# leejaeyong7/nerfacc

Hardware: AMD Instinct MI355X
Metric: rays/sec (fwd+bwd) through 128^3 occ-grid, 1M-ray batch (higher is better)
Workload: dtype f32; 1 GPU; cfg2: 1048576 image rays/GPU, 128^3 shell10 occ grid (G=1), step 2*sqrt(3)/1024, sampling+rendering fwd+bwd; rays_per_gpu=1048576, resolution=128, grid=shell10, samples_after_compaction=32244949, parallelism=ray-sharded x1, field=synthetic analytic field, native callbacks (see bench.py NativeField/TorchField)

## Files before the change

### include/nerfacc_hip.h

```cpp
#ifndef NERFACC_HIP_H
#define NERFACC_HIP_H

#include <stdint.h>

#ifdef __cplusplus
extern "C" {
#endif

#define NFA_OK 0
#define NFA_EINVAL (-1)
#define NFA_EHIP (-2)

#define NFA_MAX_GRID_LEVELS 8

typedef void *nfa_stream_t;

#define NFA_ELEM_F32 0
#define NFA_ELEM_F16 1
#define NFA_ELEM_BF16 2

const char *nfa_last_error(void);
#define NFA_VERSION 403
int nfa_version(void);
int nfa_set_tuning(const char *name, const char *value);
int nfa_device_arch(char *buf, int buflen);


int64_t nfa_cumsum_scratch_bytes(int64_t n);
int nfa_exclusive_cumsum_i64(const int64_t *cnts, int64_t n, int64_t *starts, int64_t *total,
                             void *scratch, nfa_stream_t stream);
int nfa_exclusive_cumsum_pairs_i64(const int64_t *cnts, int64_t n, int64_t *packed_info , int64_t *total,
                                   void *scratch, nfa_stream_t stream);
int nfa_exclusive_cumsum_pairs_stats_i64(const int64_t *cnts, int64_t n, int64_t *packed_info ,
                                         int64_t *total_and_stats , void *scratch, nfa_stream_t stream);

int nfa_pack_info(const int64_t *ray_indices, int64_t n, int64_t n_rays, int64_t *packed_info ,
                  int32_t *flags , void *scratch, nfa_stream_t stream);

int nfa_unpack_rows(const void *packed, const int64_t *packed_info , const uint8_t *mask, int64_t n_rays,
                    int64_t n_per_ray, int64_t n_packed, int64_t row_bytes, const void *pad_host, int32_t pad_bytes,
                    void *padded, nfa_stream_t stream);
int nfa_pack_rows(const void *padded, const int64_t *packed_info , const uint8_t *mask, int64_t n_rays,
                  int64_t n_per_ray, int64_t n_packed, int64_t row_bytes, void *packed, nfa_stream_t stream);
int nfa_mask_row_counts(const uint8_t *mask, int64_t n_rows, int64_t n_cols, int64_t *counts, nfa_stream_t stream);

int nfa_pack_bits(const uint8_t *binaries, int64_t n_cells, uint32_t *bits , nfa_stream_t stream);


int nfa_ray_aabb_intersect(const float *rays_o, const float *rays_d, int64_t n_rays,
                           const float *aabbs, int32_t n_aabbs, float near_plane, float far_plane,
                           float miss_value, float *t_mins, float *t_maxs, uint8_t *hits,
                           nfa_stream_t stream);

#define NFA_MAX_EVENT_LEVELS 8
int nfa_ray_events(const float *rays_o, const float *rays_d, int64_t n_rays, const float *aabbs, int32_t n_aabbs,
                   float *t_sorted, int64_t *t_indices, uint8_t *hits, nfa_stream_t stream);

typedef struct nfa_traverse_args {
    int64_t n_rays;
    const float *rays_o;
    const float *rays_d;
    const uint8_t *rays_mask;
    int32_t n_grids;
    int32_t res[3];
    const uint8_t *binaries;
    const float *aabbs;
    const uint8_t *hits;
    const float *t_sorted;
    const int64_t *t_indices;
    const float *near_planes;
    const float *far_planes;
    float step_size;
    float cone_angle;
    int32_t traverse_steps_limit;
    int32_t mode;
    float *iv_vals; int64_t *iv_ray_indices; uint8_t *iv_is_left; uint8_t *iv_is_right;
    int64_t *iv_starts; int64_t *iv_cnts;
    float *sm_vals; int64_t *sm_ray_indices; uint8_t *sm_is_valid;
    float *sm_t_starts; float *sm_t_ends;
    int64_t *sm_starts; int64_t *sm_cnts;
    float *terminate_planes;
    const int32_t *ray_filter;
    int32_t ray_filter_min;
    const uint64_t *bricks;
    const uint32_t *coarse;
    const int32_t *steps_limit_dev;
    const int64_t *n_listed_dev;
    const int32_t *run_if_nonzero;
} nfa_traverse_args;
int nfa_traverse_grids(const nfa_traverse_args *args, nfa_stream_t stream);

int64_t nfa_bricks_words(int32_t n_grids, const int32_t *res);
int nfa_pack_bricks(const uint8_t *binaries, int32_t n_grids, const int32_t *res, uint64_t *bricks,
                    uint32_t *coarse, nfa_stream_t stream);
int64_t nfa_walk_bits_words(int32_t n_grids, const int32_t *res);
int nfa_pack_walk_bits(const uint8_t *binaries, int32_t n_grids, const int32_t *res, uint32_t *bits, nfa_stream_t stream);
int nfa_traverse_runs(const nfa_traverse_args *args, const uint32_t *bits, int32_t *run_cnts, uint64_t *runs,
                      int32_t max_runs, int32_t *overflow_count, float near_hint, const int32_t *ray_order,
                      int64_t n_order, nfa_stream_t stream);
int nfa_bin_rays(const float *rays_o, const float *rays_d, int64_t n_rays, const float *box, int32_t *order,
                 void *scratch, nfa_stream_t stream);
int nfa_alive_rays(const float *opacity, const int64_t *packed_info , int64_t n_samples, float opacity_max,
                   int64_t n_rays, uint8_t *mask, int32_t *alive, int64_t *count, nfa_stream_t stream);
int nfa_testmode_begin(int64_t *alive_count, int32_t *state, int64_t n_rays, int32_t min_samples, int32_t max_samples,
                       int64_t *sm_cnts, int32_t *run_cnts, int64_t *zero_words, int32_t n_zero, nfa_stream_t stream);
int nfa_testmode_alive(const float *opacity, const int64_t *packed_info, int32_t *state, float opacity_max, int64_t n_rays,
                       uint8_t *mask, int32_t *alive, int64_t *count, int32_t count_samples, nfa_stream_t stream);
int nfa_bin_rays_levels(const float *rays_o, const float *rays_d, int64_t n_rays, const float *aabbs, int32_t n_grids,
                        const int32_t *res, float near_plane, int32_t *order, void *scratch,
                        uint64_t *coherence , nfa_stream_t stream);
int nfa_expand_runs(int64_t n_rays, float step_size, const int32_t *run_cnts, const uint64_t *runs,
                    int32_t max_runs, const int64_t *packed_info , float *t_starts,
                    float *t_ends, float *t_mids, int64_t *ray_indices, int64_t capacity, nfa_stream_t stream);
int nfa_fill_ray_indices(int64_t n_rays, const int64_t *packed_info , int64_t *ray_indices,
                         nfa_stream_t stream);
int nfa_traverse_cone_runs(const nfa_traverse_args *args, int32_t *run_cnts, uint64_t *runs, int32_t max_runs,
                           int32_t *overflow_count, const int32_t *ray_order ,
                           int64_t n_order, nfa_stream_t stream);
int nfa_traverse_cone_walk(const nfa_traverse_args *args, const uint32_t *bits, int32_t *run_cnts, uint64_t *runs,
                           int32_t max_runs, int32_t *overflow_count, uint32_t *arena, int32_t arena_capacity,
                           const int32_t *ray_order, int64_t n_order, nfa_stream_t stream);
int nfa_expand_cone_arena(const uint32_t *arena, int32_t n_entries, float step_size, float cone_angle,
                          const int64_t *packed_info , float *t_starts, float *t_ends, int64_t *ray_indices,
                          nfa_stream_t stream);
int nfa_expand_cone_runs(int64_t n_rays, float step_size, float cone_angle, const int32_t *run_cnts,
                         const uint64_t *runs, int32_t max_runs, const int64_t *packed_info, float *t_starts,
                         float *t_ends, int64_t *ray_indices, nfa_stream_t stream);
int nfa_expand_intervals(int64_t n_rays, float step_size, const int32_t *run_cnts, const uint64_t *runs,
                         int32_t max_runs, const int64_t *iv_packed_info , float *vals,
                         int64_t *ray_indices, uint8_t *is_left, uint8_t *is_right, nfa_stream_t stream);


int nfa_grid_cell_points(const int64_t *indices, const float *jitter , int64_t n, const int32_t *res,
                         const float *aabb , float *x , nfa_stream_t stream);
int nfa_grid_ema_update(float *occs, int64_t cell_base, const int64_t *indices, int64_t n, const float *occ,
                        float ema_decay, float *scratch , nfa_stream_t stream);
int64_t nfa_grid_rebinarize_scratch_bytes(void);
int nfa_grid_rebinarize(const float *occs, int32_t n_grids, const int32_t *res, float occ_thre, uint8_t *binaries,
                        uint32_t *walk_bits, void *scratch, nfa_stream_t stream);


void nfa_seg_plan(int64_t n_elems, int64_t n_rays, int64_t *tile_elems, int64_t *n_tiles);
int64_t nfa_seg_table_rows(int64_t n_tiles);
int nfa_seg_build_tiles(const int64_t *packed_info , int64_t n_rays, int64_t n_elems,
                        int64_t tile_elems, int64_t n_tiles, int64_t *tiles ,
                        int32_t *flags, nfa_stream_t stream);

int nfa_packed_scan(int kind, int reverse, const int64_t *packed_info, const int64_t *tiles, int64_t n_tiles,
                    int64_t n_rays, int64_t n_elems, const float *inputs, float *outputs,
                    nfa_stream_t stream);
int nfa_packed_scan_generic(int kind, int reverse, int normalize, const int64_t *packed_info,
                            int64_t n_rays, int64_t n_elems, const float *inputs, float *outputs,
                            nfa_stream_t stream);
int nfa_packed_prod_backward(int kind, const int64_t *packed_info, const int64_t *tiles, int64_t n_tiles,
                             int64_t n_rays, int64_t n_elems, const float *inputs,
                             const float *outputs, const float *grad_outputs, float *grad_inputs,
                             nfa_stream_t stream);

int nfa_render_from_density_fwd(const float *t_starts, const float *t_ends, const float *sigmas,
                                const float *prefix_trans , const int64_t *packed_info,
                                const int64_t *tiles, int64_t n_tiles, int64_t n_rays, int64_t n_elems,
                                float *weights, float *trans, float *alphas, nfa_stream_t stream);
int nfa_render_from_alpha_fwd(const float *alphas, const float *prefix_trans, const int64_t *packed_info,
                              const int64_t *tiles, int64_t n_tiles, int64_t n_rays, int64_t n_elems,
                              float *weights, float *trans, nfa_stream_t stream);
int nfa_render_from_density_bwd(const float *t_starts, const float *t_ends, const float *trans,
                                const float *alphas, const float *g_weights, const float *g_trans,
                                const float *g_alphas, const int64_t *packed_info, const int64_t *tiles, int64_t n_tiles,
                                int64_t n_rays, int64_t n_elems, float *grad_sigmas, float *grad_x,
                                nfa_stream_t stream);
int nfa_density_cdf_rows_fwd(const float *t_starts, const float *t_ends, const float *sigmas, const int64_t *packed_info,
                             const int64_t *tiles, int64_t n_tiles, int64_t n_rays, int64_t n_elems, int32_t row_len,
                             float *trans, float *alphas, float *cdfs , nfa_stream_t stream);
int nfa_density_cdf_rows_bwd(const float *t_starts, const float *t_ends, const float *trans, const float *alphas,
                             const float *g_cdfs , const int64_t *packed_info, const int64_t *tiles,
                             int64_t n_tiles, int64_t n_rays, int64_t n_elems, int32_t row_len, float *grad_sigmas,
                             nfa_stream_t stream);
int nfa_render_from_alpha_bwd(const float *alphas, const float *trans, const float *g_weights,
                              const float *g_trans, const int64_t *packed_info, const int64_t *tiles, int64_t n_tiles,
                              int64_t n_rays, int64_t n_elems, float *grad_alphas, nfa_stream_t stream);

int nfa_render_visibility(const float *t_starts, const float *t_ends, const float *sigmas_or_alphas,
                          const float *prefix_trans, float early_stop_eps, float alpha_thre,
                          const int64_t *packed_info, const int64_t *tiles, int64_t n_tiles, int64_t n_rays,
                          int64_t n_elems, uint8_t *vis, int64_t *vis_cnts, nfa_stream_t stream);
int nfa_render_visibility_cs(const float *t_starts, float step, const float *sigmas, const float *prefix_trans,
                             float early_stop_eps, float alpha_thre, const int64_t *packed_info, const int64_t *tiles,
                             int64_t n_tiles, int64_t n_rays, int64_t n_elems, uint8_t *vis, int64_t *vis_cnts,
                             nfa_stream_t stream);
int nfa_compact_samples(const uint8_t *vis, const float *t_starts, const float *t_ends,
                        const int64_t *packed_info, const int64_t *tiles, int64_t n_tiles, const int64_t *out_starts,
                        int64_t n_rays, int64_t n_elems, int64_t *out_ray_indices,
                        float *out_t_starts, float *out_t_ends, int64_t capacity, nfa_stream_t stream);

int nfa_accumulate_along_rays(const float *weights, const float *values, int32_t D,
                              const int64_t *packed_info, const int64_t *tiles, int64_t n_tiles, int64_t n_rays,
                              int64_t n_elems, int accumulate, float *out, nfa_stream_t stream);
int nfa_accumulate_along_rays_atomic(const float *weights, const float *values, int32_t D,
                                     const int64_t *ray_indices, int64_t n_rays, int64_t n_elems,
                                     float *out, nfa_stream_t stream);
int nfa_accumulate_along_rays_bwd(const float *weights, const float *values, int32_t D,
                                  const float *g_out, const int64_t *packed_info, const int64_t *tiles, int64_t n_tiles,
                                  int64_t n_rays, int64_t n_elems, float *g_weights, float *g_values,
                                  nfa_stream_t stream);
int nfa_render_accumulate_fwd(const float *weights, const float *rgbs, const float *t_starts,
                              const float *t_ends, const int64_t *packed_info, const int64_t *tiles, int64_t n_tiles,
                              int64_t n_rays, int64_t n_elems, float *colors, float *opacities,
                              float *depths, nfa_stream_t stream);
int nfa_render_accumulate_bwd(const float *weights, const float *rgbs, const float *t_starts,
                              const float *t_ends, const float *g_colors, const float *g_opacities,
                              const float *g_depths, const int64_t *packed_info, const int64_t *tiles, int64_t n_tiles,
                              int64_t n_rays, int64_t n_elems, float *g_weights, float *g_rgbs,
                              nfa_stream_t stream);

int nfa_render_fused_fwd(const float *t_starts, const float *t_ends, const float *sigmas, const float *rgbs,
                         const int64_t *packed_info, const int64_t *tiles, int64_t n_tiles, int64_t n_rays,
                         int64_t n_elems, float *weights, float *trans, float *alphas, float *colors,
                         float *opacities, float *depths, nfa_stream_t stream);
int nfa_render_fused_bwd(const float *t_starts, const float *t_ends, const float *rgbs, const float *trans,
                         const float *alphas, const float *g_colors, const float *g_opacities,
                         const float *g_depths, const float *g_weights, const float *g_trans,
                         const float *g_alphas, const int64_t *packed_info, const int64_t *tiles, int64_t n_tiles,
                         int64_t n_rays, int64_t n_elems, float *grad_sigmas, float *grad_rgbs,
                         nfa_stream_t stream);
int nfa_render_fused_fwd_cs(const float *t_starts, float step, const float *sigmas, const float *rgbs,
                            const int64_t *packed_info, const int64_t *tiles, int64_t n_tiles, int64_t n_rays,
                            int64_t n_elems, float *weights, float *trans, float *alphas, float *colors,
                            float *opacities, float *depths, nfa_stream_t stream);
int nfa_render_fused_bwd_cs(const float *t_starts, float step, const float *rgbs, const float *trans,
                            const float *alphas, const float *g_colors, const float *g_opacities,
                            const float *g_depths, const float *g_weights, const float *g_trans,
                            const float *g_alphas, const int64_t *packed_info, const int64_t *tiles, int64_t n_tiles,
                            int64_t n_rays, int64_t n_elems, float *grad_sigmas, float *grad_rgbs,
                            nfa_stream_t stream);

#define NFA_ACT_NONE 0
#define NFA_ACT_TRUNC_EXP 1
#define NFA_ACT_EXP 2
#define NFA_ACT_RELU 3
#define NFA_ACT_SOFTPLUS 4
#define NFA_RGB_ACT_NONE 0
#define NFA_RGB_ACT_SIGMOID 1
// ... 348 lines not shown
```

### nerfacc_amd/_backend.py

```python
from __future__ import annotations

import ctypes as C
import os
import threading
from typing import Optional

import torch

from . import _build

_lock = threading.Lock()
_lib: Optional[C.CDLL] = None

_vp, _i64, _i32, _f32, _u64, _int = C.c_void_p, C.c_int64, C.c_int32, C.c_float, C.c_uint64, C.c_int


class TraverseArgs(C.Structure):
    _fields_ = [
        ("n_rays", _i64), ("rays_o", _vp), ("rays_d", _vp), ("rays_mask", _vp),
        ("n_grids", _i32), ("res", _i32 * 3), ("binaries", _vp), ("aabbs", _vp),
        ("hits", _vp), ("t_sorted", _vp), ("t_indices", _vp),
        ("near_planes", _vp), ("far_planes", _vp),
        ("step_size", _f32), ("cone_angle", _f32), ("traverse_steps_limit", _i32), ("mode", _i32),
        ("iv_vals", _vp), ("iv_ray_indices", _vp), ("iv_is_left", _vp), ("iv_is_right", _vp),
        ("iv_starts", _vp), ("iv_cnts", _vp),
        ("sm_vals", _vp), ("sm_ray_indices", _vp), ("sm_is_valid", _vp),
        ("sm_t_starts", _vp), ("sm_t_ends", _vp), ("sm_starts", _vp), ("sm_cnts", _vp),
        ("terminate_planes", _vp),
        ("ray_filter", _vp), ("ray_filter_min", _i32),
        ("bricks", _vp), ("coarse", _vp),
        ("steps_limit_dev", _vp), ("n_listed_dev", _vp), ("run_if_nonzero", _vp),
    ]


class MLPDesc(C.Structure):
    _fields_ = [("n_in", _i32), ("n_out", _i32), ("width", _i32), ("n_hidden", _i32), ("bias", _i32), ("skip_mask", _i32)]


OPTIM_MAX_GROUPS, OPTIM_MAX_MILESTONES = 16, 8


class OptimGroup(C.Structure):
    _fields_ = [("lr", C.c_double), ("beta1", C.c_double), ("beta2", C.c_double), ("eps", C.c_double), ("weight_decay", C.c_double),
                ("flags", _i32), ("reserved", _i32)]


class OptimArgs(C.Structure):
    _fields_ = [("n_groups", _i32), ("n_milestones", _i32), ("groups", OptimGroup * OPTIM_MAX_GROUPS),
                ("start_factor", C.c_double), ("gamma", C.c_double), ("warmup_iters", _i64), ("milestones", _i64 * OPTIM_MAX_MILESTONES),
                ("growth_factor", _f32), ("backoff_factor", _f32), ("growth_interval", _i32), ("reserved", _i32)]


_SIGS = {
    "nfa_exclusive_cumsum_i64": [_vp, _i64, _vp, _vp, _vp, _vp],
    "nfa_exclusive_cumsum_pairs_i64": [_vp, _i64, _vp, _vp, _vp, _vp],
    "nfa_exclusive_cumsum_pairs_stats_i64": [_vp, _i64, _vp, _vp, _vp, _vp],
    "nfa_pack_info": [_vp, _i64, _i64, _vp, _vp, _vp, _vp],
    "nfa_pdf_loss_fwd": [_vp, _vp, _vp, _vp, _i64, _i32, _i32, _f32, _vp, _vp, _vp],
    "nfa_pdf_loss_bwd": [_vp, _vp, _vp, _i64, _i32, _i32, _f32, _vp, _vp, _vp, _vp],
    "nfa_pdf_loss_partials": [_i64, _i32, _i32],
    "nfa_pdf_loss_sum_fwd": [_vp, _vp, _vp, _vp, _i64, _i32, _i32, _f32, _vp, _vp, _vp],
    "nfa_pdf_loss_mean_bwd": [_vp, _vp, _vp, _i64, _i32, _i32, _f32, _vp, _vp, _vp, _vp],
    "nfa_pack_bits": [_vp, _i64, _vp, _vp],
    "nfa_unpack_rows": [_vp, _vp, _vp, _i64, _i64, _i64, _i64, _vp, _i32, _vp, _vp],
    "nfa_pack_rows": [_vp, _vp, _vp, _i64, _i64, _i64, _i64, _vp, _vp],
    "nfa_mask_row_counts": [_vp, _i64, _i64, _vp, _vp],
    "nfa_ray_aabb_intersect": [_vp, _vp, _i64, _vp, _i32, _f32, _f32, _f32, _vp, _vp, _vp, _vp],
    "nfa_ray_events": [_vp, _vp, _i64, _vp, _i32, _vp, _vp, _vp, _vp],
    "nfa_traverse_grids": [C.POINTER(TraverseArgs), _vp],
    "nfa_bricks_words": [_i32, C.POINTER(_i32)],
    "nfa_pack_bricks": [_vp, _i32, C.POINTER(_i32), _vp, _vp, _vp],
    "nfa_walk_bits_words": [_i32, C.POINTER(_i32)],
    "nfa_pack_walk_bits": [_vp, _i32, C.POINTER(_i32), _vp, _vp],
    "nfa_traverse_runs": [C.POINTER(TraverseArgs), _vp, _vp, _vp, _i32, _vp, _f32, _vp, _i64, _vp],
    "nfa_bin_rays": [_vp, _vp, _i64, _vp, _vp, _vp, _vp],
    "nfa_grid_cell_points": [_vp, _vp, _i64, C.POINTER(_i32), _vp, _vp, _vp],
    "nfa_grid_ema_update": [_vp, _i64, _vp, _i64, _vp, _f32, _vp, _vp],
    "nfa_grid_rebinarize_scratch_bytes": [],
    "nfa_grid_rebinarize": [_vp, _i32, C.POINTER(_i32), _f32, _vp, _vp, _vp, _vp],
    "nfa_expand_runs": [_i64, _f32, _vp, _vp, _i32, _vp, _vp, _vp, _vp, _vp, _i64, _vp],
    "nfa_fill_ray_indices": [_i64, _vp, _vp, _vp],
    "nfa_traverse_cone_runs": [C.POINTER(TraverseArgs), _vp, _vp, _i32, _vp, _vp, _i64, _vp],
    "nfa_alive_rays": [_vp, _vp, _i64, _f32, _i64, _vp, _vp, _vp, _vp],
    "nfa_testmode_begin": [_vp, _vp, _i64, _i32, _i32, _vp, _vp, _vp, _i32, _vp],
    "nfa_testmode_alive": [_vp, _vp, _vp, _f32, _i64, _vp, _vp, _vp, _i32, _vp],
    "nfa_traverse_cone_walk": [C.POINTER(TraverseArgs), _vp, _vp, _vp, _i32, _vp, _vp, _i32, _vp, _i64, _vp],
    "nfa_expand_cone_arena": [_vp, _i32, _f32, _f32, _vp, _vp, _vp, _vp, _vp],
    "nfa_bin_rays_levels": [_vp, _vp, _i64, _vp, _i32, C.POINTER(_i32), _f32, _vp, _vp, _vp, _vp],
    "nfa_expand_cone_runs": [_i64, _f32, _f32, _vp, _vp, _i32, _vp, _vp, _vp, _vp, _vp],
    "nfa_expand_intervals": [_i64, _f32, _vp, _vp, _i32, _vp, _vp, _vp, _vp, _vp, _vp],
    "nfa_seg_plan": [_i64, _i64, C.POINTER(_i64), C.POINTER(_i64)],
    "nfa_seg_table_rows": [_i64],
    "nfa_seg_build_tiles": [_vp, _i64, _i64, _i64, _i64, _vp, _vp, _vp],
    "nfa_packed_scan": [_int, _int, _vp, _vp, _i64, _i64, _i64, _vp, _vp, _vp],
    "nfa_packed_scan_generic": [_int, _int, _int, _vp, _i64, _i64, _vp, _vp, _vp],
    "nfa_packed_prod_backward": [_int, _vp, _vp, _i64, _i64, _i64, _vp, _vp, _vp, _vp, _vp],
    "nfa_render_from_density_fwd": [_vp, _vp, _vp, _vp, _vp, _vp, _i64, _i64, _i64, _vp, _vp, _vp, _vp],
    "nfa_render_from_alpha_fwd": [_vp, _vp, _vp, _vp, _i64, _i64, _i64, _vp, _vp, _vp],
    "nfa_render_from_density_bwd": [_vp, _vp, _vp, _vp, _vp, _vp, _vp, _vp, _vp, _i64, _i64, _i64, _vp, _vp, _vp],
    "nfa_density_cdf_rows_fwd": [_vp, _vp, _vp, _vp, _vp, _i64, _i64, _i64, _i32, _vp, _vp, _vp, _vp],
    "nfa_density_cdf_rows_bwd": [_vp, _vp, _vp, _vp, _vp, _vp, _vp, _i64, _i64, _i64, _i32, _vp, _vp],
    "nfa_render_from_alpha_bwd": [_vp, _vp, _vp, _vp, _vp, _vp, _i64, _i64, _i64, _vp, _vp],
    "nfa_render_visibility": [_vp, _vp, _vp, _vp, _f32, _f32, _vp, _vp, _i64, _i64, _i64, _vp, _vp, _vp],
    "nfa_render_visibility_cs": [_vp, _f32, _vp, _vp, _f32, _f32, _vp, _vp, _i64, _i64, _i64, _vp, _vp, _vp],
    "nfa_compact_samples": [_vp, _vp, _vp, _vp, _vp, _i64, _vp, _i64, _i64, _vp, _vp, _vp, _i64, _vp],
    "nfa_accumulate_along_rays": [_vp, _vp, _i32, _vp, _vp, _i64, _i64, _i64, _int, _vp, _vp],
    "nfa_accumulate_along_rays_atomic": [_vp, _vp, _i32, _vp, _i64, _i64, _vp, _vp],
    "nfa_accumulate_along_rays_bwd": [_vp, _vp, _i32, _vp, _vp, _vp, _i64, _i64, _i64, _vp, _vp, _vp],
    "nfa_render_accumulate_fwd": [_vp, _vp, _vp, _vp, _vp, _vp, _i64, _i64, _i64, _vp, _vp, _vp, _vp],
    "nfa_render_accumulate_bwd": [_vp, _vp, _vp, _vp, _vp, _vp, _vp, _vp, _vp, _i64, _i64, _i64, _vp, _vp, _vp],
    "nfa_render_fused_fwd": [_vp, _vp, _vp, _vp, _vp, _vp, _i64, _i64, _i64, _vp, _vp, _vp, _vp, _vp, _vp, _vp],
    "nfa_render_fused_bwd": [_vp] * 13 + [_i64, _i64, _i64, _vp, _vp, _vp],
    "nfa_render_fused_fwd_cs": [_vp, _f32, _vp, _vp, _vp, _vp, _i64, _i64, _i64, _vp, _vp, _vp, _vp, _vp, _vp, _vp],
    "nfa_render_fused_bwd_cs": [_vp, _f32] + [_vp] * 11 + [_i64, _i64, _i64, _vp, _vp, _vp],
    "nfa_render_raw_fwd": [_vp] * 5 + [_i32, _f32, _i32, _vp, _vp, _i64, _i64, _i64] + [_vp] * 9,
    "nfa_render_raw_bwd": [_vp] * 5 + [_i32, _f32, _i32] + [_vp] * 9 + [_i64, _i64, _i64, _vp, _vp, _vp],
    "nfa_render_raw_fwd_t": [_i32] + [_vp] * 5 + [_i32, _f32, _i32, _vp, _vp, _i64, _i64, _i64] + [_vp] * 9,
    "nfa_render_raw_bwd_t": [_i32] + [_vp] * 5 + [_i32, _f32, _i32] + [_vp] * 9 + [_i64, _i64, _i64, _vp, _vp, _vp],
    "nfa_render_sdf_fwd": [_vp] * 6 + [_i32, _vp, _f32, _i32, _vp, _vp, _i64, _i64, _i64] + [_vp] * 7,
    "nfa_render_sdf_bwd": [_vp] * 6 + [_i32, _vp, _f32, _i32] + [_vp] * 9 + [_i64, _i64, _i64] + [_vp] * 5,
    "nfa_render_step_accumulate": [_vp, _vp, _vp, _vp, _vp, _vp, _i64, _i64, _i64, _f32, _vp, _vp, _vp, _vp, _vp],
    "nfa_distortion_fwd": [_vp, _vp, _vp, _vp, _vp, _i64, _i64, _i64, _vp, _vp, _vp, _vp],
    "nfa_distortion_bwd": [_vp] * 8 + [_i64, _i64, _i64, _vp, _vp, _vp, _vp],
    "nfa_importance_sampling": [_vp, _vp, _vp, _i64, _i64, _i64, _int, _u64, _u64, _vp, _vp, _vp],
    "nfa_importance_sampling_t": [_vp, _vp, _vp, _i64, _i64, _i64, _int, _u64, _u64, _vp, _vp, _int, _f32, _f32, _vp, _vp, _vp],
    "nfa_importance_sampling_packed": [_vp, _vp, _vp, _i64, _i64, _vp, _vp, _int, _u64, _u64, _vp, _vp, _vp, _vp, _vp, _vp, _vp],
    "nfa_searchsorted": [_vp, _vp, _vp, _i64, _i64, _i64, _vp, _vp, _i64, _vp, _vp, _vp],
    "nfa_opencv_lens_undistortion": [_vp, _vp, _i64, _i32, _i64, _f32, _i32, _vp, _vp],
    "nfa_opencv_lens_undistortion_fisheye": [_vp, _vp, _i64, _i32, _i64, _f32, _i32, _vp, _vp],
    "nfa_hashgrid_fwd": [_vp, _vp, _i64, _i32, _i32, _i32, _vp, _vp, _vp, _i64, _vp, _vp],
    "nfa_hashgrid_bwd": [_vp, _vp, _vp, _i64, _i32, _i32, _i32, _vp, _vp, _vp, _i64, _vp, _vp, _vp],
    "nfa_sh_fwd": [_vp, _i64, _i32, _vp, _vp],
    "nfa_sh_bwd": [_vp, _vp, _i64, _i32, _vp, _vp],
    "nfa_hashgrid_fwd_t": [_i32, _vp, _vp, _i64, _i32, _i32, _i32, _vp, _vp, _vp, _i64, _vp, _vp],
    "nfa_hashgrid_bwd_t": [_i32, _vp, _vp, _vp, _i64, _i32, _i32, _i32, _vp, _vp, _vp, _i64, _vp, _vp, _vp],
    "nfa_hashgrid_bwd_bwd": [_vp, _vp, _vp, _vp, _i64, _i32, _i32, _i32, _vp, _vp, _vp, _i64, _vp, _vp, _vp, _vp],
    "nfa_hashgrid_bwd_bwd_t": [_i32, _vp, _vp, _vp, _vp, _i64, _i32, _i32, _i32, _vp, _vp, _vp, _i64, _vp, _vp, _vp, _vp],
    "nfa_hashgrid_sorted_scratch_bytes": [_i64, _i32, _i32],
    "nfa_hashgrid_bwd_sorted": [_i32, _vp, _vp, _vp, _i64, _i32, _i32, _i32, _vp, _vp, _vp, _i64, _vp, _vp, _vp, _i64, _vp],
    "nfa_hashgrid_bwd_bwd_sorted": [_i32, _vp, _vp, _vp, _vp, _i64, _i32, _i32, _i32, _vp, _vp, _vp, _i64, _vp, _vp, _vp, _vp, _i64, _vp],
    "nfa_hashgrid_fwd_i": [_i32, _i32, _vp, _vp, _i64, _i32, _i32, _i32, _vp, _vp, _vp, _i64, _vp, _vp],
    "nfa_hashgrid_bwd_i": [_i32, _i32, _vp, _vp, _vp, _i64, _i32, _i32, _i32, _vp, _vp, _vp, _i64, _vp, _vp, _vp],
    "nfa_hashgrid_bwd_bwd_i": [_i32, _i32, _vp, _vp, _vp, _vp, _i64, _i32, _i32, _i32, _vp, _vp, _vp, _i64, _vp, _vp, _vp, _vp],
    "nfa_hashgrid_bwd_sorted_i": [_i32, _i32, _vp, _vp, _vp, _i64, _i32, _i32, _i32, _vp, _vp, _vp, _i64, _vp, _vp, _vp, _i64, _vp],
    "nfa_hashgrid_bwd_bwd_sorted_i": [_i32, _i32, _vp, _vp, _vp, _vp, _i64, _i32, _i32, _i32, _vp, _vp, _vp, _i64, _vp, _vp, _vp, _vp,
                                      _i64, _vp],
    "nfa_hashgrid_fwd_d": [_i32, _i32, _i32, _vp, _vp, _i64, _i32, _i32, _i32, _vp, _vp, _vp, _i64, _vp, _vp],
    "nfa_hashgrid_bwd_d": [_i32, _i32, _i32, _vp, _vp, _vp, _i64, _i32, _i32, _i32, _vp, _vp, _vp, _i64, _vp, _vp, _vp],
    "nfa_hashgrid_bwd_sorted_d": [_i32, _i32, _i32, _vp, _vp, _vp, _i64, _i32, _i32, _i32, _vp, _vp, _vp, _i64, _vp, _vp, _vp, _i64,
                                  _vp],
    "nfa_hashgrid_sorted_scratch_bytes_d": [_i32, _i64, _i32, _i32],
    "nfa_sh_fwd_t": [_i32, _vp, _i64, _i32, _vp, _vp],
    "nfa_sh_bwd_t": [_i32, _vp, _vp, _i64, _i32, _vp, _vp],
    "nfa_planegrid_fwd": [_i32, _i32, _i32, _vp, _vp, _i64, _i32, _i32, C.POINTER(_i32), _vp, _vp],
    "nfa_planegrid_bwd": [_i32, _i32, _i32, _vp, _vp, _vp, _i64, _i32, _i32, C.POINTER(_i32), _vp, _vp, _vp],
    "nfa_planereg_partials": [_i32, _i32, _i32, C.POINTER(_i32)],
    "nfa_planereg_fwd": [_i32, _vp, _i32, _i32, C.POINTER(_i32), _vp, _i64, _vp, _vp],
    "nfa_planereg_bwd": [_i32, _vp, _i32, _i32, C.POINTER(_i32), _vp, _vp, _vp],
    "nfa_vmgrid_fwd": [_i32, _i32, _vp, _vp, _i64, _i32, C.POINTER(_i32), _vp, _vp],
    "nfa_vmgrid_bwd": [_i32, _i32, _vp, _vp, _vp, _i64, _i32, C.POINTER(_i32), _vp, _vp, _vp],
    "nfa_vmgrid_resample": [_vp, C.POINTER(_i32), _vp, C.POINTER(_i32), _i32, _vp],
    "nfa_vmreg_partials": [_i32, C.POINTER(_i32)],
    "nfa_vmreg_fwd": [_vp, _i32, C.POINTER(_i32), _vp, _i64, _vp, _vp, _vp],
    "nfa_vmreg_bwd": [_vp, _i32, C.POINTER(_i32), _vp, _vp, _vp, _vp],
    "nfa_sinenc_fwd": [_i32, _vp, _vp, _vp, _i64, _i32, _i32, _i32, _i32, _vp, _vp],
    "nfa_sinenc_bwd": [_i32, _vp, _vp, _vp, _vp, _i64, _i32, _i32, _i32, _i32, _vp, _vp, _vp],
    "nfa_sinenc_bwd_bwd": [_i32, _vp, _vp, _vp, _vp, _i64, _i32, _i32, _i32, _i32, _vp, _vp, _vp],
    "nfa_sample_positions_fwd": [_vp, _vp, _vp, _vp, _vp, _i64, _i64, _i64, _vp, _vp, _i32, _i32, _vp, _vp, _vp, _vp],
    "nfa_sample_positions_bwd": [_vp] * 9 + [_i64, _i64, _i64, _i64, _vp, _vp, _i32, _i32, _vp, _vp, _vp, _vp, _vp, _vp],
    "nfa_generate_rays_fwd": [_vp, _vp, _i32, _vp, _i64, _i64, _vp, _i64, _vp, _i64, _vp, _i32, _i64, _i32, _i32, _f32, _i32, _f32, _i32,
                              _vp, _vp, _vp],
    "nfa_generate_rays_bwd": [_vp, _vp, _i32, _vp, _vp, _i64, _i64, _vp, _i64, _vp, _i64, _vp, _i32, _i64, _i32, _i32, _f32, _i32, _f32,
                              _i32, _vp, _vp, _vp, _i64, _i32, _vp, _vp, _vp],
    "nfa_generate_rays_chunk": [],
    "nfa_mlp_pack_weights": [_i32, _vp, _i32, _i32, _i32, _i32, _vp, _i64, _vp, _i64, _vp],
    "nfa_mlp_fwd": [_i32, _vp, _i32, _vp, _i64, _i32, _i32, _i32, _i32, _vp, _i32, _vp, _i32, _vp],
    "nfa_mlp_bwd_data": [_i32, _vp, _i32, _vp, _vp, _i64, _i32, _i32, _i32, _i32, _vp, _vp, _vp, _i32, _vp],
    "nfa_mlp_bwd_weights": [_i32, _vp, _i32, _vp, _vp, _vp, _i64, _i32, _i32, _i32, _i32, _vp, _i64, _vp, _vp],
    "nfa_mlp_tangent": [_i32, _vp, _i32, _vp, _vp, _i64, _i32, _i32, _i32, _i32, _vp, _vp, _i32, _vp],
    "nfa_mlp_net_pack_weights": [_i32, C.POINTER(MLPDesc), _vp, _vp, _i64, _vp, _i64, _vp],
    "nfa_mlp_net_fwd": [_i32, C.POINTER(MLPDesc), _vp, _i32, _vp, _vp, _i64, _vp, _i32, _vp, _i32, _vp],
    "nfa_mlp_net_bwd_data": [_i32, C.POINTER(MLPDesc), _vp, _i32, _vp, _vp, _i64, _vp, _vp, _vp, _i32, _vp],
    "nfa_mlp_net_bwd_weights": [_i32, C.POINTER(MLPDesc), _vp, _i32, _vp, _vp, _vp, _i64, _vp, _i64, _vp, _i32, _vp],
    "nfa_mlp_net_tangent": [_i32, C.POINTER(MLPDesc), _vp, _i32, _vp, _vp, _i64, _vp, _vp, _i32, _vp],
    "nfa_mlp_stream_pack_weights": [_i32, C.POINTER(MLPDesc), _vp, _vp, _i64, _vp, _i64, _vp],
    "nfa_mlp_stream_fwd": [_i32, C.POINTER(MLPDesc), _vp, _i32, _vp, _vp, _i64, _vp, _i32, _vp, _i32, _vp],
    "nfa_mlp_stream_bwd_data": [_i32, C.POINTER(MLPDesc), _vp, _i32, _vp, _vp, _i64, _vp, _vp, _vp, _i32, _vp],
    "nfa_mlp_stream_bwd_weights": [_i32, C.POINTER(MLPDesc), _vp, _i32, _vp, _vp, _vp, _i64, _vp, _i64, _vp, _i32, _vp],
    "nfa_optim_chunk_elems": [],
    "nfa_optim_scan": [_i32, _vp, _i32, _vp, _i64, _vp, _vp],
    "nfa_optim_decide": [C.POINTER(OptimArgs), _vp, _vp, _vp],
    "nfa_optim_update": [_i32, _vp, _i32, _vp, _i64, _vp, _i32, _vp],
    "nfa_cumsum_scratch_bytes": [_i64],
    "nfa_last_error": [],
    "nfa_version": [],
    "nfa_set_tuning": [C.c_char_p, C.c_char_p],
    "nfa_device_arch": [C.c_char_p, _int],
}
_RESTYPES = {"nfa_grid_rebinarize_scratch_bytes": _i64, "nfa_hashgrid_sorted_scratch_bytes": _i64, "nfa_hashgrid_sorted_scratch_bytes_d": _i64, "nfa_planereg_partials": _i64, "nfa_vmreg_partials": _i64, "nfa_bricks_words": _i64, "nfa_walk_bits_words": _i64, "nfa_pdf_loss_partials": _i64, "nfa_cumsum_scratch_bytes": _i64, "nfa_seg_table_rows": _i64, "nfa_seg_plan": None, "nfa_last_error": C.c_char_p}

EXPORTED_SYMBOLS = tuple(_SIGS)


def library_path() -> str:
    return _build.LIB_PATH


def load() -> C.CDLL:
    global _lib
    if _lib is not None:
        return _lib
    with _lock:
        if _lib is not None:
            return _lib
        path = _build.LIB_PATH
        if _build.is_stale() and _build.hipcc() is not None:
            path = _build.build()
        if not os.path.exists(path):
            raise RuntimeError(
                "nerfacc_amd: libnerfacc_hip.so is missing and hipcc is not available to build it. "
                "There is no CPU fallback for the native ops.")
        lib = C.CDLL(path)
        for name, argtypes in _SIGS.items():
            fn = getattr(lib, name)
            fn.argtypes = argtypes
            fn.restype = _RESTYPES[name] if name in _RESTYPES else _int
        if lib.nfa_version() != ABI_VERSION:
            raise RuntimeError(f"nerfacc_amd: {path} was built from include/nerfacc_hip.h version {lib.nfa_version()}, these "
                               f"bindings are written for {ABI_VERSION}: rebuild the library (nerfacc_amd._build.build(force=True))")
        _lib = lib
    return _lib


ABI_VERSION = 403


ELEM_CODES = {torch.float32: 0, torch.float16: 1, torch.bfloat16: 2}
INTERP_CODES = {"Linear": 0, "Smoothstep": 1}
PLANE_REDUCE_CODES = {"product": 0, "sum": 1}
VM_REDUCE_CODES = {"concat": 0, "sum": 1}


def set_tuning(name: str, value: Optional[str]) -> None:
    call("nfa_set_tuning", name.encode(), None if value is None else str(value).encode())


class NativeError(RuntimeError):
    """Counterpart of the RuntimeError TORCH_CHECK raises in the reference."""


def call(name: str, *args) -> None:
    lib = load()
    rc = getattr(lib, name)(*args)
    if rc != 0:
        msg = lib.nfa_last_error()
        raise NativeError(f"{name}: {msg.decode() if msg else rc}")


def call_group(name: str, fn) -> None:
    fn()


def ptr(t: Optional[torch.Tensor]):
    return None if t is None else t.data_ptr()


_RAW_STREAM = getattr(torch._C, "_cuda_getCurrentRawStream", None)
_CUR_DEVICE = getattr(torch._C, "_cuda_getDevice", None)


def stream() -> int:
    if _RAW_STREAM is not None and _CUR_DEVICE is not None:
        return _RAW_STREAM(_CUR_DEVICE())
    return torch.cuda.current_stream().cuda_stream


def require_device(*tensors: Optional[torch.Tensor]) -> torch.device:
    dev = None
    for t in tensors:
        if t is None:
            continue
        if not t.is_cuda:
            raise NotImplementedError(
                "nerfacc_amd: this op runs only on a ROCm device (the reference has no CPU "
                "implementation of its native ops either); got a tensor on " + str(t.device))
        if dev is None:
            dev = t.device
        elif t.device != dev:
            raise RuntimeError(f"nerfacc_amd: tensors on different devices ({dev} vs {t.device})")
    if dev is None:
        raise RuntimeError("nerfacc_amd: no tensor argument")
    return dev


def seg_plan(n_elems: int, n_rays: int = 0):
    t, n = _i64(0), _i64(0)
    load().nfa_seg_plan(n_elems, n_rays, C.byref(t), C.byref(n))
    return int(t.value), int(n.value)


def cumsum_scratch(n: int, device) -> torch.Tensor:
    nbytes = ((max(n, 1) + 2047) // 2048 + 1) * 8
    return torch.empty(nbytes // 8, dtype=torch.int64, device=device)
```

### nerfacc_amd/_segments.py

```python
from __future__ import annotations

import ctypes
import weakref
from dataclasses import dataclass
from typing import Optional

import torch
from torch import Tensor

from . import _backend as B


@dataclass
class SegInfo:
    packed_info: Tensor
    n_rays: int
    n_elems: int
    tiles: Optional[Tensor]
    contiguous: bool
    sorted_indices: bool = True
    n_tiles: int = 0
    trusted: bool = False


_ATTR = "_nfa_seg"
_ATTR_RI = "_nfa_seg_from_ray_indices"


def _build_tiles(packed_info: Tensor, n_elems: int, trusted: bool) -> SegInfo:
    dev = B.require_device(packed_info)
    n_rays = packed_info.shape[0]
    with torch.cuda.device(dev):
        tile_elems, n_tiles = B.seg_plan(n_elems, n_rays)
        tiles = torch.empty((int(B.load().nfa_seg_table_rows(n_tiles)), 2), dtype=torch.int64, device=dev)
        flag = None if trusted else torch.empty(1, dtype=torch.int32, device=dev)
        B.call("nfa_seg_build_tiles", B.ptr(packed_info), n_rays, n_elems, tile_elems, n_tiles, B.ptr(tiles), B.ptr(flag),
               B.stream())
        ok = True if trusted else (int(flag.item()) == 0)
    return SegInfo(packed_info, n_rays, n_elems, tiles if ok else None, ok, n_tiles=n_tiles, trusted=trusted)


def seginfo_from_packed(packed_info: Tensor, n_elems: int, trusted: bool = False) -> SegInfo:
    assert packed_info.dim() == 2 and packed_info.shape[-1] == 2, "packed_info must be 2-D with shape (B, 2)."
    cached = getattr(packed_info, _ATTR, None)
    if cached is not None and cached[0] == packed_info._version and cached[1] == n_elems:
        return cached[2]
    pi = packed_info
    if pi.dtype != torch.int64 or not pi.is_contiguous():
        pi = pi.to(torch.int64).contiguous()
    info = _build_tiles(pi, n_elems, trusted)
    try:
        setattr(packed_info, _ATTR, (packed_info._version, n_elems, info))
    except Exception:
        pass
    return info


def tag_trusted(packed_info: Tensor, n_elems: int) -> SegInfo:
    return seginfo_from_packed(packed_info, n_elems, trusted=True)


def pack_info_native(ray_indices: Tensor, n_rays: int):
    dev = B.require_device(ray_indices)
    ri = ray_indices if (ray_indices.dtype == torch.int64 and ray_indices.is_contiguous()) else \
        ray_indices.to(torch.int64).contiguous()
    with torch.cuda.device(dev):
        packed = torch.empty((n_rays, 2), dtype=torch.int64, device=dev)
        flag = torch.empty(1, dtype=torch.int32, device=dev)
        scratch = B.cumsum_scratch(n_rays, dev)
        B.call("nfa_pack_info", B.ptr(ri), ri.numel(), n_rays, B.ptr(packed), B.ptr(flag), B.ptr(scratch), B.stream())
    return packed, flag


def seginfo_from_ray_indices(ray_indices: Tensor, n_rays: int) -> SegInfo:
    assert ray_indices.dim() == 1, "ray_indices must be a 1D tensor with shape (n_samples)."
    assert n_rays is not None, "n_rays must be provided"
    cached = getattr(ray_indices, _ATTR_RI, None)
    if cached is not None and cached[0] == ray_indices._version and cached[1] == n_rays:
        return cached[2]
    packed, flag = pack_info_native(ray_indices, n_rays)
    info = _build_tiles(packed, ray_indices.numel(), trusted=True)
    info.sorted_indices = int(flag.item()) == 0
    try:
        setattr(ray_indices, _ATTR_RI, (ray_indices._version, n_rays, info))
    except Exception:
        pass
    return info


def tag_ray_indices(ray_indices: Tensor, n_rays: int, info: SegInfo) -> None:
    setattr(ray_indices, _ATTR_RI, (ray_indices._version, n_rays, info))


def resolve(n_elems: int, packed_info: Optional[Tensor], ray_indices: Optional[Tensor],
            n_rays: Optional[int]) -> Optional[SegInfo]:
    if packed_info is not None:
        return seginfo_from_packed(packed_info, n_elems)
    if ray_indices is not None:
        if n_rays is None:
            n_rays = int(ray_indices.max().item()) + 1 if ray_indices.numel() else 0
        return seginfo_from_ray_indices(ray_indices, n_rays)
    return None


_ATTR_CS = "_nfa_const_step"


def tag_const_step(t_starts: Tensor, t_ends: Tensor, step: float) -> None:
    tag = (t_ends._version, weakref.ref(t_starts), t_starts.data_ptr(), t_starts._version, ctypes.c_float(float(step)).value)
    try:
        setattr(t_ends, _ATTR_CS, tag)
    except Exception:
        pass


def const_step_of(t_starts: Optional[Tensor], t_ends: Optional[Tensor]) -> Optional[float]:
    tag = getattr(t_ends, _ATTR_CS, None) if t_ends is not None else None
    if tag is None or t_starts is None:
        return None
    te_version, ts_ref, ts_ptr, ts_version, step = tag
    if t_ends._version != te_version or ts_ref() is not t_starts:
        return None
    if t_starts.data_ptr() != ts_ptr or t_starts._version != ts_version:
        return None
    for t in (t_starts, t_ends):
        if not (t.is_cuda and t.dtype == torch.float32 and t.dim() == 1 and t.is_contiguous()):
            return None
    if t_starts.shape != t_ends.shape or not (0.0 < step < float("inf")):
        return None
    return step


_UNIFORM: "dict[tuple, SegInfo]" = {}


def uniform_seginfo(n_rows: int, row_len: int, device: torch.device) -> SegInfo:
    key = (int(n_rows), int(row_len), device.type, device.index)
    info = _UNIFORM.get(key)
    if info is None:
        starts = torch.arange(n_rows, dtype=torch.int64, device=device) * row_len
        packed = torch.stack([starts, torch.full_like(starts, row_len)], dim=-1)
        info = _build_tiles(packed, n_rows * row_len, trusted=True)
        setattr(packed, _ATTR, (packed._version, n_rows * row_len, info))
        if len(_UNIFORM) >= 6:
            _UNIFORM.pop(next(iter(_UNIFORM)))
        _UNIFORM[key] = info
    return info


def batched_native(*tensors: Optional[Tensor]) -> Optional[SegInfo]:
    ref = None
    for t in tensors:
        if t is None:
            continue
        if not t.is_cuda or t.dtype != torch.float32 or t.dim() < 1:
            return None
        if ref is None:
            ref = t
        elif t.shape != ref.shape:
            return None
    if ref is None or ref.numel() == 0:
        return None
    return uniform_seginfo(ref.numel() // ref.shape[-1], ref.shape[-1], ref.device)
```

### nerfacc_amd/csrc/common.hip.h

```cpp
#pragma once
#include <hip/hip_runtime.h>
#include <stdint.h>
#include <stdio.h>
#include <stdlib.h>
#include <string.h>

#include <type_traits>

#include "../../include/nerfacc_hip.h"

#define NFA_WAVE 64

namespace nfa {

void set_error(const char *fmt, ...);

#define NFA_REQUIRE(cond, ...)                         \
    do {                                               \
        if (!(cond)) {                                 \
            nfa::set_error(__VA_ARGS__);               \
            return NFA_EINVAL;                         \
        }                                              \
    } while (0)

#define NFA_CHECK_LAUNCH(name)                                                       \
    do {                                                                             \
        hipError_t e__ = hipGetLastError();                                          \
        if (e__ != hipSuccess) {                                                     \
            nfa::set_error("%s: launch failed: %s", name, hipGetErrorString(e__));   \
            return NFA_EHIP;                                                         \
        }                                                                            \
    } while (0)

const char *tuning_env(const char *name);

struct RefillPlan {
    bool refill;
    int64_t chunk;
    int32_t min_busy;
};
static inline RefillPlan refill_plan(int64_t n_walk, int32_t steps_limit)
{
    const char *refill_env = tuning_env("NFA_REFILL"), *refill_all = tuning_env("NFA_REFILL_ALL");
    if (!(steps_limit > 0 || (refill_all && refill_all[0] == '1')) || (refill_env && refill_env[0] == '0')) return RefillPlan{false, 64, 64};
    int64_t chunk = ((n_walk + 4095) / 4096 + 63) / 64 * 64;
    chunk = chunk < 64 ? 64 : (chunk > 1024 ? 1024 : chunk);
    int min_busy = 48;
    if (refill_env) { long c = 0; int m = 0; if (sscanf(refill_env, "%ld,%d", &c, &m) == 2 && c >= 64 && m >= 1 && m <= 64) { chunk = c / 64 * 64; min_busy = m; } }
    return RefillPlan{true, chunk, min_busy};
}

static inline hipStream_t as_stream(nfa_stream_t s) { return reinterpret_cast<hipStream_t>(s); }

__host__ __device__ static inline int64_t ceil_div64(int64_t a, int64_t b) { return (a + b - 1) / b; }

static inline unsigned grid_1d(int64_t n, int block, int64_t cap = 256 * 16)
{
    int64_t g = ceil_div64(n, block);
    if (g > cap) g = cap;
    if (g < 1) g = 1;
    return (unsigned)g;
}

static inline bool aligned16(const void *p) { return (reinterpret_cast<uintptr_t>(p) & 15) == 0; }
template <typename... P>
static inline bool all_aligned16(P... p) { return (aligned16(p) && ...); }

template <class F>
static void dispatch_bool(bool b, F &&f)
{
    if (b) f(std::true_type{});
    else f(std::false_type{});
}
template <class F>
static void dispatch_channels(int c, F &&f)
{
    if (c == 4) f(std::integral_constant<int, 4>{});
    else if (c == 3) f(std::integral_constant<int, 3>{});
    else if (c == 2) f(std::integral_constant<int, 2>{});
    else f(std::integral_constant<int, 1>{});
}
template <class F>
static void dispatch_lanes(int l, F &&f)
{
    if (l == 2) f(std::integral_constant<int, 2>{});
    else if (l == 4) f(std::integral_constant<int, 4>{});
    else if (l == 8) f(std::integral_constant<int, 8>{});
    else if (l == 16) f(std::integral_constant<int, 16>{});
    else if (l == 32) f(std::integral_constant<int, 32>{});
    else f(std::integral_constant<int, 64>{});
}
template <int... V, class Fn>
static void dispatch_value(int32_t v, Fn &&f)
{
    (void)((v == V && (f(std::integral_constant<int, V>{}), true)) || ...);
}

__device__ __forceinline__ int lane_id() { return __lane_id(); }

template <typename T>
__device__ __forceinline__ T wave_shfl_up(T v, int delta) { return __shfl_up(v, delta, NFA_WAVE); }
template <typename T>
__device__ __forceinline__ T wave_shfl(T v, int src) { return __shfl(v, src, NFA_WAVE); }

__device__ __forceinline__ int64_t wave_incl_sum_i64(int64_t v)
{
    const int lane = lane_id();
#pragma unroll
    for (int off = 1; off < NFA_WAVE; off <<= 1) {
        int64_t u = __shfl_up(v, off, NFA_WAVE);
        if (lane >= off) v += u;
    }
    return v;
}

__device__ __forceinline__ float wave_sum_f32(float v)
{
#pragma unroll
    for (int off = 32; off > 0; off >>= 1) v += __shfl_xor(v, off, NFA_WAVE);
    return v;
}

__device__ __forceinline__ int64_t uniform64(int64_t v)
{
    const uint32_t lo = (uint32_t)__builtin_amdgcn_readfirstlane((int32_t)(uint32_t)v);
    const uint32_t hi = (uint32_t)__builtin_amdgcn_readfirstlane((int32_t)(uint32_t)((uint64_t)v >> 32));
    return (int64_t)(((uint64_t)hi << 32) | lo);
}

template <int S>
__device__ __forceinline__ int32_t dpp_step(int32_t old, int32_t src)
{
    static_assert(S >= 0 && S < 6, "dpp_step");
    if constexpr (S == 0) return __builtin_amdgcn_update_dpp(old, src, 0x111, 0xf, 0xf, false);
    else if constexpr (S == 1) return __builtin_amdgcn_update_dpp(old, src, 0x112, 0xf, 0xf, false);
    else if constexpr (S == 2) return __builtin_amdgcn_update_dpp(old, src, 0x114, 0xf, 0xf, false);
    else if constexpr (S == 3) return __builtin_amdgcn_update_dpp(old, src, 0x118, 0xf, 0xf, false);
    else if constexpr (S == 4) return __builtin_amdgcn_update_dpp(old, src, 0x142, 0xa, 0xf, false);
    else return __builtin_amdgcn_update_dpp(old, src, 0x143, 0xc, 0xf, false);
}
template <int S>
__device__ __forceinline__ float dpp_step(float old, float src)
{
    return __int_as_float(dpp_step<S>(__float_as_int(old), __float_as_int(src)));
}
__device__ __forceinline__ int32_t dpp_prev_lane(int32_t old, int32_t src)
{
    return __builtin_amdgcn_update_dpp(old, src, 0x138, 0xf, 0xf, false);
}
__device__ __forceinline__ float dpp_prev_lane(float old, float src)
{
    return __int_as_float(dpp_prev_lane(__float_as_int(old), __float_as_int(src)));
}
__device__ __forceinline__ int32_t event_level(int64_t idx, int32_t G)
{
    const int32_t i = (int32_t)idx;
    return i >= G ? i - G : i;
}

__device__ __forceinline__ uint32_t mad_u24(uint32_t a, uint32_t b, uint32_t c)
{
    uint32_t r;
    asm("v_mad_u32_u24 %0, %1, %2, %3" : "=v"(r) : "v"(a), "v"(b), "v"(c));
    return r;
}
__device__ __forceinline__ int64_t xcd_fair_block(uint32_t b, uint32_t n_blocks)
{
    const uint32_t group = b >> 3;
    if (((group + 1u) << 3) > n_blocks) return b;
    return (int64_t)((b & ~7u) | ((b + group) & 7u));
}

__device__ __forceinline__ uint32_t sel_mask(uint32_t k, uint32_t x, uint32_t y)
{
    return __builtin_amdgcn_bitop3_b32(k, x, y, 0xca);
}
__device__ __forceinline__ float sel_mask(uint32_t k, float x, float y)
{
    return __builtin_bit_cast(float, __builtin_amdgcn_bitop3_b32(k, __builtin_bit_cast(uint32_t, x), __builtin_bit_cast(uint32_t, y), 0xca));
}
__device__ __forceinline__ uint32_t mask_less(float a, float b)
{
    return (uint32_t)(__builtin_bit_cast(int32_t, a - b) >> 31);
}
__device__ __forceinline__ float min3_f32(float a, float b, float c)
{
    float m;
    asm("v_min3_f32 %0, %1, %2, %3" : "=v"(m) : "v"(a), "v"(b), "v"(c));
    return m;
}

__device__ __forceinline__ int32_t last_lane(int32_t v) { return __builtin_amdgcn_readlane(v, 63); }
__device__ __forceinline__ float last_lane(float v) { return __int_as_float(__builtin_amdgcn_readlane(__float_as_int(v), 63)); }
__device__ __forceinline__ int32_t lane_value(int32_t v, int32_t l) { return __builtin_amdgcn_readlane(v, l); }
__device__ __forceinline__ float lane_value(float v, int32_t l) { return __int_as_float(__builtin_amdgcn_readlane(__float_as_int(v), l)); }


typedef float nfa_v4f __attribute__((ext_vector_type(4)));
typedef long long nfa_v2l __attribute__((ext_vector_type(2)));
typedef uint32_t nfa_v2u __attribute__((ext_vector_type(2)));
typedef uint32_t nfa_v4u __attribute__((ext_vector_type(4)));

typedef _Float16 nfa_f16;
// ... 200 lines not shown
```

### nerfacc_amd/csrc/grid.hip

```cpp
#include <stdarg.h>

#include "common.hip.h"
#include "march.h"

namespace nfa {

static thread_local char g_err[512] = "";
void set_error(const char *fmt, ...)
{
    va_list ap;
    va_start(ap, fmt);
    vsnprintf(g_err, sizeof(g_err), fmt, ap);
    va_end(ap);
}

struct TuningKnob { char name[32]; char value[64]; };
static TuningKnob g_knobs[8];
static int g_n_knobs = 0;
const char *tuning_env(const char *name)
{
    for (int i = 0; i < g_n_knobs; ++i)
        if (strcmp(g_knobs[i].name, name) == 0) return g_knobs[i].value[0] ? g_knobs[i].value : nullptr;
    return nullptr;
}
// ... 252 lines not shown
        if (a.traverse_steps_limit <= 0) return;
    }
    const int64_t n_walk = (EMIT == EMIT_RUNS && ro.order) ? ro.n_order : a.n_rays;
    for (int64_t slot_i = (int64_t)blockIdx.x * blockDim.x + threadIdx.x; slot_i < n_walk;
         slot_i += (int64_t)blockDim.x * gridDim.x) {
        const int64_t tid = (EMIT == EMIT_RUNS && ro.order) ? (int64_t)ro.order[slot_i] : slot_i;
        const bool overalloc = a.mode == 2;
        if (ray_masked(a, ro, tid)) continue;
        if (a.ray_filter != nullptr && a.ray_filter[tid] <= a.ray_filter_min) continue;
        int64_t iv_base = 0, sm_base = 0;
        if (EMIT != EMIT_NONE && EMIT != EMIT_RUNS) {
            if (a.mode == 1) {
                if (HAS_IV && a.iv_cnts[tid] == 0) continue;
                if (HAS_SM && a.sm_cnts[tid] == 0) continue;
            }
            if (HAS_IV) iv_base = a.iv_starts[tid];
            if (HAS_SM) sm_base = a.sm_starts[tid];
        }
        float near_plane, far_plane, o[3], d[3];
        const bool ray_ok = ray_load(a, tid, near_plane, far_plane, o, d);
        const float inv[3] = {1.0f / d[0], 1.0f / d[1], 1.0f / d[2]};

        RayState st;
        st.t_last = near_plane;
        st.continuous = 0;
        st.n_intervals = 0;
        st.n_samples = 0;
        st.brick_id = -1; st.brick_lo = st.brick_hi = 0u;
        st.n_runs = 0; st.run_len = 0;

        int32_t ev = ray_ok ? 0 : 2 * a.n_grids, level;
        float this_tmin, this_tmax;
        while (next_span<FUSED>(a, tid, o, inv, near_plane, far_plane, ev, level, this_tmin, this_tmax)) {
            traverse_span<EMIT, HAS_IV, HAS_SM>(a, tid, o, d, inv, level, this_tmin, this_tmax, iv_base, sm_base, st, ro);
            if (FUSED || (a.traverse_steps_limit > 0 && st.n_samples >= a.traverse_steps_limit)) break;
        }
        if (EMIT == EMIT_RUNS) {
            run_ray_close(a, ro, tid, st.t_last, st.n_samples, st.n_runs);
            continue;
        }
        if (a.terminate_planes) a.terminate_planes[tid] = st.t_last;
        if (EMIT == EMIT_NONE || overalloc) {
            if (HAS_IV) a.iv_cnts[tid] = st.n_intervals;
            if (HAS_SM) a.sm_cnts[tid] = st.n_samples;
        }
    }
}

template <int EMIT, bool HAS_IV, bool HAS_SM>
static void launch_traverse(const nfa_traverse_args &a, bool fused, hipStream_t s, const RunOut ro = RunOut{nullptr, nullptr, 0, nullptr, nullptr, 0})
{
    const unsigned grid = grid_1d((EMIT == EMIT_RUNS && ro.order) ? ro.n_order : a.n_rays, 256, 1 << 20);
    if (fused) hipLaunchKernelGGL((traverse_kernel<EMIT, HAS_IV, HAS_SM, true>), dim3(grid), dim3(256), 0, s, a, ro);
    else       hipLaunchKernelGGL((traverse_kernel<EMIT, HAS_IV, HAS_SM, false>), dim3(grid), dim3(256), 0, s, a, ro);
}

template <bool FUSED>
struct BrickWalker {
    const nfa_traverse_args &a;
    const RunOut &ro;
    int64_t tid;
    int32_t ev;
    float near_plane, far_plane, o[3], d[3], inv[3];
    RayState st;
    SpanState &sp;
    __device__ __forceinline__ bool take(int64_t ray)
    {
        tid = ray;
        if (ray_masked(a, ro, tid)) return false;
        if (a.ray_filter != nullptr && a.ray_filter[tid] <= a.ray_filter_min) return false;
        const bool ray_ok = ray_load(a, tid, near_plane, far_plane, o, d);
#pragma unroll
        for (int ax = 0; ax < 3; ++ax) inv[ax] = 1.0f / d[ax];
        st.t_last = near_plane; st.continuous = 0; st.n_samples = 0;
        st.brick_id = -1; st.n_runs = 0; st.run_len = 0;
        ev = ray_ok ? 0 : 2 * a.n_grids;
        return true;
    }
    __device__ __forceinline__ bool next_span()
    {
        int32_t level;
        float this_tmin, this_tmax;
        if (!nfa::next_span<FUSED>(a, tid, o, inv, near_plane, far_plane, ev, level, this_tmin, this_tmax)) return false;
        span_begin(a, o, d, inv, level, this_tmin, this_tmax, st, sp);
        return true;
    }
    __device__ __forceinline__ int cell()
    {
        if (!span_cell<EMIT_RUNS, false, true, true>(a, tid, 0, 0, sp, st, ro)) return RF_WALK;
        return (a.traverse_steps_limit > 0 && st.n_samples >= a.traverse_steps_limit) ? RF_FINISH : RF_SPAN;
    }
    __device__ __forceinline__ void finish() { run_ray_close(a, ro, tid, st.t_last, st.n_samples, st.n_runs); }
};
template <bool FUSED>
__global__ __launch_bounds__(256) void traverse_refill_kernel(const nfa_traverse_args a, const RunOut ro, const int32_t chunk,
                                                              const int32_t min_busy)
{
    SpanState sp;
    BrickWalker<FUSED> w{a, ro, 0, 0, 0.0f, 0.0f, {0.0f, 0.0f, 0.0f}, {0.0f, 0.0f, 0.0f}, {0.0f, 0.0f, 0.0f}, RayState{0.0f, 0, 0, 0, -1, 0u, 0u, 0, 0}, sp};
    refill_schedule(w, ro.order, ro.order ? ro.n_order : a.n_rays, (int64_t)blockIdx.x * (blockDim.x >> 6) + (threadIdx.x >> 6), chunk, min_busy);
}

constexpr int CS_THREADS = 256;
constexpr int CS_ITEMS = 8;
constexpr int CS_BLOCK = CS_THREADS * CS_ITEMS;

__device__ __forceinline__ int64_t block_excl_scan_i64(int64_t v, int64_t &block_total, int64_t *lds )
{
    const int lane = lane_id(), wave = threadIdx.x >> 6;
    const int64_t incl = wave_incl_sum_i64(v);
    if (lane == 63) lds[wave] = incl;
    __syncthreads();
    int64_t wave_off = 0, tot = 0;
#pragma unroll
    for (int w = 0; w < CS_THREADS / 64; ++w) {
        const int64_t x = lds[w];
        if (w < wave) wave_off += x;
        tot += x;
    }
    __syncthreads();
    block_total = tot;
    return wave_off + incl - v;
}

__global__ __launch_bounds__(CS_THREADS) void cumsum_partials_kernel(const int64_t *__restrict__ in, int64_t n,
                                                                      int64_t in_stride, int64_t *__restrict__ partials)
{
    __shared__ int64_t lds[8];
    const int64_t base = (int64_t)blockIdx.x * CS_BLOCK + (int64_t)threadIdx.x * CS_ITEMS;
    int64_t s = 0;
#pragma unroll
    for (int k = 0; k < CS_ITEMS; ++k)
        if (base + k < n) s += in[(base + k) * in_stride];
    int64_t tot;
    block_excl_scan_i64(s, tot, lds);
    if (threadIdx.x == 0) partials[blockIdx.x] = tot;
}

__global__ __launch_bounds__(CS_THREADS) void cumsum_spine_kernel(int64_t *partials, int64_t n_blocks, int64_t *total)
{
    __shared__ int64_t lds[8];
    int64_t carry = 0;
    for (int64_t base = 0; base < n_blocks; base += CS_THREADS) {
        const int64_t i = base + threadIdx.x;
        const int64_t v = i < n_blocks ? partials[i] : 0;
        int64_t tot;
        const int64_t ex = block_excl_scan_i64(v, tot, lds);
        if (i < n_blocks) partials[i] = carry + ex;
        carry += tot;
    }
    if (threadIdx.x == 0 && total) *total = carry;
}

template <bool SPINE>
__global__ __launch_bounds__(CS_THREADS) void cumsum_final_kernel(const int64_t *__restrict__ in, int64_t n,
                                                                   int64_t in_stride,
                                                                   const int64_t *__restrict__ partials,
                                                                   int64_t *__restrict__ out, int pairs,
                                                                   int64_t *__restrict__ total,
                                                                   unsigned long long *__restrict__ stats = nullptr)
{
    __shared__ int64_t lds[8];
    int64_t block_off = 0;
    if (SPINE) {
        int64_t before = 0;
        for (int64_t j = threadIdx.x; j < (int64_t)blockIdx.x; j += CS_THREADS) before += partials[j];
        block_excl_scan_i64(before, block_off, lds);
    } else {
        block_off = partials[blockIdx.x];
    }
    const int64_t base = (int64_t)blockIdx.x * CS_BLOCK + (int64_t)threadIdx.x * CS_ITEMS;
    int64_t v[CS_ITEMS];
    int64_t s = 0;
#pragma unroll
    for (int k = 0; k < CS_ITEMS; ++k) {
        v[k] = (base + k < n) ? in[(base + k) * in_stride] : 0;
        s += v[k];
    }
    int64_t tot;
    int64_t run = block_off + block_excl_scan_i64(s, tot, lds);
    if (SPINE && total && blockIdx.x == gridDim.x - 1 && threadIdx.x == 0) *total = block_off + tot;
    if (SPINE && stats && (blockIdx.x & 7) == 0) {
        int64_t m = 0;
#pragma unroll
        for (int k = 0; k < CS_ITEMS; ++k) m = v[k] > m ? v[k] : m;
        for (int off = 1; off < 8; off <<= 1) { const int64_t u = __shfl_xor(m, off, 64); m = u > m ? u : m; }
        int64_t gm = (lane_id() & 7) == 0 ? m : 0;
        for (int off = 8; off < 64; off <<= 1) gm += __shfl_xor(gm, off, 64);
        if (lane_id() == 0) atomicAdd(&stats[0], (unsigned long long)gm);
        if (threadIdx.x == 0) atomicAdd(&stats[1], (unsigned long long)tot);
    }
#pragma unroll
    for (int k = 0; k < CS_ITEMS; ++k) {
        if (base + k < n) {
            if (pairs) { out[2 * (base + k)] = run; out[2 * (base + k) + 1] = v[k]; }
            else out[base + k] = run;
        }
        run += v[k];
    }
}

static int run_cumsum(const int64_t *in, int64_t n, int64_t in_stride, int64_t *out, int pairs, int64_t *total,
                      void *scratch, hipStream_t s, unsigned long long *stats = nullptr)
{
    const int64_t n_blocks = ceil_div64(n > 0 ? n : 1, CS_BLOCK);
    int64_t *partials = reinterpret_cast<int64_t *>(scratch);
    hipLaunchKernelGGL(cumsum_partials_kernel, dim3((unsigned)n_blocks), dim3(CS_THREADS), 0, s, in, n, in_stride, partials);
    if (n_blocks <= 2048) {
        hipLaunchKernelGGL(cumsum_final_kernel<true>, dim3((unsigned)n_blocks), dim3(CS_THREADS), 0, s, in, n, in_stride, partials,
                           out, pairs, total, stats);
    } else {
        hipLaunchKernelGGL(cumsum_spine_kernel, dim3(1), dim3(CS_THREADS), 0, s, partials, n_blocks, total);
        hipLaunchKernelGGL(cumsum_final_kernel<false>, dim3((unsigned)n_blocks), dim3(CS_THREADS), 0, s, in, n, in_stride, partials,
                           out, pairs, nullptr, nullptr);
    }
    NFA_CHECK_LAUNCH("exclusive_cumsum_i64");
    return NFA_OK;
}

__global__ __launch_bounds__(256) void pack_hist_kernel(const int64_t *__restrict__ ray_indices, int64_t n,
                                                        int64_t n_rays, unsigned long long *__restrict__ packed,
                                                        int32_t *__restrict__ flags)
{
    const int lane = lane_id();
    for (int64_t base = ((int64_t)blockIdx.x * blockDim.x + threadIdx.x) - lane; base < n;
         base += (int64_t)blockDim.x * gridDim.x) {
        const int64_t i = base + lane;
        const bool valid = i < n;
        const int64_t r = valid ? ray_indices[i] : -1;
        int64_t prev = __shfl_up(r, 1, NFA_WAVE);
        if (lane == 0) prev = (i > 0 && valid) ? ray_indices[i - 1] : r;
        const bool in_range = valid && r >= 0 && r < n_rays;
        if (valid && (!in_range || r < prev)) atomicOr(flags, 1);
        const bool head = valid && (lane == 0 || r != prev);
        const unsigned long long heads = __ballot(head);
        const unsigned long long live = __ballot(valid);
        if (head && in_range) {
            const unsigned long long later = (lane == 63) ? 0ull : (heads >> (lane + 1));
            const int next = later ? (lane + 1 + __builtin_ctzll(later)) : (int)__builtin_popcountll(live);
            atomicAdd(&packed[2 * r + 1], (unsigned long long)(next - lane));
        }
    }
}

__global__ void zero_i64_kernel(int64_t *p, int64_t n, int32_t *flags)
{
    for (int64_t i = (int64_t)blockIdx.x * blockDim.x + threadIdx.x; i < n; i += (int64_t)blockDim.x * gridDim.x) p[i] = 0;
    if (flags && blockIdx.x == 0 && threadIdx.x == 0) *flags = 0;
}

__global__ __launch_bounds__(256) void pack_bits_kernel(const uint8_t *__restrict__ b, int64_t n, uint32_t *__restrict__ bits)
{
    const int lane = lane_id();
    for (int64_t base = ((int64_t)blockIdx.x * blockDim.x + threadIdx.x) - lane; base < n;
         base += (int64_t)blockDim.x * gridDim.x) {
        const int64_t i = base + lane;
        const unsigned long long m = __ballot(i < n && b[i] != 0);
        if (lane == 0) bits[base >> 5] = (uint32_t)m;
        if (lane == 32 && base + 32 < n) bits[(base >> 5) + 1] = (uint32_t)(m >> 32);
    }
}

}

using namespace nfa;

extern "C" {

const char *nfa_last_error(void) { return g_err; }
int nfa_version(void) { return NFA_VERSION; }
int nfa_set_tuning(const char *name, const char *value)
{
    NFA_REQUIRE(name && strlen(name) > 0 && strlen(name) < sizeof(g_knobs[0].name), "set_tuning: bad name");
    NFA_REQUIRE(!value || strlen(value) < sizeof(g_knobs[0].value), "set_tuning: value too long");
    int i = 0;
    while (i < g_n_knobs && strcmp(g_knobs[i].name, name) != 0) ++i;
    if (i == g_n_knobs) {
        NFA_REQUIRE(g_n_knobs < (int)(sizeof(g_knobs) / sizeof(g_knobs[0])), "set_tuning: too many knobs");
        strcpy(g_knobs[g_n_knobs++].name, name);
    }
    strcpy(g_knobs[i].value, value ? value : "");
    return NFA_OK;
}

int nfa_device_arch(char *buf, int buflen)
{
    int dev = 0;
    hipDeviceProp_t prop;
    if (hipGetDevice(&dev) != hipSuccess || hipGetDeviceProperties(&prop, dev) != hipSuccess) {
        set_error("no HIP device");
        return NFA_EHIP;
    }
    snprintf(buf, buflen, "%s", prop.gcnArchName);
    return NFA_OK;
}

int64_t nfa_cumsum_scratch_bytes(int64_t n) { return (ceil_div64(n > 0 ? n : 1, CS_BLOCK) + 1) * 8; }

int nfa_exclusive_cumsum_i64(const int64_t *cnts, int64_t n, int64_t *starts, int64_t *total, void *scratch,
                             nfa_stream_t stream)
{
    NFA_REQUIRE(n >= 0 && scratch && (n == 0 || (cnts && starts)), "exclusive_cumsum_i64: bad arguments");
    return run_cumsum(cnts, n, 1, starts, 0, total, scratch, as_stream(stream));
}

int nfa_exclusive_cumsum_pairs_i64(const int64_t *cnts, int64_t n, int64_t *packed_info, int64_t *total, void *scratch,
                                   nfa_stream_t stream)
{
    NFA_REQUIRE(n >= 0 && scratch && (n == 0 || (cnts && packed_info)), "exclusive_cumsum_pairs_i64: bad arguments");
    return run_cumsum(cnts, n, 1, packed_info, 1, total, scratch, as_stream(stream));
}

int nfa_exclusive_cumsum_pairs_stats_i64(const int64_t *cnts, int64_t n, int64_t *packed_info, int64_t *total_and_stats,
                                         void *scratch, nfa_stream_t stream)
{
    NFA_REQUIRE(n >= 0 && scratch && total_and_stats && (n == 0 || (cnts && packed_info)),
                "exclusive_cumsum_pairs_stats_i64: bad arguments");
    return run_cumsum(cnts, n, 1, packed_info, 1, total_and_stats, scratch, as_stream(stream),
                      reinterpret_cast<unsigned long long *>(total_and_stats + 1));
}

int nfa_pack_info(const int64_t *ray_indices, int64_t n, int64_t n_rays, int64_t *packed_info, int32_t *flags,
                  void *scratch, nfa_stream_t stream)
{
    NFA_REQUIRE(n >= 0 && n_rays >= 0 && flags && scratch, "pack_info: bad arguments");
    NFA_REQUIRE(n_rays == 0 || packed_info, "pack_info: packed_info is null");
    NFA_REQUIRE(n == 0 || ray_indices, "pack_info: ray_indices is null");
    hipStream_t s = as_stream(stream);
    hipLaunchKernelGGL(zero_i64_kernel, dim3(grid_1d(2 * n_rays + 1, 256)), dim3(256), 0, s, packed_info, 2 * n_rays, flags);
    if (n > 0 && n_rays > 0)
        hipLaunchKernelGGL(pack_hist_kernel, dim3(grid_1d(n, 256)), dim3(256), 0, s, ray_indices, n, n_rays,
                           reinterpret_cast<unsigned long long *>(packed_info), flags);
    NFA_CHECK_LAUNCH("pack_info");
    if (n_rays == 0) return NFA_OK;
    return run_cumsum(packed_info + 1, n_rays, 2, packed_info, 1, nullptr, scratch, s);
}

int nfa_pack_bits(const uint8_t *binaries, int64_t n_cells, uint32_t *bits, nfa_stream_t stream)
{
    NFA_REQUIRE(n_cells >= 0 && (n_cells == 0 || (binaries && bits)), "pack_bits: bad arguments");
    if (n_cells == 0) return NFA_OK;
    hipLaunchKernelGGL(pack_bits_kernel, dim3(grid_1d(n_cells, 256)), dim3(256), 0, as_stream(stream), binaries, n_cells, bits);
    NFA_CHECK_LAUNCH("pack_bits");
    return NFA_OK;
}

int nfa_ray_aabb_intersect(const float *rays_o, const float *rays_d, int64_t n_rays, const float *aabbs,
                           int32_t n_aabbs, float near_plane, float far_plane, float miss_value, float *t_mins,
                           float *t_maxs, uint8_t *hits, nfa_stream_t stream)
{
    NFA_REQUIRE(n_rays >= 0 && n_aabbs >= 0, "ray_aabb_intersect: negative size");
    if (n_rays * (int64_t)n_aabbs == 0) return NFA_OK;
    NFA_REQUIRE(rays_o && rays_d && aabbs && t_mins && t_maxs && hits, "ray_aabb_intersect: null pointer");
    hipLaunchKernelGGL(ray_aabb_kernel, dim3(grid_1d(n_rays * n_aabbs, 256)), dim3(256), 0, as_stream(stream), rays_o,
                       rays_d, n_rays, aabbs, n_aabbs, near_plane, far_plane, miss_value, t_mins, t_maxs, hits);
    NFA_CHECK_LAUNCH("ray_aabb_intersect");
    return NFA_OK;
}

int nfa_ray_events(const float *rays_o, const float *rays_d, int64_t n_rays, const float *aabbs, int32_t n_aabbs,
                   float *t_sorted, int64_t *t_indices, uint8_t *hits, nfa_stream_t stream)
{
    NFA_REQUIRE(n_rays >= 0 && n_aabbs >= 1 && n_aabbs <= NFA_MAX_EVENT_LEVELS, "ray_events: 1..NFA_MAX_EVENT_LEVELS boxes");
    if (n_rays == 0) return NFA_OK;
    NFA_REQUIRE(rays_o && rays_d && aabbs && t_sorted && t_indices && hits, "ray_events: null pointer");
    const dim3 grid(grid_1d(n_rays, 256)), block(256);
    hipStream_t s = as_stream(stream);
    static constexpr decltype(&ray_events_kernel<1>) kernels[NFA_MAX_EVENT_LEVELS] = {
        ray_events_kernel<1>, ray_events_kernel<2>, ray_events_kernel<3>, ray_events_kernel<4>,
        ray_events_kernel<5>, ray_events_kernel<6>, ray_events_kernel<7>, ray_events_kernel<8>};
    hipLaunchKernelGGL(kernels[n_aabbs - 1], grid, block, 0, s, rays_o, rays_d, n_rays, aabbs, t_sorted, t_indices, hits);
    NFA_CHECK_LAUNCH("ray_events");
    return NFA_OK;
}

int nfa_traverse_grids(const nfa_traverse_args *pa, nfa_stream_t stream)
{
    NFA_REQUIRE(pa != nullptr, "traverse_grids: null args");
    const nfa_traverse_args &a = *pa;
    NFA_REQUIRE(a.n_rays >= 0 && a.n_rays < (int64_t)1 << 31, "traverse_grids: n_rays out of range");
    if (a.n_rays == 0) return NFA_OK;
    NFA_REQUIRE(a.mode >= 0 && a.mode <= 2, "traverse_grids: mode must be 0, 1 or 2");
    NFA_REQUIRE(a.rays_o && a.rays_d && a.binaries && a.aabbs && a.near_planes && a.far_planes,
                "traverse_grids: null input pointer");
    NFA_REQUIRE(a.n_grids >= 1 && a.res[0] > 0 && a.res[1] > 0 && a.res[2] > 0, "traverse_grids: bad grid shape");
    NFA_REQUIRE((int64_t)a.res[0] * a.res[1] * a.res[2] < (int64_t)1 << 31, "traverse_grids: grid level too large");
    const bool fused = !a.t_sorted && !a.t_indices && !a.hits;
    NFA_REQUIRE(fused || (a.t_sorted && a.t_indices && a.hits),
                "traverse_grids: t_sorted, t_indices and hits must be given together");
    NFA_REQUIRE(!fused || a.n_grids == 1, "traverse_grids: in-kernel intersection supports one grid; pass t_sorted/t_indices/hits");
    NFA_REQUIRE(a.mode != 2 || a.traverse_steps_limit > 0,
                "traverse_steps_limit must be > 0 when over_allocate is true");
    const bool has_iv = a.iv_cnts != nullptr, has_sm = a.sm_cnts != nullptr;
    NFA_REQUIRE(has_iv || has_sm, "traverse_grids: nothing to compute");
    const bool direct = a.sm_t_starts != nullptr;
    hipStream_t s = as_stream(stream);
    if (a.mode == 0) {
        if (has_iv && has_sm) launch_traverse<EMIT_NONE, true, true>(a, fused, s);
        else if (has_sm) launch_traverse<EMIT_NONE, false, true>(a, fused, s);
        else launch_traverse<EMIT_NONE, true, false>(a, fused, s);
    } else {
        NFA_REQUIRE(!has_iv || (a.iv_vals && a.iv_ray_indices && a.iv_is_left && a.iv_is_right && a.iv_starts),
                    "traverse_grids: interval outputs missing");
        NFA_REQUIRE(!has_sm || a.sm_starts, "traverse_grids: sample starts missing");
        if (direct) {
            NFA_REQUIRE(!has_iv && has_sm && a.sm_t_ends,
                        "traverse_grids: direct emission needs sm_t_starts, sm_t_ends and no intervals");
            launch_traverse<EMIT_DIRECT, false, true>(a, fused, s);
        } else {
            NFA_REQUIRE(!has_sm || (a.sm_vals && a.sm_ray_indices && a.sm_is_valid), "traverse_grids: sample outputs missing");
            if (has_iv && has_sm) launch_traverse<EMIT_API, true, true>(a, fused, s);
            else if (has_sm) launch_traverse<EMIT_API, false, true>(a, fused, s);
            else launch_traverse<EMIT_API, true, false>(a, fused, s);
        }
    }
    NFA_CHECK_LAUNCH("traverse_grids");
    return NFA_OK;
}

int nfa_traverse_cone_runs(const nfa_traverse_args *pa, int32_t *run_cnts, uint64_t *runs, int32_t max_runs,
                           int32_t *overflow_count, const int32_t *ray_order, int64_t n_order, nfa_stream_t stream)
{
    NFA_REQUIRE(pa != nullptr, "traverse_cone_runs: null args");
    const nfa_traverse_args &a = *pa;
    NFA_REQUIRE(a.n_rays >= 0 && a.n_rays < (int64_t)1 << 31, "traverse_cone_runs: n_rays out of range");
    NFA_REQUIRE(overflow_count, "traverse_cone_runs: overflow_count is null");
    hipStream_t s = as_stream(stream);
    if (hipMemsetAsync(overflow_count, 0, sizeof(int32_t), s) != hipSuccess) { set_error("traverse_cone_runs: memset failed"); return NFA_EHIP; }
    if (a.n_rays == 0) return NFA_OK;
    NFA_REQUIRE(a.step_size > 0.0f && a.cone_angle > 0.0f, "traverse_cone_runs: needs step_size > 0 and cone_angle > 0");
    NFA_REQUIRE(a.mode == 0 || a.mode == 2, "traverse_cone_runs: mode must be 0 (all rays) or 2 (rays_mask + traverse_steps_limit)");
    NFA_REQUIRE(a.mode != 2 || a.traverse_steps_limit > 0, "traverse_steps_limit must be > 0 when over_allocate is true");
    NFA_REQUIRE(a.rays_o && a.rays_d && a.binaries && a.aabbs && a.near_planes && a.far_planes && a.sm_cnts && !a.iv_cnts &&
                    run_cnts && runs, "traverse_cone_runs: null pointer (or interval outputs requested)");
    NFA_REQUIRE(max_runs >= 1 && max_runs <= 32, "traverse_cone_runs: max_runs must be in [1, 32]");
    NFA_REQUIRE(a.n_grids >= 1 && a.res[0] > 0 && a.res[1] > 0 && a.res[2] > 0, "traverse_cone_runs: bad grid shape");
    NFA_REQUIRE((int64_t)a.res[0] * a.res[1] * a.res[2] < (int64_t)1 << 31, "traverse_cone_runs: grid level too large");
    const bool fused = !a.t_sorted && !a.t_indices && !a.hits;
    NFA_REQUIRE(fused || (a.t_sorted && a.t_indices && a.hits), "traverse_cone_runs: t_sorted, t_indices and hits must be given together");
    NFA_REQUIRE(!fused || a.n_grids == 1, "traverse_cone_runs: in-kernel intersection supports one grid");
    RunOut ro;
    ro.run_cnts = run_cnts;
    ro.runs = reinterpret_cast<unsigned long long *>(runs);
    ro.max_runs = max_runs;
    ro.overflow = overflow_count;
    ro.order = ray_order;
    ro.n_order = ray_order ? n_order : a.n_rays;
    NFA_REQUIRE(!ray_order || (n_order >= 0 && n_order <= a.n_rays), "traverse_cone_runs: n_order out of range");
    if (ray_order && n_order == 0) return NFA_OK;
    const RefillPlan plan = refill_plan(ro.n_order, a.traverse_steps_limit);
    if (plan.refill) {
        const unsigned grid = (unsigned)ceil_div64(ceil_div64(ro.n_order, plan.chunk), 4);
        if (fused) hipLaunchKernelGGL((traverse_refill_kernel<true>), dim3(grid), dim3(256), 0, s, a, ro, (int32_t)plan.chunk, plan.min_busy);
        else       hipLaunchKernelGGL((traverse_refill_kernel<false>), dim3(grid), dim3(256), 0, s, a, ro, (int32_t)plan.chunk, plan.min_busy);
    } else {
        launch_traverse<EMIT_RUNS, false, true>(a, fused, s, ro);
    }
    NFA_CHECK_LAUNCH("traverse_cone_runs");
    return NFA_OK;
}

}
```

### nerfacc_amd/csrc/segscan.hip

```cpp
#include <stdlib.h>

#include "common.hip.h"
#include "samples.h"

namespace nfa {

constexpr int SE = 4;
constexpr int SQ = SE / 4;
constexpr int SEG_CHUNK = 64 * SE;
#ifndef NFA_SEG_TILE_ROWS
#define NFA_SEG_TILE_ROWS 256
#endif
constexpr int64_t SEG_TILE_ROWS = NFA_SEG_TILE_ROWS;
#ifndef NFA_VIS_EXP_FREE
#define NFA_VIS_EXP_FREE 1
#endif
#ifndef NFA_SEG_WAVES_PER_BLOCK
#define NFA_SEG_WAVES_PER_BLOCK 4
#endif
constexpr int SEG_WAVES_PER_BLOCK = NFA_SEG_WAVES_PER_BLOCK;

__global__ __launch_bounds__(256) void seg_build_tiles_kernel(const int64_t *__restrict__ packed_info, int64_t n_rays,
                                                              int64_t n_elems, int64_t tile_elems, int64_t n_tiles,
                                                              longlong2 *__restrict__ tiles, int32_t *__restrict__ flags)
{
    for (int64_t r = (int64_t)blockIdx.x * blockDim.x + threadIdx.x; r <= n_rays;
         r += (int64_t)blockDim.x * gridDim.x) {
        int64_t b_lo, b_hi, e_first;
        bool bad = false;
        if (r < n_rays) {
            const int64_t s = packed_info[2 * r], n = packed_info[2 * r + 1];
            int64_t s_prev = -1;
            if (r > 0) {
                const int64_t ps = packed_info[2 * r - 2], pn = packed_info[2 * r - 1];
                s_prev = ps;
                bad |= (ps + pn != s);
            }
            bad |= (n < 0) || (s < 0) || (s + n > n_elems);
            if (bad) { if (flags) atomicOr(flags, 1); continue; }
            b_lo = (s_prev < 0) ? 0 : s_prev / tile_elems + (r - 1) / SEG_TILE_ROWS + 1;
            b_hi = s / tile_elems + r / SEG_TILE_ROWS;
            e_first = s;
        } else {
            const int64_t s_prev = n_rays > 0 ? packed_info[2 * n_rays - 2] : -1;
            const int64_t n_prev = n_rays > 0 ? packed_info[2 * n_rays - 1] : 0;
            b_lo = (s_prev < 0) ? 0 : s_prev / tile_elems + (n_rays - 1) / SEG_TILE_ROWS + 1;
            b_hi = n_tiles;
            e_first = (s_prev < 0) ? 0 : s_prev + n_prev;
            if (s_prev > n_elems) { if (flags) atomicOr(flags, 1); continue; }
        }
        for (int64_t b = b_lo; b <= b_hi && b <= n_tiles; ++b) tiles[b] = make_longlong2(r, e_first);
    }
}

__host__ __device__ inline int64_t seg_table_rows(int64_t n_tiles) { return n_tiles + 1; }

struct F4 { float v[SE]; };

struct Pos {
    int64_t c;
    int32_t off;
    int32_t safe;
    bool valid[SE];
    bool any, all;
    int32_t d_lo, d_hi;
    bool qany[SQ], qall[SQ];
    __device__ __forceinline__ int64_t p0() const { return c + off; }
};

template <bool VEC>
__device__ __forceinline__ void ld4(const float *__restrict__ p, const Pos &q, F4 &out)
{
    const float *b = p + q.c;
    if (VEC) {
#pragma unroll
        for (int h = 0; h < SQ; ++h) {
            const nfa_v4f v = *reinterpret_cast<const nfa_v4f *>(b + (q.qany[h] ? q.off + 4 * h : q.safe));
            out.v[4 * h] = v.x; out.v[4 * h + 1] = v.y; out.v[4 * h + 2] = v.z; out.v[4 * h + 3] = v.w;
        }
    } else {
#pragma unroll
        for (int j = 0; j < SE; ++j) out.v[j] = b[q.valid[j] ? q.off + j : q.safe];
    }
}
__device__ __forceinline__ float sel(const F4 &r, int j, const bool valid[SE], float fill) { return valid[j] ? r.v[j] : fill; }

#define NFA_ELEMENTWISE_PATH() asm volatile("; element-wise path" ::: "memory")
template <bool VEC>
__device__ __forceinline__ void store4(float *__restrict__ p, const Pos &q, const float v[SE])
{
    float *b = p + q.c;
#pragma unroll
    for (int h = 0; h < SQ; ++h) {
        if (VEC && q.qall[h]) {
            store_f4(b + q.off + 4 * h, v[4 * h], v[4 * h + 1], v[4 * h + 2], v[4 * h + 3]);
        } else {
            NFA_ELEMENTWISE_PATH();
#pragma unroll
            for (int j = 4 * h; j < 4 * h + 4; ++j)
                if (q.valid[j]) b[q.off + j] = v[j];
        }
    }
}

struct StepHeads {
    int32_t lh[SE];
    uint32_t acc;
    bool open_prefix;
    bool carry_on_lane_end;
    int32_t carry_lane;
    int32_t ph;
    int32_t rid[SE], prev_rid[SE];
    bool is_head[SE];
};

template <int S>
__device__ __forceinline__ void heads_step(int32_t &ah, uint32_t &acc)
{
    const int32_t uh = dpp_step<S>(-1, ah);
    if (ah < 0) { acc |= 1u << S; ah = uh; }
}

template <int DIR>
__device__ __forceinline__ void resolve_heads(const int32_t hj[SE], const bool valid[SE], int32_t carry_rid, StepHeads &hd)
{
#pragma unroll
    for (int k = 0; k < SE; ++k) {
        const int j = DIR > 0 ? k : SE - 1 - k;
        const int32_t h = valid[j] ? hj[j] : -1;
        hd.is_head[k] = h >= 0;
        hd.lh[k] = (k == 0 || h >= 0) ? h : hd.lh[k - 1 < 0 ? 0 : k - 1];
    }
    int32_t ah = hd.lh[SE - 1];
    uint32_t acc = 0;
    heads_step<0>(ah, acc); heads_step<1>(ah, acc); heads_step<2>(ah, acc);
    heads_step<3>(ah, acc); heads_step<4>(ah, acc); heads_step<5>(ah, acc);
    const int lane = lane_id(), r = lane & 15;
    const uint32_t has_src = (r >= 1 ? 1u : 0u) | (r >= 2 ? 2u : 0u) | (r >= 4 ? 4u : 0u) | (r >= 8 ? 8u : 0u) |
                             ((lane & 16) ? 16u : 0u) | (lane >= 32 ? 32u : 0u);
    hd.acc = acc & has_src;
    int32_t ph = dpp_prev_lane(-1, ah);
    hd.open_prefix = ph < 0;
    if (ph < 0) ph = carry_rid;
    hd.ph = ph;
    int32_t pr = ph;
#pragma unroll
    for (int k = 0; k < SE; ++k) {
        hd.prev_rid[k] = pr;
        hd.rid[k] = hd.lh[k] >= 0 ? hd.lh[k] : ph;
        pr = hd.rid[k];
    }
}

template <int S, int N, class FI, class FC>
__device__ __forceinline__ void values_step(const StepHeads &hd, float av[N], FI identity, FC comb)
{
    const bool take = (hd.acc >> S) & 1u;
#pragma unroll
    for (int ch = 0; ch < N; ++ch) {
        const float uv = dpp_step<S>(identity(ch), av[ch]);
        if (take) av[ch] = comb(ch, uv, av[ch]);
    }
}

template <int N, class FI, class FC>
__device__ __forceinline__ void scan_values(const StepHeads &hd, const float x[SE][N], float carry[N], float incl[SE][N],
// ... 2743 lines not shown
```

### nerfacc_amd/csrc/walk.hip

```cpp
#include "common.hip.h"
#include "march.h"
#include "walk_layout.h"

namespace nfa {

constexpr int WK_EV = 16;
static_assert(WK_EV == 16 || WK_EV == 8, "the list-full test is one bit of the slot address: a power of two");
constexpr int WK_WAVES = 5;
constexpr int WK_LG = 8;
constexpr int WK_THREADS = 1 << (WK_LG - 2);
constexpr uint32_t WK_FULL = (uint32_t)WK_EV << WK_LG;
constexpr uint32_t WK_GUARD = (1u << 9) | (1u << 19) | (1u << 29);
constexpr int WK_MAX_RES = 512;

__global__ __launch_bounds__(256) void pack_walk_bits_kernel(const uint8_t *__restrict__ binaries, int32_t n_grids, int32_t rx, int32_t ry,
                                                             int32_t rz, WalkLayout L, uint32_t *__restrict__ bits)
{
    const int64_t n_words = ((int64_t)n_grids << L.bits) >> 5;
    for (int64_t wi = (int64_t)blockIdx.x * blockDim.x + threadIdx.x; wi < n_words; wi += (int64_t)blockDim.x * gridDim.x) {
        const uint32_t base = (uint32_t)(wi << 5);
        const uint32_t lvl = base >> L.bits, in_lvl = base & ((1u << L.bits) - 1u);
        uint32_t w = 0u;
        for (uint32_t b = 0; b < 32u; ++b) {
            const uint32_t pidx = in_lvl | b;
            const uint32_t x = bit_extract(pidx, L.mask[0]), y = bit_extract(pidx, L.mask[1]), z = bit_extract(pidx, L.mask[2]);
            const uint32_t rest = pidx & ~(L.mask[0] | L.mask[1] | L.mask[2]);
            if (rest == 0u && x < (uint32_t)rx && y < (uint32_t)ry && z < (uint32_t)rz &&
                binaries[(((int64_t)lvl * rx + x) * ry + y) * rz + z])
                w |= 1u << b;
        }
        bits[wi] = w;
    }
}

struct WalkParams {
    const uint32_t *bits;
    WalkLayout lay;
    int32_t *run_cnts;
    unsigned long long *runs;
    int64_t n_rays;
    int32_t max_runs;
    int32_t *overflow;
    const int32_t *order;
    int64_t n_order;
    ApproachTable approach;
    LatticeTable lat;
};

enum { WK_EMPTY = 0, WK_OCC = 1, WK_SPAN = 2 };
__device__ __forceinline__ bool is_span_entry(uint32_t ev_span, int32_t k) { return (ev_span >> k) & 1u; }

struct Marcher {
    float t_last;
    int32_t continuous;
    int32_t n_samples, n_chains, n_runs;
    float run_inc;
    float span_tmax;
    int32_t ptype;
    int32_t at_near;
    uint32_t fe, fq;
    float fstep, frcp;
};

__device__ __forceinline__ float vmin_f32(float a, float b)
{
    float m;
    asm("v_min_f32 %0, %1, %2" : "=v"(m) : "v"(a), "v"(b));
    return m;
}

__device__ __forceinline__ void marcher_refresh(Marcher &s, float dt)
{
    const uint32_t e = f32_bits(s.t_last) >> 23;
    if (e == s.fe) return;
    s.fe = e; s.fq = 0u; s.fstep = 0.f; s.frcp = 0.f;
    if (e >= 1u && e < 254u) {
        const float r = ldexpf(dt, 150 - (int)e);
        if (r >= 0.5f && r < 8388608.0f) {
            const float k = floorf(r), f = r - k;
            if (f != 0.5f) {
                s.fq = (uint32_t)k + (f > 0.5f ? 1u : 0u);
                s.fstep = ldexpf((float)s.fq, (int)e - 150);
                s.frcp = NFA_RCP(s.fstep);
            }
        }
    }
}

__device__ __forceinline__ void store_run(const WalkParams &p, int32_t slot, int64_t tid, unsigned long long rec)
{
    if (slot < p.max_runs) (p.runs + tid)[(uint64_t)(uint32_t)slot * (uint64_t)(uint32_t)p.n_rays] = rec;
}

__device__ __forceinline__ void marcher_emit(Marcher &s, float t0, float inc, uint32_t n, const WalkParams &p, int64_t tid)
{
    if (!(s.continuous && inc == s.run_inc)) {
        store_run(p, s.n_runs, tid,
                      (unsigned long long)f32_bits(t0) |
                          ((unsigned long long)((uint32_t)s.n_samples | (s.continuous ? 0x80000000u : 0u)) << 32));
        s.n_runs++;
        s.n_chains += s.continuous ? 0 : 1;
        s.run_inc = inc;
    }
    s.n_samples += (int32_t)n;
    s.continuous = 1;
}

struct ApproachLds {
    float T[APPROACH_MAX];
    uint32_t q[APPROACH_MAX];
};
__device__ __forceinline__ void marcher_approach(const WalkParams &p, const ApproachLds &tb, float &t, float half, float thr)
{
    const uint32_t n = p.approach.n, e_lo = p.approach.e_lo;
    if (n == 0u || f32_bits(t) != p.approach.near_bits) return;
    const float c = thr - half;
    if (!(c > 0.0f)) return;
    uint32_t ec = f32_bits(c) >> 23;
    if (ec > e_lo + n - 1u) ec = e_lo + n - 1u;
    for (int d = 0; d < 2; ++d) {
        const uint32_t e = ec - (uint32_t)d;
        if (e < e_lo || e > ec) return;
        const uint32_t i = e - e_lo;
        const float T = tb.T[i];
        if (tb.q[i] != 0u && T > t && T + half < thr) { t = T; return; }
    }
}

__device__ __forceinline__ int marcher_cross(Marcher &s, float thr, int type, float dt, float half, int32_t limit, const WalkParams &p,
                                             const ApproachLds &tb, int64_t tid)
{
    int progress = 0;
    if (s.at_near) {
        s.at_near = 0;
        progress = 1;
        if (type != WK_OCC) marcher_approach(p, tb, s.t_last, half, thr);
    }
#pragma unroll 1
    for (int round = 0; round < 4; ++round) {
        const uint32_t fe_before = s.fe;
        marcher_refresh(s, dt);
        if (s.fe != fe_before) progress = 1;
        if (s.fq == 0u) return 0;
        const float t = s.t_last;
        if (!(t + half < thr)) break;
        const uint32_t bt = f32_bits(t), q = s.fq;
        const uint32_t room = (bt | 0x7FFFFFu) - bt;
        uint32_t budget = 0xFFFFFFFFu;
        if (type == WK_OCC && limit > 0) {
            if (s.n_samples >= limit) break;
            budget = (uint32_t)(limit - s.n_samples);
        }
        if (q <= room) {
            uint32_t n_b = (uint32_t)((float)room * NFA_RCP((float)q));
            if (n_b * q > room) n_b--;
            if (n_b * q > room) n_b--;
            if ((n_b + 1u) * q <= room) n_b++;
            if ((n_b + 1u) * q <= room) n_b++;
            if (n_b == 0u || n_b * q > room || (n_b + 1u) * q <= room) return 0;
            if (!(bits_f32(bt + (n_b - 1u) * q) + half < thr)) break;
            n_b = min(n_b, budget);
            if (type == WK_OCC) marcher_emit(s, t, s.fstep, n_b, p, tid);
            s.t_last = bits_f32(bt + n_b * q);
            progress = 1;
            if (n_b == budget) break;
            budget -= n_b;
        }
        const float t1 = s.t_last;
        if (!(t1 + half < thr)) break;
        const float tn = t1 + dt;
        if (tn == t1 || (f32_bits(tn) >> 23) == (f32_bits(t1) >> 23)) return 0;
        if (type == WK_OCC) marcher_emit(s, t1, tn - t1, 1u, p, tid);
        s.t_last = tn;
        progress = 1;
    }
    marcher_refresh(s, dt);
    return progress ? 2 : 1;
}

__device__ __forceinline__ void marcher_general(Marcher &s, float thr, int type, float dt, float half, int32_t limit,
                                                const WalkParams &p, int64_t tid)
{
    Stepper stp;
    stepper_init(stp);
    const bool emit = type == WK_OCC;
    for (;;) {
        if (!(s.t_last + half < thr)) break;
        uint32_t budget = 0xFFFFFFFFu;
        if (emit && limit > 0) {
            if (s.n_samples >= limit) break;
            budget = (uint32_t)(limit - s.n_samples);
        }
        const float t = s.t_last;
        float tn = t, inc;
        const uint32_t n = stepper_advance(stp, tn, dt, half, thr, budget, &inc);
        if (n == 0u) {
            if (!emit) s.t_last = thr;
// ... 417 lines not shown
        bool hit = true;
        const float *bmin = a.aabbs, *bmax = a.aabbs + 3;
        if (inv[0] >= 0) { tmin = (bmin[0] - o[0]) * inv[0]; tmax = (bmax[0] - o[0]) * inv[0]; }
        else             { tmin = (bmax[0] - o[0]) * inv[0]; tmax = (bmin[0] - o[0]) * inv[0]; }
#pragma unroll
        for (int ax = 1; ax < 3; ++ax) {
            if (inv[ax] >= 0) { lo = (bmin[ax] - o[ax]) * inv[ax]; hi = (bmax[ax] - o[ax]) * inv[ax]; }
            else              { lo = (bmax[ax] - o[ax]) * inv[ax]; hi = (bmin[ax] - o[ax]) * inv[ax]; }
            if (tmin > hi || lo > tmax) hit = false;
            if (lo > tmin) tmin = lo;
            if (hi < tmax) tmax = hi;
        }
        if (tmax <= 0) hit = false;
        f_tmin = fmaxf(tmin, near_plane); f_tmax = fminf(tmax, far_plane);
        f_pending = hit && f_tmin < f_tmax;
    }
    const int32_t G = a.n_grids;
    int32_t next_i = 0;
    if (!(isfinite(o[0]) && isfinite(o[1]) && isfinite(o[2]) && isfinite(d[0]) && isfinite(d[1]) && isfinite(d[2]))) {
        f_pending = false;
        next_i = 2 * G;
    }
    if (LATTICE && f32_bits(near_plane) != p.lat.near_bits) {
        atomicOr(reinterpret_cast<unsigned int *>(p.overflow + 1), 1u);
        f_pending = false;
        next_i = 2 * G;
    }

    WalkSpan sp;
    sp.tx = sp.ty = sp.tz = sp.dx = sp.dy = sp.dz = 0.f; sp.mx = sp.my = sp.mz = 0u; sp.rem = 0u; sp.widx = 0u; sp.flip = 0u; sp.end = 0u; sp.over = 0u;
    int32_t in_span = 0, has_open = 0, open_type = 0;
    float m_p = 0.f, m_q = 0.f;
    uint32_t i_p = 0u, w_p = 0u, i_q = 0u, w_q = 0u;
    int32_t par = 0;
    uint32_t ev_addr = lane_off;
    uint32_t ev_span = 0u;
    float m_last = 0.f;

    for (;;) {
        int32_t finished = 0;
        for (;;) {
            if (!in_span) {
                const uint32_t used = (ev_addr >> WK_LG) + (uint32_t)has_open;
                if (used > (uint32_t)(WK_EV - 2)) break;
                float this_tmin = 0.f, this_tmax = 0.f;
                int32_t level = 0;
                bool found = false;
                if (FUSED) {
                    found = f_pending; f_pending = false;
                    this_tmin = f_tmin; this_tmax = f_tmax;
                } else {
                    const uint8_t *hits = a.hits + tid * G;
                    const float *ts = a.t_sorted + tid * 2 * G;
                    const int64_t *ti = a.t_indices + tid * 2 * G;
                    while (!found && next_i < 2 * G - 1) {
                        const int32_t i = next_i++;
                        const int64_t idx = ti[i];
                        level = event_level(idx, G);
                        if ((uint32_t)level >= (uint32_t)G || !hits[level]) continue;
                        if (!(idx < G)) {
                            const int64_t nidx = ti[i + 1];
                            if (nidx < G) continue;
                            level = event_level(nidx, G);
                            if ((uint32_t)level >= (uint32_t)G || !hits[level]) continue;
                        }
                        this_tmin = fmaxf(ts[i], near_plane); this_tmax = fminf(ts[i + 1], far_plane);
                        if (this_tmin >= this_tmax) continue;
                        found = true;
                    }
                }
                if (!found) { finished = 1; break; }
                uint32_t kk = used;
                *reinterpret_cast<float *>(col + (kk << WK_LG)) = this_tmin;
                *reinterpret_cast<float *>(col + ((kk + 1u) << WK_LG)) = this_tmax;
                ev_span |= 1u << kk;
                walk_span_setup(a, p.lay, o, d, level, this_tmin, this_tmax, sp);
                const uint32_t idx0 = sp.widx ^ sp.flip;
                w_p = bits[idx0 >> 5]; i_p = idx0;
                open_type = (int32_t)((w_p >> (idx0 & 31u)) & 1u);
                ev_span |= (uint32_t)open_type << (16u + kk);
                ev_addr = ((kk + 2u) << WK_LG) | lane_off;
                has_open = 1;
                in_span = 1;
                __builtin_amdgcn_s_waitcnt(0xC07F);
                m_p = dda_step_reg_end(sp.dx, sp.dy, sp.dz, sp.mx, sp.my, sp.mz, sp.tx, sp.ty, sp.tz, sp.end, sp.widx, sp.over);
                walk_request(sp.widx, sp.flip, bits, i_q, w_q);
                par = 0;
            }
            float tx = sp.tx, ty = sp.ty, tz = sp.tz;
            const uint32_t flip = sp.flip;
            uint32_t over = sp.over;
            uint32_t widx = sp.widx;
            __builtin_amdgcn_s_waitcnt(0x0070);
            if (over != 0u) {
                bool go = true;
                if (par) {
                    m_p = dda_step_reg_end(sp.dx, sp.dy, sp.dz, sp.mx, sp.my, sp.mz, tx, ty, tz, sp.end, widx, over);
                    walk_arrived(w_q, over);
                    walk_record(m_q, w_q, i_q, open_type, ev_addr, ev_lds);
                    walk_request(widx, flip, bits, i_q, w_q);
                    par = 0;
                    go = !walk_stop(over, ev_addr);
                }
                if (go) for (;;) {
                    m_q = dda_step_reg_end(sp.dx, sp.dy, sp.dz, sp.mx, sp.my, sp.mz, tx, ty, tz, sp.end, widx, over);
                    walk_arrived(w_p, over);
                    walk_record(m_p, w_p, i_p, open_type, ev_addr, ev_lds);
                    walk_request(widx, flip, bits, i_p, w_p);
                    if (walk_stop(over, ev_addr)) { par = 1; break; }
                    m_p = dda_step_reg_end(sp.dx, sp.dy, sp.dz, sp.mx, sp.my, sp.mz, tx, ty, tz, sp.end, widx, over);
                    walk_arrived(w_q, over);
                    walk_record(m_q, w_q, i_q, open_type, ev_addr, ev_lds);
                    walk_request(widx, flip, bits, i_q, w_q);
                    if (walk_stop(over, ev_addr)) break;
                }
                asm volatile("" : "+v"(par));
                m_last = par ? m_p : m_q;
            }
            walk_arrived_all(w_p, w_q);
            sp.tx = tx; sp.ty = ty; sp.tz = tz; sp.widx = widx; sp.over = over;
            if (ev_addr >= WK_FULL) break;
            m_last = par ? m_q : m_p;
            walk_record(m_last, par ? w_q : w_p, par ? i_q : i_p, open_type, ev_addr, ev_lds);
            in_span = 0;
        }
        int32_t cnt = (int32_t)(ev_addr >> WK_LG);
        if (finished && has_open) { cnt += 1; has_open = 0; }
        if (LATTICE) lattice_run<HAS_LIMIT>(ls, col, cnt, ev_span, dt * 0.5f, limit, p, lt, tid);
        else marcher_run<HAS_LIMIT>(s, col, cnt, ev_span, dt, limit, p, tb, tid);
        if (finished || (limit > 0 && (LATTICE ? ls.n_samples : s.n_samples) >= limit)) break;
        ev_span = 0u;
        ev_addr = lane_off;
        if (has_open) *reinterpret_cast<float *>(col) = m_last;
    }
    if (LATTICE) { out.t_last = lattice_value(lt, ls.jr); out.n_samples = ls.n_samples; out.n_chains = ls.n_chains; out.n_runs = ls.n_runs; }
    else { out.t_last = s.t_last; out.n_samples = s.n_samples; out.n_chains = s.n_chains; out.n_runs = s.n_runs; }
}

template <bool FUSED, bool HAS_LIMIT, bool LATTICE>
__device__ __forceinline__ void walk_body(const nfa_traverse_args &a, const WalkParams &p)
{
    __shared__ __attribute__((aligned(16))) char ev_lds[(WK_EV + 1) << WK_LG];
    __shared__ ApproachLds tb;
    __shared__ LatticeLds lt;
    if (LATTICE) lattice_to_lds(lt);
    else approach_to_lds(tb);
    __syncthreads();
    const uint32_t lane_off = 4u * threadIdx.x;
    const int32_t steps_limit = (HAS_LIMIT && a.steps_limit_dev) ? *a.steps_limit_dev : a.traverse_steps_limit;
    if (HAS_LIMIT && steps_limit <= 0) return;
    int64_t n_walk = p.order ? p.n_order : a.n_rays;
    if (p.order && a.n_listed_dev) n_walk = min(n_walk, *a.n_listed_dev);
    const int64_t bid = xcd_fair_block(blockIdx.x, gridDim.x);
    for (int64_t slot_i = bid * blockDim.x + threadIdx.x; slot_i < n_walk;
         slot_i += (int64_t)blockDim.x * gridDim.x) {
        const int64_t tid = p.order ? (int64_t)p.order[slot_i] : slot_i;
        if (a.mode == 2 && a.rays_mask != nullptr && !a.rays_mask[tid]) {
            if (a.terminate_planes) a.terminate_planes[tid] = a.near_planes[tid];
            a.sm_cnts[tid] = 0;
            if (a.iv_cnts) a.iv_cnts[tid] = 0;
            p.run_cnts[tid] = 0;
            continue;
        }
        WalkOut s;
        walk_ray<FUSED, HAS_LIMIT, LATTICE>(a, p, tid, ev_lds, lane_off, tb, lt, steps_limit, s);
        if (a.terminate_planes) a.terminate_planes[tid] = s.t_last;
        a.sm_cnts[tid] = s.n_samples;
        if (a.iv_cnts) a.iv_cnts[tid] = s.n_samples + s.n_chains;
        int32_t n_runs = s.n_runs;
        if (s.n_samples > (1 << 21) && n_runs <= p.max_runs) n_runs = p.max_runs + 1;
        p.run_cnts[tid] = n_runs;
        if (n_runs > p.max_runs) atomicAdd(p.overflow, 1);
    }
}
template <bool FUSED, bool HAS_LIMIT>
__attribute__((amdgpu_waves_per_eu(WK_WAVES, WK_WAVES))) __global__ __launch_bounds__(WK_THREADS) void walk_lattice_kernel(const nfa_traverse_args a, const WalkParams p)
{
    walk_body<FUSED, HAS_LIMIT, true>(a, p);
}
template <bool FUSED, bool HAS_LIMIT>
__global__ __launch_bounds__(WK_THREADS) void walk_kernel(const nfa_traverse_args a, const WalkParams p)
{
    walk_body<FUSED, HAS_LIMIT, false>(a, p);
}

struct ConeParams {
    const uint32_t *bits;
    WalkLayout lay;
    RunOut ro;
    int32_t chunk, min_busy;
    char *tab_lds;
    uint4 *arena;
    int32_t arena_cap;
    int32_t *arena_count;
};
constexpr uint32_t CONE_ARENA_BLOCK = 16u;
constexpr uint32_t CONE_ARENA_NONE = 0xFFFFFFFFu;
constexpr uint32_t CONE_ARENA_FRESH = 0xFFFFFFFEu;
struct ConeRay {
    float t_last;
    int32_t continuous, n_samples, n_runs, run_len;
};

__device__ __forceinline__ void cone_span_begin(const nfa_traverse_args &a, const ConeParams &p, const float o[3], const float d[3],
                                                int32_t level, float this_tmin, float this_tmax, ConeRay &st, WalkSpan &sp,
                                                unsigned long long &w_cur, uint32_t &i_cur)
{
    if (!st.continuous) st.t_last = fast_forward(st.t_last, this_tmin, a.step_size, a.cone_angle);
    walk_span_setup(a, p.lay, o, d, level, this_tmin, this_tmax, sp);
    dda_table_write(p.tab_lds, sp);
    i_cur = sp.widx ^ sp.flip;
    w_cur = reinterpret_cast<const unsigned long long *>(p.bits)[i_cur >> 6];
}

template <bool SPLIT>
__device__ __forceinline__ bool cone_cell(const nfa_traverse_args &a, const ConeParams &p, int64_t tid, float this_tmax, WalkSpan &sp,
                                          unsigned long long &w_cur, uint32_t &i_cur, ConeRay &st, uint32_t *arena_slot )
{
    const int32_t limit = a.traverse_steps_limit;
    const uint32_t w_half = (i_cur & 32u) ? (uint32_t)(w_cur >> 32) : (uint32_t)w_cur;
    const bool occupied = __builtin_amdgcn_ubfe(w_half, i_cur, 1u) != 0u;
    const uint32_t tab_x = 16u * threadIdx.x;
    float m;
    bool done;
    if constexpr (SPLIT) {
        m = dda_step_lds(p.tab_lds, tab_x, tab_x + 2u * WK_TAB_AXIS, sp.tx, sp.ty, sp.tz, sp.rem, sp.widx);
        done = (sp.rem & WK_GUARD) != WK_GUARD;
    } else {
        m = dda_step_lds_end(p.tab_lds, tab_x, tab_x + 2u * WK_TAB_AXIS, sp.tx, sp.ty, sp.tz, sp.end, sp.widx, sp.over);
        done = sp.over == 0u;
    }
    const float t_traverse = vmin_f32(m, this_tmax);
    const uint32_t i_next = sp.widx ^ sp.flip;
    const bool fetch = !done && ((i_next ^ i_cur) >> 6) != 0u;
    unsigned long long w_next = 0ull;
    if (fetch) w_next = reinterpret_cast<const unsigned long long *>(p.bits)[i_next >> 6];

    auto emit = [&](float) {
        const bool cut = !st.continuous || st.run_len == CONE_RUN_CAP;
        if (cut) {
            const unsigned long long rec = run_record(st.t_last, st.n_samples, st.continuous);
            const int32_t inl = p.arena ? p.ro.max_runs - 1 : p.ro.max_runs;
            if (st.n_runs < inl) {
                p.ro.runs[(int64_t)st.n_runs * a.n_rays + tid] = rec;
            } else if (p.arena) {
                uint32_t e = *arena_slot;
                if (st.n_runs == inl) {
                    p.ro.runs[(int64_t)inl * a.n_rays + tid] = 0x7FC00000ull | ((unsigned long long)(uint32_t)st.n_samples << 32);
                    e = CONE_ARENA_FRESH;
                } else if (e < CONE_ARENA_NONE) {
                    reinterpret_cast<uint32_t *>(p.arena + e)[3] = (uint32_t)st.run_len;
                }
                if (e != CONE_ARENA_NONE) {
                    e = (e == CONE_ARENA_FRESH || ((e + 1u) & (CONE_ARENA_BLOCK - 1u)) == 0u) ? (uint32_t)atomicAdd(p.arena_count, (int32_t)CONE_ARENA_BLOCK)
                                                                                             : e + 1u;
                    if (e + CONE_ARENA_BLOCK <= (uint32_t)p.arena_cap || (e & (CONE_ARENA_BLOCK - 1u)) != 0u)
                        p.arena[e] = make_uint4((uint32_t)rec, (uint32_t)(rec >> 32), (uint32_t)tid, 0u);
                    else
                        e = CONE_ARENA_NONE;
                }
                *arena_slot = e;
            }
            st.n_runs++;
        }
        st.run_len = cut ? 1 : st.run_len + 1;
    };
    march_cell<SPLIT>(st.t_last, st.continuous, st.n_samples, occupied, t_traverse, a.step_size, a.cone_angle, limit, emit);
    i_cur = i_next;
    w_cur = fetch ? w_next : w_cur;
    return done || (limit > 0 && st.n_samples >= limit);
}

constexpr int CONE_EV_MAX = 8;
struct EventsStaged {
    uint32_t ti_pack, hit_mask;
    float *ts_col;
    __device__ __forceinline__ void stage(const nfa_traverse_args &a, int64_t tid)
    {
        const int32_t G = a.n_grids;
        const EventsInMemory e(a, tid);
        uint32_t pk = 0u, hm = 0u;
#pragma unroll
        for (int i = 0; i < CONE_EV_MAX; ++i)
            if (i < 2 * G) {
                const int64_t v = e.ti[i];
                pk |= ((uint64_t)v < (uint64_t)(2 * G) ? (uint32_t)v : 15u) << (4 * i);
                ts_col[i * CONE_THREADS] = e.ts[i];
            }
#pragma unroll
        for (int g = 0; g < CONE_EV_MAX / 2; ++g)
            if (g < G) hm |= (e.hits[g] != 0 ? 1u : 0u) << g;
        ti_pack = pk; hit_mask = hm;
    }
    __device__ __forceinline__ int32_t index(int32_t i) const { return (int32_t)((ti_pack >> (4 * i)) & 15u); }
    __device__ __forceinline__ float t(int32_t i) const { return ts_col[i * CONE_THREADS]; }
    __device__ __forceinline__ bool hit(int32_t level) const { return ((hit_mask >> level) & 1u) != 0u; }
};

template <bool FUSED>
__device__ __forceinline__ bool cone_next_span(const nfa_traverse_args &a, const ConeParams &p, int64_t tid, const EventsStaged *staged,
                                               const float o[3], const float d[3], float near_plane, float far_plane, int32_t &ev,
                                               ConeRay &st, WalkSpan &sp, float &span_tmax, unsigned long long &w_cur, uint32_t &i_cur)
{
    int32_t level = 0;
    float this_tmin, this_tmax;
    bool found;
    if (FUSED) {
        if (ev != 0) return false;
        ev = 1;
        const float inv[3] = {1.0f / d[0], 1.0f / d[1], 1.0f / d[2]};
        float lo, hi;
        found = true;
        const float *bmin = a.aabbs, *bmax = a.aabbs + 3;
        if (inv[0] >= 0) { this_tmin = (bmin[0] - o[0]) * inv[0]; this_tmax = (bmax[0] - o[0]) * inv[0]; }
        else             { this_tmin = (bmax[0] - o[0]) * inv[0]; this_tmax = (bmin[0] - o[0]) * inv[0]; }
#pragma unroll
        for (int ax = 1; ax < 3; ++ax) {
            if (inv[ax] >= 0) { lo = (bmin[ax] - o[ax]) * inv[ax]; hi = (bmax[ax] - o[ax]) * inv[ax]; }
            else              { lo = (bmax[ax] - o[ax]) * inv[ax]; hi = (bmin[ax] - o[ax]) * inv[ax]; }
            if (this_tmin > hi || lo > this_tmax) found = false;
            if (lo > this_tmin) this_tmin = lo;
            if (hi < this_tmax) this_tmax = hi;
        }
        if (this_tmax <= 0) found = false;
        this_tmin = fmaxf(this_tmin, near_plane); this_tmax = fminf(this_tmax, far_plane);
        found = found && this_tmin < this_tmax;
    } else if (staged) {
        found = next_event_span(*staged, a.n_grids, near_plane, far_plane, ev, level, this_tmin, this_tmax);
    } else {
        found = next_event_span(EventsInMemory(a, tid), a.n_grids, near_plane, far_plane, ev, level, this_tmin, this_tmax);
    }
    if (!found) return false;
    span_tmax = this_tmax;
    cone_span_begin(a, p, o, d, level, this_tmin, this_tmax, st, sp, w_cur, i_cur);
    return true;
}

__device__ __forceinline__ void cone_ray_out(const nfa_traverse_args &a, const ConeParams &p, int64_t tid, const ConeRay &st,
                                             const uint32_t *arena_slot)
{
    int32_t n_runs = st.n_runs;
    if (p.arena && n_runs >= p.ro.max_runs) {
        const uint32_t e = *arena_slot;
        if (e < CONE_ARENA_FRESH) { reinterpret_cast<uint32_t *>(p.arena + e)[3] = (uint32_t)st.run_len; n_runs = p.ro.max_runs; }
        else n_runs = p.ro.max_runs + 1;
    }
    run_ray_close(a, p.ro, tid, st.t_last, st.n_samples, n_runs);
}

constexpr int CONE_WALK_WAVES = 6;
template <bool FUSED>
__attribute__((amdgpu_waves_per_eu(CONE_WALK_WAVES, CONE_WALK_WAVES)))
__global__ __launch_bounds__(CONE_THREADS) void cone_walk_kernel(const nfa_traverse_args a, const ConeParams p_in)
{
    __shared__ __attribute__((aligned(16))) char s_tab[3 * WK_TAB_AXIS];
    ConeParams p = p_in;
    p.tab_lds = s_tab;
    __shared__ uint32_t s_arena[CONE_THREADS];
    uint32_t *const arena_slot = s_arena + threadIdx.x;
    const int64_t n_walk = p.ro.order ? p.ro.n_order : a.n_rays;
    const int32_t limit = a.traverse_steps_limit;
    for (int64_t slot_i = xcd_fair_block(blockIdx.x, gridDim.x) * blockDim.x + threadIdx.x; slot_i < n_walk;
         slot_i += (int64_t)blockDim.x * gridDim.x) {
        const int64_t tid = p.ro.order ? (int64_t)p.ro.order[slot_i] : slot_i;
        if (ray_masked(a, p.ro, tid)) continue;
        float near_plane, far_plane, o[3], d[3];
        const bool ray_ok = ray_load(a, tid, near_plane, far_plane, o, d);
        ConeRay st;
        st.t_last = near_plane; st.continuous = 0; st.n_samples = 0; st.n_runs = 0; st.run_len = 0;
        int32_t ev = ray_ok ? 0 : 2 * a.n_grids;
        WalkSpan sp;
        float span_tmax = 0.f;
        unsigned long long w_cur = 0ull;
        uint32_t i_cur = 0u;
        while (cone_next_span<FUSED>(a, p, tid, nullptr, o, d, near_plane, far_plane, ev, st, sp, span_tmax, w_cur, i_cur)) {
            while (!cone_cell<false>(a, p, tid, span_tmax, sp, w_cur, i_cur, st, arena_slot)) {}
            if (limit > 0 && st.n_samples >= limit) break;
        }
        cone_ray_out(a, p, tid, st, arena_slot);
    }
}

template <bool FUSED, bool STAGED >
struct ConeWalker {
    const nfa_traverse_args &a;
    const ConeParams &p;
    uint32_t *arena_slot;
    EventsStaged staged;
    int64_t tid;
    int32_t ev;
    float near_plane, far_plane, span_tmax, o[3], d[3];
    ConeRay st;
    WalkSpan sp;
    unsigned long long w_cur;
    uint32_t i_cur;
    __device__ __forceinline__ bool take(int64_t ray)
    {
        tid = ray;
        if (ray_masked(a, p.ro, tid)) return false;
        const bool ray_ok = ray_load(a, tid, near_plane, far_plane, o, d);
        if (STAGED) staged.stage(a, tid);
        st.t_last = near_plane; st.continuous = 0; st.n_samples = 0; st.n_runs = 0; st.run_len = 0;
        ev = ray_ok ? 0 : 2 * a.n_grids;
        return true;
    }
    __device__ __forceinline__ bool next_span()
    {
        return cone_next_span<FUSED>(a, p, tid, STAGED ? &staged : nullptr, o, d, near_plane, far_plane, ev, st, sp, span_tmax, w_cur, i_cur);
    }
    __device__ __forceinline__ int cell()
    {
        if (!cone_cell<true>(a, p, tid, span_tmax, sp, w_cur, i_cur, st, arena_slot)) return RF_WALK;
        return (a.traverse_steps_limit > 0 && st.n_samples >= a.traverse_steps_limit) ? RF_FINISH : RF_SPAN;
    }
    __device__ __forceinline__ void finish() { cone_ray_out(a, p, tid, st, arena_slot); }
};
template <bool FUSED, bool STAGED>
__global__ __launch_bounds__(CONE_THREADS) void cone_refill_kernel(const nfa_traverse_args a, const ConeParams p_in)
{
    static_assert(!(FUSED && STAGED), "a fused walk has no event list");
    __shared__ __attribute__((aligned(16))) char s_tab[3 * WK_TAB_AXIS];
    ConeParams p = p_in;
    p.tab_lds = s_tab;
    __shared__ float ts_lds[STAGED ? CONE_EV_MAX * CONE_THREADS : 1];
    __shared__ uint32_t s_arena[CONE_THREADS];
    ConeWalker<FUSED, STAGED> w{a, p, s_arena + threadIdx.x, {0u, 0u, ts_lds + (STAGED ? threadIdx.x : 0)}};
    refill_schedule(w, p.ro.order, p.ro.order ? p.ro.n_order : a.n_rays,
                    xcd_fair_block(blockIdx.x, gridDim.x) * (blockDim.x >> 6) + (threadIdx.x >> 6), p.chunk, p.min_busy);
}


}

using namespace nfa;

extern "C" {

int64_t nfa_walk_bits_words(int32_t n_grids, const int32_t *res)
{
    const WalkLayout L = walk_layout(res);
    return (((int64_t)n_grids << L.bits) + 31) / 32;
}

int nfa_pack_walk_bits(const uint8_t *binaries, int32_t n_grids, const int32_t *res, uint32_t *bits, nfa_stream_t stream)
{
    NFA_REQUIRE(binaries && res && bits && n_grids >= 1, "pack_walk_bits: bad arguments");
    NFA_REQUIRE(res[0] > 0 && res[1] > 0 && res[2] > 0 && res[0] <= WK_MAX_RES && res[1] <= WK_MAX_RES && res[2] <= WK_MAX_RES,
                "pack_walk_bits: 1..512 cells per axis");
    const WalkLayout L = walk_layout(res);
    NFA_REQUIRE(L.bits >= 5 && ((int64_t)n_grids << L.bits) < ((int64_t)1 << 31), "pack_walk_bits: grid too large");
    const int64_t n_words = ((int64_t)n_grids << L.bits) >> 5;
    hipLaunchKernelGGL(pack_walk_bits_kernel, dim3(grid_1d(n_words, 256)), dim3(256), 0, as_stream(stream), binaries, n_grids, res[0],
                       res[1], res[2], L, bits);
    NFA_CHECK_LAUNCH("pack_walk_bits");
    return NFA_OK;
}

int nfa_traverse_runs(const nfa_traverse_args *pa, const uint32_t *bits, int32_t *run_cnts, uint64_t *runs, int32_t max_runs,
                      int32_t *overflow_count, float near_hint, const int32_t *ray_order, int64_t n_order, nfa_stream_t stream)
{
    NFA_REQUIRE(pa != nullptr, "traverse_runs: null args");
    const nfa_traverse_args &a = *pa;
    NFA_REQUIRE(a.n_rays >= 0 && a.n_rays < (int64_t)1 << 31, "traverse_runs: n_rays out of range");
    NFA_REQUIRE(overflow_count, "traverse_runs: overflow_count is null");
    hipStream_t s = as_stream(stream);
    if (!a.steps_limit_dev && hipMemsetAsync(overflow_count, 0, 2 * sizeof(int32_t), s) != hipSuccess) { set_error("traverse_runs: memset failed"); return NFA_EHIP; }
    if (a.n_rays == 0) return NFA_OK;
    NFA_REQUIRE(a.step_size > 0.0f && a.cone_angle == 0.0f, "traverse_runs: needs step_size > 0 and cone_angle == 0");
    NFA_REQUIRE(a.mode == 0 || a.mode == 2, "traverse_runs: mode must be 0 (all rays) or 2 (rays_mask + limit)");
    NFA_REQUIRE(a.mode != 2 || a.traverse_steps_limit > 0, "traverse_steps_limit must be > 0 when over_allocate is true");
    NFA_REQUIRE(a.rays_o && a.rays_d && a.aabbs && a.near_planes && a.far_planes && a.sm_cnts && bits && run_cnts && runs,
                "traverse_runs: null pointer");
    NFA_REQUIRE(max_runs >= 1 && max_runs <= 32, "traverse_runs: max_runs must be in [1, 32]");
    NFA_REQUIRE(a.n_grids >= 1 && a.res[0] > 0 && a.res[1] > 0 && a.res[2] > 0, "traverse_runs: bad grid shape");
    NFA_REQUIRE(a.res[0] <= WK_MAX_RES && a.res[1] <= WK_MAX_RES && a.res[2] <= WK_MAX_RES,
                "traverse_runs: at most 512 cells per axis (use nfa_traverse_grids beyond)");
    const bool fused = !a.t_sorted && !a.t_indices && !a.hits;
    NFA_REQUIRE(fused || (a.t_sorted && a.t_indices && a.hits), "traverse_runs: t_sorted, t_indices and hits must be given together");
    NFA_REQUIRE(!fused || a.n_grids == 1, "traverse_runs: in-kernel intersection supports one grid");
    WalkParams p;
    p.bits = bits;
    p.lay = walk_layout(a.res);
    NFA_REQUIRE(p.lay.bits >= 5 && ((int64_t)a.n_grids << p.lay.bits) < ((int64_t)1 << 31), "traverse_runs: grid too large");
    p.run_cnts = run_cnts;
    p.runs = reinterpret_cast<unsigned long long *>(runs);
    p.max_runs = max_runs;
    p.n_rays = a.n_rays;
    p.overflow = overflow_count;
    p.order = ray_order;
    p.n_order = ray_order ? n_order : a.n_rays;
    NFA_REQUIRE(!ray_order || (n_order >= 0 && n_order <= a.n_rays), "traverse_runs: n_order out of range");
    if (ray_order && n_order == 0) return NFA_OK;
    p.approach.n = 0;
    p.lat.n_rows = 0;
    if (near_hint == near_hint && !tuning_env("NFA_WALK_NO_LATTICE")) lattice_table_build(p.lat, near_hint, a.step_size);
    const bool lattice = p.lat.n_rows >= 1 && p.lat.n_binades >= 1;
    if (!lattice && near_hint == near_hint) approach_table_build(p.approach, near_hint, a.step_size);
    const size_t shmem = 0;
    const unsigned grid = grid_1d(p.n_order, WK_THREADS, 1 << 20);
    const bool lim = a.traverse_steps_limit > 0;
    static constexpr decltype(&walk_kernel<false, false>) kernels[2][2][2] = {
        {{walk_lattice_kernel<true, false>, walk_lattice_kernel<true, true>}, {walk_lattice_kernel<false, false>, walk_lattice_kernel<false, true>}},
        {{walk_kernel<true, false>, walk_kernel<true, true>}, {walk_kernel<false, false>, walk_kernel<false, true>}}};
    hipLaunchKernelGGL(kernels[!lattice][!fused][lim], dim3(grid), dim3(WK_THREADS), shmem, s, a, p);
    NFA_CHECK_LAUNCH("traverse_runs");
    return NFA_OK;
}

__global__ __launch_bounds__(256) void expand_cone_arena_kernel(const uint4 *__restrict__ arena, int32_t n_entries, float step, float cone,
                                                                const longlong2 *__restrict__ packed_info, float *__restrict__ t_starts,
                                                                float *__restrict__ t_ends, int64_t *__restrict__ ray_indices)
{
    const int32_t e = (int32_t)(blockIdx.x * 4u + (threadIdx.x >> 6));
    if (e >= n_entries) return;
    const uint4 rec = arena[e];
    const uint32_t i = threadIdx.x & 63u;
    if (i >= rec.w) return;
    float t = bits_f32(rec.x);
    for (uint32_t k = 0; k < i; ++k) t = t + calc_dt(t, cone, step);
    const int64_t at = packed_info[rec.z].x + (int64_t)(rec.y & 0x7FFFFFFFu) + i;
    t_starts[at] = t;
    t_ends[at] = t + calc_dt(t, cone, step);
    ray_indices[at] = (int64_t)rec.z;
}

int nfa_expand_cone_arena(const uint32_t *arena, int32_t n_entries, float step_size, float cone_angle, const int64_t *packed_info,
                          float *t_starts, float *t_ends, int64_t *ray_indices, nfa_stream_t stream)
{
    NFA_REQUIRE(n_entries >= 0, "expand_cone_arena: negative n_entries");
    if (n_entries == 0) return NFA_OK;
    NFA_REQUIRE(arena && packed_info && t_starts && t_ends && ray_indices, "expand_cone_arena: null pointer");
    NFA_REQUIRE(step_size > 0.0f && cone_angle > 0.0f, "expand_cone_arena: step_size and cone_angle must be > 0");
    hipLaunchKernelGGL(expand_cone_arena_kernel, dim3((unsigned)((n_entries + 3) / 4)), dim3(256), 0, as_stream(stream),
                       reinterpret_cast<const uint4 *>(arena), n_entries, step_size, cone_angle, reinterpret_cast<const longlong2 *>(packed_info),
                       t_starts, t_ends, ray_indices);
    NFA_CHECK_LAUNCH("expand_cone_arena");
    return NFA_OK;
}

int nfa_traverse_cone_walk(const nfa_traverse_args *pa, const uint32_t *bits, int32_t *run_cnts, uint64_t *runs, int32_t max_runs,
                           int32_t *overflow_count, uint32_t *arena, int32_t arena_capacity, const int32_t *ray_order, int64_t n_order,
                           nfa_stream_t stream)
{
    NFA_REQUIRE(pa != nullptr, "traverse_cone_walk: null args");
    const nfa_traverse_args &a = *pa;
    NFA_REQUIRE(a.n_rays >= 0 && a.n_rays < (int64_t)1 << 31, "traverse_cone_walk: n_rays out of range");
    NFA_REQUIRE(overflow_count, "traverse_cone_walk: overflow_count is null");
    hipStream_t s = as_stream(stream);
    if (hipMemsetAsync(overflow_count, 0, 2 * sizeof(int32_t), s) != hipSuccess) { set_error("traverse_cone_walk: memset failed"); return NFA_EHIP; }
    NFA_REQUIRE(arena_capacity >= 0 && (arena == nullptr || arena_capacity % (int32_t)CONE_ARENA_BLOCK == 0), "traverse_cone_walk: arena_capacity must be a multiple of 16");
    if (a.n_rays == 0) return NFA_OK;
    NFA_REQUIRE(a.step_size > 0.0f && a.cone_angle > 0.0f, "traverse_cone_walk: needs step_size > 0 and cone_angle > 0");
    NFA_REQUIRE(a.mode == 0 || a.mode == 2, "traverse_cone_walk: mode must be 0 (all rays) or 2 (rays_mask + traverse_steps_limit)");
    NFA_REQUIRE(a.mode != 2 || a.traverse_steps_limit > 0, "traverse_steps_limit must be > 0 when over_allocate is true");
    NFA_REQUIRE(a.rays_o && a.rays_d && a.aabbs && a.near_planes && a.far_planes && a.sm_cnts && !a.iv_cnts && bits && run_cnts && runs,
                "traverse_cone_walk: null pointer (or interval outputs requested)");
    NFA_REQUIRE(max_runs >= 1 && max_runs <= 32, "traverse_cone_walk: max_runs must be in [1, 32]");
    NFA_REQUIRE(a.n_grids >= 1 && a.res[0] > 0 && a.res[1] > 0 && a.res[2] > 0, "traverse_cone_walk: bad grid shape");
    NFA_REQUIRE(a.res[0] <= WK_MAX_RES && a.res[1] <= WK_MAX_RES && a.res[2] <= WK_MAX_RES,
                "traverse_cone_walk: at most 512 cells per axis (use nfa_traverse_cone_runs beyond)");
    const bool fused = !a.t_sorted && !a.t_indices && !a.hits;
    NFA_REQUIRE(fused || (a.t_sorted && a.t_indices && a.hits), "traverse_cone_walk: t_sorted, t_indices and hits must be given together");
    NFA_REQUIRE(!fused || a.n_grids == 1, "traverse_cone_walk: in-kernel intersection supports one grid");
    ConeParams p;
    p.bits = bits;
    p.lay = walk_layout(a.res);
    NFA_REQUIRE(p.lay.bits >= 6 && ((int64_t)a.n_grids << p.lay.bits) < ((int64_t)1 << 31),
                "traverse_cone_walk: a level of the grid copy must be a whole number of 64-bit words (at least 4 cells per axis) and the copy below 2^31 bits");
    p.ro.run_cnts = run_cnts;
    p.ro.runs = reinterpret_cast<unsigned long long *>(runs);
    p.ro.max_runs = max_runs;
    p.ro.overflow = overflow_count;
    p.arena = (arena && arena_capacity > 0 && max_runs >= 2) ? reinterpret_cast<uint4 *>(arena) : nullptr;
    p.arena_cap = arena_capacity;
    p.arena_count = overflow_count + 1;
    p.ro.order = ray_order;
    p.ro.n_order = ray_order ? n_order : a.n_rays;
    NFA_REQUIRE(!ray_order || (n_order >= 0 && n_order <= a.n_rays), "traverse_cone_walk: n_order out of range");
    if (ray_order && n_order == 0) return NFA_OK;
    const RefillPlan plan = refill_plan(p.ro.n_order, a.traverse_steps_limit);
    p.chunk = (int32_t)plan.chunk; p.min_busy = plan.min_busy;
    if (plan.refill) {
        const unsigned grid = (unsigned)ceil_div64(ceil_div64(p.ro.n_order, plan.chunk), CONE_THREADS / 64);
        const char *staged_env = tuning_env("NFA_CONE_STAGED");
        const bool staged = !fused && 2 * a.n_grids <= CONE_EV_MAX && !(staged_env && staged_env[0] == '0');
        if (fused)       hipLaunchKernelGGL((cone_refill_kernel<true, false>), dim3(grid), dim3(CONE_THREADS), 0, s, a, p);
        else if (staged) hipLaunchKernelGGL((cone_refill_kernel<false, true>), dim3(grid), dim3(CONE_THREADS), 0, s, a, p);
        else             hipLaunchKernelGGL((cone_refill_kernel<false, false>), dim3(grid), dim3(CONE_THREADS), 0, s, a, p);
    } else {
        const unsigned grid = grid_1d(p.ro.n_order, CONE_THREADS, 1 << 20);
        if (fused) hipLaunchKernelGGL((cone_walk_kernel<true>), dim3(grid), dim3(CONE_THREADS), 0, s, a, p);
        else       hipLaunchKernelGGL((cone_walk_kernel<false>), dim3(grid), dim3(CONE_THREADS), 0, s, a, p);
    }
    NFA_CHECK_LAUNCH("traverse_cone_walk");
    return NFA_OK;
}

}
```

### nerfacc_amd/grid.py

```python
from __future__ import annotations

import ctypes as C
import os
from typing import Optional, Tuple

import torch
from torch import Tensor

from . import _backend as B
from ._segments import tag_const_step, tag_ray_indices, tag_trusted
from .data_specs import RayIntervals, RaySamples


@torch.no_grad()
def ray_aabb_intersect(
    rays_o: Tensor,
    rays_d: Tensor,
    aabbs: Tensor,
    near_plane: float = -float("inf"),
    far_plane: float = float("inf"),
    miss_value: float = float("inf"),
) -> Tuple[Tensor, Tensor, Tensor]:
    assert rays_o.ndim == 2 and rays_o.shape[-1] == 3
    assert rays_d.ndim == 2 and rays_d.shape[-1] == 3
    assert aabbs.ndim == 2 and aabbs.shape[-1] == 6
    dev = B.require_device(rays_o, rays_d, aabbs)
    rays_o, rays_d, aabbs = rays_o.float().contiguous(), rays_d.float().contiguous(), aabbs.float().contiguous()
    n, m = rays_o.shape[0], aabbs.shape[0]
    t_mins = torch.empty((n, m), dtype=torch.float32, device=dev)
    t_maxs = torch.empty((n, m), dtype=torch.float32, device=dev)
    hits = torch.empty((n, m), dtype=torch.bool, device=dev)
    with torch.cuda.device(dev):
        B.call("nfa_ray_aabb_intersect", B.ptr(rays_o), B.ptr(rays_d), n, B.ptr(aabbs), m, float(near_plane),
               float(far_plane), float(miss_value), B.ptr(t_mins), B.ptr(t_maxs), B.ptr(hits), B.stream())
    return t_mins, t_maxs, hits


def _traverse_args(rays_o, rays_d, rays_mask, binaries, aabbs, t_sorted, t_indices, hits, near_planes, far_planes,
                   step_size, cone_angle, limit, mode) -> B.TraverseArgs:
    a = B.TraverseArgs()
    a.n_rays = rays_o.shape[0]
    a.rays_o, a.rays_d, a.rays_mask = B.ptr(rays_o), B.ptr(rays_d), B.ptr(rays_mask)
    a.n_grids = binaries.shape[0]
    a.res[0], a.res[1], a.res[2] = binaries.shape[1], binaries.shape[2], binaries.shape[3]
    a.binaries, a.aabbs = B.ptr(binaries), B.ptr(aabbs)
    a.hits, a.t_sorted, a.t_indices = B.ptr(hits), B.ptr(t_sorted), B.ptr(t_indices)
    a.near_planes, a.far_planes = B.ptr(near_planes), B.ptr(far_planes)
    a.step_size, a.cone_angle = float(step_size), float(cone_angle)
    a.traverse_steps_limit, a.mode = int(limit), int(mode)
    bricks, coarse = _get_bricks(binaries)
    a._keepalive = (bricks, coarse)
    a.bricks, a.coarse = B.ptr(bricks), B.ptr(coarse)
    return a


def _launch(a: B.TraverseArgs) -> None:
    B.call("nfa_traverse_grids", C.byref(a), B.stream())


def _exclusive_cumsum(cnts: Tensor, total_out: Tensor):
    starts = torch.empty_like(cnts)
    scratch = B.cumsum_scratch(cnts.numel(), cnts.device)
    B.call("nfa_exclusive_cumsum_i64", B.ptr(cnts), cnts.numel(), B.ptr(starts), B.ptr(total_out), B.ptr(scratch),
           B.stream())
    return starts


def _cumsum_packed(cnts: Tensor, total_out: Tensor, stats: bool = False) -> Tensor:
    packed = torch.empty((cnts.numel(), 2), dtype=torch.int64, device=cnts.device)
    scratch = B.cumsum_scratch(cnts.numel(), cnts.device)
    B.call("nfa_exclusive_cumsum_pairs_stats_i64" if stats else "nfa_exclusive_cumsum_pairs_i64", B.ptr(cnts), cnts.numel(),
           B.ptr(packed), B.ptr(total_out), B.ptr(scratch), B.stream())
    return packed


MAX_EVENT_LEVELS = 8


def ray_events(rays_o: Tensor, rays_d: Tensor, aabbs: Tensor):
    G = aabbs.shape[0]
    if G > MAX_EVENT_LEVELS or not rays_o.is_cuda:
        t_mins, t_maxs, hits = ray_aabb_intersect(rays_o, rays_d, aabbs)
        t_sorted, t_indices = torch.sort(torch.cat([t_mins, t_maxs], dim=-1), dim=-1)
        return t_sorted, t_indices, hits
    dev = B.require_device(rays_o, rays_d, aabbs)
    rays_o, rays_d, aabbs = rays_o.float().contiguous(), rays_d.float().contiguous(), aabbs.float().contiguous()
    n = rays_o.shape[0]
    t_sorted = torch.empty((n, 2 * G), dtype=torch.float32, device=dev)
    t_indices = torch.empty((n, 2 * G), dtype=torch.int64, device=dev)
    hits = torch.empty((n, G), dtype=torch.bool, device=dev)
    with torch.cuda.device(dev):
        B.call("nfa_ray_events", B.ptr(rays_o), B.ptr(rays_d), n, B.ptr(aabbs), G, B.ptr(t_sorted), B.ptr(t_indices),
               B.ptr(hits), B.stream())
    return t_sorted, t_indices, hits


def _prepare(rays_o, rays_d, binaries, aabbs, near_planes, far_planes, rays_mask, t_sorted, t_indices, hits,
             allow_fused: bool):
    dev = B.require_device(rays_o, rays_d, binaries, aabbs)
    assert rays_o.ndim == 2 and rays_o.shape[-1] == 3 and rays_d.shape == rays_o.shape
    assert binaries.ndim == 4 and aabbs.ndim == 2 and aabbs.shape == (binaries.shape[0], 6)
    rays_o, rays_d, aabbs = rays_o.float().contiguous(), rays_d.float().contiguous(), aabbs.float().contiguous()
    binaries = (binaries if binaries.dtype == torch.bool else binaries.bool()).contiguous()
    n_rays = rays_o.shape[0]
    if near_planes is None:
        near_planes = torch.zeros(n_rays, dtype=torch.float32, device=dev)
    if far_planes is None:
        far_planes = torch.full((n_rays,), float("inf"), dtype=torch.float32, device=dev)
    near_planes, far_planes = near_planes.float().contiguous(), far_planes.float().contiguous()
    if rays_mask is not None:
        rays_mask = rays_mask.bool().contiguous()
    if t_sorted is None or t_indices is None or hits is None:
        if allow_fused and binaries.shape[0] == 1:
            t_sorted = t_indices = hits = None
        else:
            t_sorted, t_indices, hits = ray_events(rays_o, rays_d, aabbs)
    if t_sorted is not None:
        t_sorted = t_sorted.float().contiguous()
        t_indices = t_indices.to(torch.int64).contiguous()
        hits = hits.bool().contiguous()
    return dev, rays_o, rays_d, binaries, aabbs, near_planes, far_planes, rays_mask, t_sorted, t_indices, hits


@torch.no_grad()
def traverse_grids(
    rays_o: Tensor,
    rays_d: Tensor,
    binaries: Tensor,
    aabbs: Tensor,
    near_planes: Optional[Tensor] = None,
    far_planes: Optional[Tensor] = None,
    step_size: Optional[float] = 1e-3,
    cone_angle: Optional[float] = 0.0,
    traverse_steps_limit: Optional[int] = None,
    over_allocate: Optional[bool] = False,
    rays_mask: Optional[Tensor] = None,
    t_sorted: Optional[Tensor] = None,
    t_indices: Optional[Tensor] = None,
    hits: Optional[Tensor] = None,
) -> Tuple[RayIntervals, RaySamples, Tensor]:
    near_hint = 0.0 if near_planes is None else None
    if traverse_steps_limit is None:
        traverse_steps_limit = -1
    if over_allocate:
        assert traverse_steps_limit > 0, "traverse_steps_limit must be set if over_allocate is True."
    (dev, rays_o, rays_d, binaries, aabbs, near_planes, far_planes, rays_mask, t_sorted, t_indices,
     hits) = _prepare(rays_o, rays_d, binaries, aabbs, near_planes, far_planes, rays_mask, t_sorted, t_indices, hits,
                      allow_fused=True)
    n_rays = rays_o.shape[0]
    i64 = dict(dtype=torch.int64, device=dev)
    with torch.cuda.device(dev):
        terminate = torch.empty(n_rays, dtype=torch.float32, device=dev)
        totals = torch.empty(2, **i64)
        iv_packed = sm_packed = None
        if over_allocate:
            limit = int(traverse_steps_limit)
            mask_l = torch.ones(n_rays, **i64) if rays_mask is None else rays_mask.to(torch.int64)
            sm_alloc = mask_l * limit
            iv_alloc = sm_alloc * 2
            sm_off = torch.cumsum(sm_alloc, 0) - sm_alloc
            iv_off = sm_off * 2
            n_alive = int(mask_l.sum().item()) if rays_mask is not None else n_rays
            n_sm, n_iv = n_alive * limit, n_alive * limit * 2
            iv_cnts, sm_cnts = torch.empty(n_rays, **i64), torch.empty(n_rays, **i64)
            iv_vals = torch.zeros(n_iv, dtype=torch.float32, device=dev)
            iv_ri = torch.zeros(n_iv, **i64)
            iv_l = torch.zeros(n_iv, dtype=torch.bool, device=dev)
            iv_r = torch.zeros(n_iv, dtype=torch.bool, device=dev)
            sm_vals = torch.zeros(n_sm, dtype=torch.float32, device=dev)
            sm_ri = torch.zeros(n_sm, **i64)
            sm_valid = torch.zeros(n_sm, dtype=torch.bool, device=dev)
            a = _traverse_args(rays_o, rays_d, rays_mask, binaries, aabbs, t_sorted, t_indices, hits, near_planes,
                               far_planes, step_size, cone_angle, limit, 2)
            a.iv_vals, a.iv_ray_indices, a.iv_is_left, a.iv_is_right = B.ptr(iv_vals), B.ptr(iv_ri), B.ptr(iv_l), B.ptr(iv_r)
            a.iv_starts, a.iv_cnts = B.ptr(iv_off), B.ptr(iv_cnts)
            a.sm_vals, a.sm_ray_indices, a.sm_is_valid = B.ptr(sm_vals), B.ptr(sm_ri), B.ptr(sm_valid)
            a.sm_starts, a.sm_cnts = B.ptr(sm_off), B.ptr(sm_cnts)
            a.terminate_planes = B.ptr(terminate)
            _launch(a)
            iv_starts = _exclusive_cumsum(iv_cnts, totals[0:1])
            sm_starts = _exclusive_cumsum(sm_cnts, totals[1:2])
        elif float(step_size) > 0.0 and float(cone_angle) == 0.0 and _walk_supported(binaries):
            iv_cnts, sm_cnts = torch.empty(n_rays, **i64), torch.empty(n_rays, **i64)
            meta = torch.zeros(3, **i64)
            a = _traverse_args(rays_o, rays_d, None, binaries, aabbs, t_sorted, t_indices, hits, near_planes,
                               far_planes, step_size, cone_angle, traverse_steps_limit, 0)
            a.iv_cnts, a.sm_cnts, a.terminate_planes = B.ptr(iv_cnts), B.ptr(sm_cnts), B.ptr(terminate)
            bits = _get_walk_bits(binaries)
            run_cnts = torch.empty(n_rays, dtype=torch.int32, device=dev)
            runs = torch.empty((MAX_RUNS, n_rays), dtype=torch.int64, device=dev)
            while True:
                B.call("nfa_traverse_runs", C.byref(a), B.ptr(bits), B.ptr(run_cnts), B.ptr(runs), MAX_RUNS,
                       B.ptr(meta[2:3]), float("nan") if near_hint is None else near_hint, None, 0, B.stream())
                iv_packed = _cumsum_packed(iv_cnts, meta[0:1])
                sm_packed = _cumsum_packed(sm_cnts, meta[1:2])
                n_iv, n_sm, n_overflow = (int(v) for v in meta.tolist())
                n_overflow, off_lattice = n_overflow & 0xFFFFFFFF, n_overflow >> 32
                if not off_lattice or near_hint is None:
                    break
                near_hint = None
                meta.zero_()
            iv_vals = torch.empty(n_iv, dtype=torch.float32, device=dev)
            iv_ri = torch.empty(n_iv, **i64)
            iv_l = torch.empty(n_iv, dtype=torch.bool, device=dev)
            iv_r = torch.empty(n_iv, dtype=torch.bool, device=dev)
            sm_vals = torch.empty(n_sm, dtype=torch.float32, device=dev)
            sm_ri = torch.empty(n_sm, **i64)
            sm_valid = torch.ones(n_sm, dtype=torch.bool, device=dev)
            if n_sm > 0:
                B.call("nfa_expand_runs", n_rays, float(step_size), B.ptr(run_cnts), B.ptr(runs), MAX_RUNS, B.ptr(sm_packed),
                       None, None, B.ptr(sm_vals), B.ptr(sm_ri), n_sm, B.stream())
                B.call("nfa_expand_intervals", n_rays, float(step_size), B.ptr(run_cnts), B.ptr(runs), MAX_RUNS,
                       B.ptr(iv_packed), B.ptr(iv_vals), B.ptr(iv_ri), B.ptr(iv_l), B.ptr(iv_r), B.stream())
                if n_overflow > 0:
                    iv_starts, sm_starts = iv_packed[:, 0].contiguous(), sm_packed[:, 0].contiguous()
                    a.mode = 1
                    a.terminate_planes = None
                    a.iv_vals, a.iv_ray_indices, a.iv_is_left, a.iv_is_right = (B.ptr(iv_vals), B.ptr(iv_ri), B.ptr(iv_l),
                                                                                 B.ptr(iv_r))
                    a.iv_starts = B.ptr(iv_starts)
                    a.sm_vals, a.sm_ray_indices, a.sm_is_valid = B.ptr(sm_vals), B.ptr(sm_ri), B.ptr(sm_valid)
                    a.sm_starts = B.ptr(sm_starts)
                    a.ray_filter, a.ray_filter_min = B.ptr(run_cnts), MAX_RUNS
                    _launch(a)
        else:
            iv_cnts, sm_cnts = torch.empty(n_rays, **i64), torch.empty(n_rays, **i64)
            a = _traverse_args(rays_o, rays_d, None, binaries, aabbs, t_sorted, t_indices, hits, near_planes,
                               far_planes, step_size, cone_angle, traverse_steps_limit, 0)
            a.iv_cnts, a.sm_cnts, a.terminate_planes = B.ptr(iv_cnts), B.ptr(sm_cnts), B.ptr(terminate)
            _launch(a)
            iv_starts = _exclusive_cumsum(iv_cnts, totals[0:1])
            sm_starts = _exclusive_cumsum(sm_cnts, totals[1:2])
            n_iv, n_sm = (int(v) for v in totals.tolist())
            iv_vals = torch.empty(n_iv, dtype=torch.float32, device=dev)
            iv_ri = torch.empty(n_iv, **i64)
            iv_l = torch.empty(n_iv, dtype=torch.bool, device=dev)
            iv_r = torch.empty(n_iv, dtype=torch.bool, device=dev)
            sm_vals = torch.empty(n_sm, dtype=torch.float32, device=dev)
            sm_ri = torch.empty(n_sm, **i64)
            sm_valid = torch.empty(n_sm, dtype=torch.bool, device=dev)
            if n_sm > 0:
                a.mode = 1
                a.terminate_planes = None
                a.iv_vals, a.iv_ray_indices, a.iv_is_left, a.iv_is_right = B.ptr(iv_vals), B.ptr(iv_ri), B.ptr(iv_l), B.ptr(iv_r)
                a.iv_starts = B.ptr(iv_starts)
                a.sm_vals, a.sm_ray_indices, a.sm_is_valid = B.ptr(sm_vals), B.ptr(sm_ri), B.ptr(sm_valid)
                a.sm_starts = B.ptr(sm_starts)
                _launch(a)
        if iv_packed is None:
            iv_packed = torch.stack([iv_starts, iv_cnts], dim=-1)
            sm_packed = torch.stack([sm_starts, sm_cnts], dim=-1)
    if not over_allocate:
        tag_trusted(iv_packed, n_iv)
        info = tag_trusted(sm_packed, n_sm)
        tag_ray_indices(sm_ri, n_rays, info)
    intervals = RayIntervals(vals=iv_vals, packed_info=iv_packed, ray_indices=iv_ri, is_left=iv_l, is_right=iv_r)
    samples = RaySamples(vals=sm_vals, packed_info=sm_packed, ray_indices=sm_ri, is_valid=sm_valid)
    return intervals, samples, terminate


MAX_RUNS = int(os.environ.get("NERFACC_AMD_MAX_RUNS", "32"))


def _get_bricks(binaries: Tensor):
    cached = getattr(binaries, "_nfa_bricks", None)
    if cached is not None and cached[0] == binaries._version:
        return cached[1], cached[2]
    dev = binaries.device
    res = (C.c_int32 * 3)(*binaries.shape[1:])
    words = int(B.load().nfa_bricks_words(binaries.shape[0], res))
    bricks = torch.empty(words, dtype=torch.int64, device=dev)
    coarse = torch.empty((words + 31) // 32, dtype=torch.int32, device=dev)
    B.call("nfa_pack_bricks", B.ptr(binaries), binaries.shape[0], res, B.ptr(bricks), B.ptr(coarse), B.stream())
    try:
        binaries._nfa_bricks = (binaries._version, bricks, coarse)
    except Exception:
        pass
    return bricks, coarse


WALK_MAX_RES = 512


def _walk_supported(binaries: Tensor) -> bool:
    if max(binaries.shape[1:]) > WALK_MAX_RES:
        return False
    res = (C.c_int32 * 3)(*binaries.shape[1:])
    return int(B.load().nfa_walk_bits_words(binaries.shape[0], res)) * 32 < (1 << 31)


def _get_walk_bits(binaries: Tensor) -> Tensor:
    cached = getattr(binaries, "_nfa_walk_bits", None)
    if cached is not None and cached[0] == binaries._version:
        return cached[1]
    res = (C.c_int32 * 3)(*binaries.shape[1:])
    words = int(B.load().nfa_walk_bits_words(binaries.shape[0], res))
    bits = torch.empty(words, dtype=torch.int32, device=binaries.device)
    B.call("nfa_pack_walk_bits", B.ptr(binaries), binaries.shape[0], res, B.ptr(bits), B.stream())
    try:
        binaries._nfa_walk_bits = (binaries._version, bits)
    except Exception:
        pass
    return bits


_SIDE_STREAMS: dict = {}


def _side_stream(dev) -> "torch.cuda.Stream":
    key = (dev.index, torch.cuda.current_stream(dev).cuda_stream)
    st = _SIDE_STREAMS.get(key)
    if st is None:
        st = _SIDE_STREAMS[key] = torch.cuda.Stream(device=dev)
    return st


SPECULATE = os.environ.get("NERFACC_AMD_SPECULATE", "1") != "0"
_SPEC_CAPACITY: dict = {}
_PINNED: dict = {}


def _pinned_meta(dev) -> Tensor:
    buf = _PINNED.get(dev.index)
    if buf is None:
        buf = _PINNED[dev.index] = torch.empty(8, dtype=torch.int64, pin_memory=True)
    return buf


CONE_RUNS = os.environ.get("NERFACC_AMD_CONE_RUNS", "1") != "0"
ALIVE_LIST_FRACTION = float(os.environ.get("NERFACC_AMD_ALIVE_FRACTION", "0.75"))
CONE_WALK = os.environ.get("NERFACC_AMD_CONE_WALK", "1") != "0"
CONE_ARENA = os.environ.get("NERFACC_AMD_CONE_ARENA", "1") != "0"
CONE_ARENA_MIN = 4096
CONE_BIN_THRESHOLD = 1.25


@torch.no_grad()
def _traverse_samples(rays_o, rays_d, binaries, aabbs, near_planes, far_planes, step_size, cone_angle,
                      rays_mask=None, traverse_steps_limit=None, t_sorted=None, t_indices=None, hits=None,
                      return_terminate=False, near_hint=None, bin_rays=False, stats_sink=None, speculate=True, n_alive=None,
                      alive_list=None):
    limit = -1 if traverse_steps_limit is None else int(traverse_steps_limit)
    use_runs = float(step_size) > 0.0 and float(cone_angle) == 0.0 and _walk_supported(binaries)
    use_cone_runs = CONE_RUNS and float(step_size) > 0.0 and float(cone_angle) > 0.0
    if (rays_mask is not None or limit > 0) and (not (use_runs or use_cone_runs) or (use_cone_runs and limit <= 0)):
        iv, sm, term = traverse_grids(rays_o, rays_d, binaries, aabbs, near_planes, far_planes, step_size, cone_angle,
                                      limit if limit > 0 else None, limit > 0, rays_mask, t_sorted, t_indices, hits)
        valid = sm.is_valid if sm.is_valid is not None else torch.ones_like(sm.ray_indices, dtype=torch.bool)
        out = (sm.ray_indices[valid], iv.vals[iv.is_left], iv.vals[iv.is_right], sm.packed_info)
        return (*out, term) if return_terminate else out
    (dev, rays_o, rays_d, binaries, aabbs, near_planes, far_planes, rays_mask, t_sorted, t_indices,
     hits) = _prepare(rays_o, rays_d, binaries, aabbs, near_planes, far_planes, rays_mask, t_sorted, t_indices, hits,
                      allow_fused=True)
    n_rays = rays_o.shape[0]
    with torch.cuda.device(dev):
        masked = rays_mask is not None or limit > 0
        spec_key = (n_rays, dev.index)
        binned = bool(bin_rays) and n_rays >= 4096
        alive = None
        if (alive_list is not None and n_alive is not None and rays_mask is not None and (use_runs or use_cone_runs) and not binned
                and 0 <= n_alive <= alive_list.numel() and alive_list.dtype == torch.int32 and alive_list.device == dev):
            alive = alive_list[:int(n_alive)]
            sm_cnts = torch.zeros(n_rays, dtype=torch.int64, device=dev)
            terminate = near_planes.clone() if return_terminate else None
        elif (rays_mask is not None and n_alive is not None and (use_runs or use_cone_runs) and not binned
                and 0 <= n_alive and n_alive < ALIVE_LIST_FRACTION * n_rays):
            alive = torch.nonzero_static(rays_mask, size=int(n_alive)).view(-1).to(torch.int32)
            sm_cnts = torch.zeros(n_rays, dtype=torch.int64, device=dev)
            terminate = near_planes.clone() if return_terminate else None
        else:
            sm_cnts = torch.empty(n_rays, dtype=torch.int64, device=dev)
            terminate = torch.empty(n_rays, dtype=torch.float32, device=dev) if return_terminate else None
        meta = torch.zeros(6, dtype=torch.int64, device=dev)
        a = _traverse_args(rays_o, rays_d, rays_mask, binaries, aabbs, t_sorted, t_indices, hits, near_planes, far_planes,
                           step_size, cone_angle, limit, 2 if ((use_runs or use_cone_runs) and masked) else 0)
        a.sm_cnts = B.ptr(sm_cnts)
        a.terminate_planes = B.ptr(terminate)
        if use_runs:
            bits = _get_walk_bits(binaries)
            run_cnts = (torch.zeros if alive is not None else torch.empty)(n_rays, dtype=torch.int32, device=dev)
            runs = torch.empty((MAX_RUNS, n_rays), dtype=torch.int64, device=dev)
            order = alive
            if binned:
                order = torch.empty(n_rays, dtype=torch.int32, device=dev)
                scratch = torch.empty(1024 + n_rays, dtype=torch.uint8, device=dev)
                B.call("nfa_bin_rays", B.ptr(rays_o), B.ptr(rays_d), n_rays, B.ptr(aabbs[-1]), B.ptr(order), B.ptr(scratch),
                       B.stream())
            B.call("nfa_traverse_runs", C.byref(a), B.ptr(bits), B.ptr(run_cnts), B.ptr(runs), MAX_RUNS,
                   B.ptr(meta[3:4]), float("nan") if near_hint is None else float(near_hint), B.ptr(order),
                   0 if order is None else order.numel(), B.stream())
        elif use_cone_runs:
            _get_bricks(binaries)
            arena, arena_cap = None, 0
            run_cnts = (torch.zeros if alive is not None else torch.empty)(n_rays, dtype=torch.int32, device=dev)
            runs = torch.empty((MAX_RUNS, n_rays), dtype=torch.int64, device=dev)
            order = alive
            if binned or (bin_rays is None and n_rays >= 65536 and alive is None and limit <= 0):
                order = torch.empty(n_rays, dtype=torch.int32, device=dev)
                scratch = torch.empty(1024 + n_rays, dtype=torch.uint8, device=dev)
                res3 = (C.c_int32 * 3)(*binaries.shape[1:])
                B.call("nfa_bin_rays_levels", B.ptr(rays_o), B.ptr(rays_d), n_rays, B.ptr(aabbs), binaries.shape[0], res3,
                       float(near_hint) if near_hint is not None else 0.0, B.ptr(order), B.ptr(scratch), B.ptr(meta[4:6]), B.stream())
                if not binned and not (stats_sink is not None and stats_sink.get("cells_max_over_mean", 1.0) > CONE_BIN_THRESHOLD):
                    order = None
            if CONE_WALK and _walk_supported(binaries) and min(binaries.shape[1:]) >= 4:
                arena_cap = CONE_ARENA and max(CONE_ARENA_MIN, (n_rays // 8 + 15) // 16 * 16)
                arena = torch.zeros(2 * arena_cap, dtype=torch.int64, device=dev) if arena_cap else None
                B.call("nfa_traverse_cone_walk", C.byref(a), B.ptr(_get_walk_bits(binaries)), B.ptr(run_cnts), B.ptr(runs), MAX_RUNS,
                       B.ptr(meta[3:4]), B.ptr(arena), arena_cap, B.ptr(order), 0 if order is None else order.numel(), B.stream())
            else:
                B.call("nfa_traverse_cone_runs", C.byref(a), B.ptr(run_cnts), B.ptr(runs), MAX_RUNS, B.ptr(meta[3:4]), B.ptr(order),
                       0 if order is None else order.numel(), B.stream())
        else:
            _launch(a)
        packed_info = _cumsum_packed(sm_cnts, meta[0:3], stats=True)
        cap = _SPEC_CAPACITY.get(spec_key, 0) if (SPECULATE and speculate and use_runs) else 0
        t_starts = t_ends = ray_indices = None
        if cap > 0:
            host = _pinned_meta(dev)
            main = torch.cuda.current_stream()
            ready = torch.cuda.Event(); ready.record(main)
            side = _side_stream(dev)
            with torch.cuda.stream(side):
                side.wait_event(ready)
                host[:6].copy_(meta, non_blocking=True)
                done = torch.cuda.Event(); done.record(side)
            t_starts = torch.empty(cap, dtype=torch.float32, device=dev)
            t_ends = torch.empty(cap, dtype=torch.float32, device=dev)
            ray_indices = torch.empty(cap, dtype=torch.int64, device=dev)
            B.call("nfa_expand_runs", n_rays, float(step_size), B.ptr(run_cnts), B.ptr(runs), MAX_RUNS,
                   B.ptr(packed_info), B.ptr(t_starts), B.ptr(t_ends), None, B.ptr(ray_indices), cap, B.stream())
            done.synchronize()
            n_sm, s_max, s_sum, n_overflow, c_max, c_sum = (int(v) for v in host[:6].tolist())
        else:
            n_sm, s_max, s_sum, n_overflow, c_max, c_sum = (int(v) for v in meta.tolist())
        n_overflow, off_lattice = n_overflow & 0xFFFFFFFF, n_overflow >> 32
        n_arena = 0
        if use_cone_runs and arena is not None:
            n_arena, off_lattice = min(off_lattice, arena_cap), 0
        if off_lattice and use_runs and near_hint is not None:
            return _traverse_samples(rays_o, rays_d, binaries, aabbs, near_planes, far_planes, step_size, cone_angle,
                                     rays_mask=rays_mask, traverse_steps_limit=traverse_steps_limit, t_sorted=t_sorted,
                                     t_indices=t_indices, hits=hits, return_terminate=return_terminate, near_hint=None,
                                     bin_rays=bin_rays, stats_sink=stats_sink, speculate=speculate, n_alive=n_alive,
                                     alive_list=alive_list)
        if stats_sink is not None and c_sum > 0:
            stats_sink["cells_max_over_mean"] = 64.0 * c_max / c_sum
        if SPECULATE and use_runs:
            _SPEC_CAPACITY[spec_key] = ((int(n_sm * 1.03) + 4096) // 4096) * 4096
        if stats_sink is not None and s_sum > 0:
            stats_sink["max_over_mean"] = 64.0 * s_max / s_sum
        expanded = cap > 0 and n_sm <= cap
        if expanded:
            t_starts, t_ends, ray_indices = t_starts[:n_sm], t_ends[:n_sm], ray_indices[:n_sm]
        else:
            t_starts = torch.empty(n_sm, dtype=torch.float32, device=dev)
            t_ends = torch.empty(n_sm, dtype=torch.float32, device=dev)
            ray_indices = torch.empty(n_sm, dtype=torch.int64, device=dev)
        if n_sm > 0:
            main = torch.cuda.current_stream()
            joined = None
            if (use_runs or use_cone_runs) and n_overflow > 0:
                sm_starts = packed_info[:, 0].contiguous()
                side = _side_stream(dev)
                side.wait_stream(main)
                with torch.cuda.stream(side):
                    a.mode = 1
                    a.terminate_planes = None
                    a.sm_starts = B.ptr(sm_starts)
                    a.sm_t_starts, a.sm_t_ends, a.sm_ray_indices = B.ptr(t_starts), B.ptr(t_ends), B.ptr(ray_indices)
                    a.ray_filter, a.ray_filter_min = B.ptr(run_cnts), MAX_RUNS
                    _launch(a)
                    joined = torch.cuda.Event()
                    joined.record(side)
            if use_runs and not expanded:
                B.call("nfa_expand_runs", n_rays, float(step_size), B.ptr(run_cnts), B.ptr(runs), MAX_RUNS,
                       B.ptr(packed_info), B.ptr(t_starts), B.ptr(t_ends), None, B.ptr(ray_indices), n_sm, B.stream())
            elif use_cone_runs:
                B.call("nfa_expand_cone_runs", n_rays, float(step_size), float(cone_angle), B.ptr(run_cnts), B.ptr(runs),
                       MAX_RUNS, B.ptr(packed_info), B.ptr(t_starts), B.ptr(t_ends), B.ptr(ray_indices), B.stream())
                if n_arena > 0:
                    B.call("nfa_expand_cone_arena", B.ptr(arena), n_arena, float(step_size), float(cone_angle), B.ptr(packed_info),
                           B.ptr(t_starts), B.ptr(t_ends), B.ptr(ray_indices), B.stream())
            if joined is not None:
                main.wait_event(joined)
            if not (use_runs or use_cone_runs):
                a.mode = 1
                a.terminate_planes = None
                sm_starts = packed_info[:, 0].contiguous()
                a.sm_starts = B.ptr(sm_starts)
                a.sm_t_starts, a.sm_t_ends = B.ptr(t_starts), B.ptr(t_ends)
                a.sm_ray_indices = None
                _launch(a)
                B.call("nfa_fill_ray_indices", n_rays, B.ptr(packed_info), B.ptr(ray_indices), B.stream())
    info = tag_trusted(packed_info, n_sm)
    tag_ray_indices(ray_indices, n_rays, info)
    if use_runs and not masked:
        tag_const_step(t_starts, t_ends, step_size)
    out = (ray_indices, t_starts, t_ends, packed_info)
    return (*out, terminate) if return_terminate else out


def _enlarge_aabb(aabb: Tensor, factor: float) -> Tensor:
    center = (aabb[:3] + aabb[3:]) / 2
    extent = (aabb[3:] - aabb[:3]) / 2
    return torch.cat([center - extent * factor, center + extent * factor])


def _query(x: Tensor, data: Tensor, base_aabb: Tensor) -> Tuple[Tensor, Tensor]:
    lo, hi = base_aabb[:3], base_aabb[3:]
    u = (x - lo) / (hi - lo)
    r = (u - 0.5).abs().amax(dim=-1).clamp_min(0.1)
    mip = (torch.frexp(r)[1].long() + 1).clamp_min(0)
    inside = mip < data.shape[0]
    uu = (u - 0.5) / (2 ** mip)[:, None] + 0.5
    res = torch.tensor(data.shape[1:], device=x.device)
    ix = torch.minimum((uu * res).long(), res - 1)
    lvl = mip.clamp_max(data.shape[0] - 1)
    return data[lvl, ix[:, 0], ix[:, 1], ix[:, 2]] * inside, inside
```

Measured before the change: 724.7 million rays/s.

## Fuse cumsum block partials into walk kernel and emit segment tiles during scan

The ray-walk kernel now reduces per-wavefront sample counts with DPP and atomically accumulates them into per-scan-block partials held in a 'book' buffer. This lets the exclusive cumsum skip its partials pass. The final cumsum kernel also writes the segment tile table (row/element start per tile) used by later segmented scans, so that table need not be built separately. The cost is a larger memset of the book buffer, extra atomics in the walk, and more complex tile-validity logic that falls back when the speculated capacity or tile size mismatches.

```diff
diff --git a/include/nerfacc_hip.h b/include/nerfacc_hip.h
--- a/include/nerfacc_hip.h
+++ b/include/nerfacc_hip.h
@@ -33,6 +33,10 @@
                                    void *scratch, nfa_stream_t stream);
 int nfa_exclusive_cumsum_pairs_stats_i64(const int64_t *cnts, int64_t n, int64_t *packed_info ,
                                          int64_t *total_and_stats , void *scratch, nfa_stream_t stream);
+int nfa_exclusive_cumsum_pairs_tiles_i64(const int64_t *cnts, int64_t n, int64_t *packed_info ,
+                                         int64_t *total_and_stats , void *scratch, int partials_filled,
+                                         int64_t *tiles , int64_t tile_rows, int64_t tile_elems,
+                                         nfa_stream_t stream);
 
 int nfa_pack_info(const int64_t *ray_indices, int64_t n, int64_t n_rays, int64_t *packed_info ,
                   int32_t *flags , void *scratch, nfa_stream_t stream);
@@ -87,7 +91,13 @@
     const int32_t *steps_limit_dev;
     const int64_t *n_listed_dev;
     const int32_t *run_if_nonzero;
+    int64_t *book;
+    int64_t book_words;
 } nfa_traverse_args;
+#define NFA_SCAN_BLOCK 2048
+#define NFA_BOOK_OVERFLOW 3
+#define NFA_BOOK_PARTIALS 8
+int64_t nfa_book_words(int64_t n_rays);
 int nfa_traverse_grids(const nfa_traverse_args *args, nfa_stream_t stream);
 
 int64_t nfa_bricks_words(int32_t n_grids, const int32_t *res);
diff --git a/nerfacc_amd/_backend.py b/nerfacc_amd/_backend.py
--- a/nerfacc_amd/_backend.py
+++ b/nerfacc_amd/_backend.py
@@ -30,6 +30,7 @@
         ("ray_filter", _vp), ("ray_filter_min", _i32),
         ("bricks", _vp), ("coarse", _vp),
         ("steps_limit_dev", _vp), ("n_listed_dev", _vp), ("run_if_nonzero", _vp),
+        ("book", _vp), ("book_words", _i64),
     ]
 
 
@@ -55,6 +56,8 @@
     "nfa_exclusive_cumsum_i64": [_vp, _i64, _vp, _vp, _vp, _vp],
     "nfa_exclusive_cumsum_pairs_i64": [_vp, _i64, _vp, _vp, _vp, _vp],
     "nfa_exclusive_cumsum_pairs_stats_i64": [_vp, _i64, _vp, _vp, _vp, _vp],
+    "nfa_exclusive_cumsum_pairs_tiles_i64": [_vp, _i64, _vp, _vp, _vp, _int, _vp, _i64, _i64, _vp],
+    "nfa_book_words": [_i64],
     "nfa_pack_info": [_vp, _i64, _i64, _vp, _vp, _vp, _vp],
     "nfa_pdf_loss_fwd": [_vp, _vp, _vp, _vp, _i64, _i32, _i32, _f32, _vp, _vp, _vp],
     "nfa_pdf_loss_bwd": [_vp, _vp, _vp, _i64, _i32, _i32, _f32, _vp, _vp, _vp, _vp],
@@ -197,7 +200,7 @@
     "nfa_set_tuning": [C.c_char_p, C.c_char_p],
     "nfa_device_arch": [C.c_char_p, _int],
 }
-_RESTYPES = {"nfa_grid_rebinarize_scratch_bytes": _i64, "nfa_hashgrid_sorted_scratch_bytes": _i64, "nfa_hashgrid_sorted_scratch_bytes_d": _i64, "nfa_planereg_partials": _i64, "nfa_vmreg_partials": _i64, "nfa_bricks_words": _i64, "nfa_walk_bits_words": _i64, "nfa_pdf_loss_partials": _i64, "nfa_cumsum_scratch_bytes": _i64, "nfa_seg_table_rows": _i64, "nfa_seg_plan": None, "nfa_last_error": C.c_char_p}
+_RESTYPES = {"nfa_grid_rebinarize_scratch_bytes": _i64, "nfa_hashgrid_sorted_scratch_bytes": _i64, "nfa_hashgrid_sorted_scratch_bytes_d": _i64, "nfa_planereg_partials": _i64, "nfa_vmreg_partials": _i64, "nfa_bricks_words": _i64, "nfa_walk_bits_words": _i64, "nfa_pdf_loss_partials": _i64, "nfa_cumsum_scratch_bytes": _i64, "nfa_book_words": _i64, "nfa_seg_table_rows": _i64, "nfa_seg_plan": None, "nfa_last_error": C.c_char_p}
 
 EXPORTED_SYMBOLS = tuple(_SIGS)
 
@@ -302,3 +305,10 @@
 def cumsum_scratch(n: int, device) -> torch.Tensor:
     nbytes = ((max(n, 1) + 2047) // 2048 + 1) * 8
     return torch.empty(nbytes // 8, dtype=torch.int64, device=device)
+
+
+BOOK_OVERFLOW, BOOK_PARTIALS = 3, 8
+
+
+def walk_book(n_rays: int, device) -> torch.Tensor:
+    return torch.empty(BOOK_PARTIALS + ((max(n_rays, 1) + 2047) // 2048 + 8) // 8 * 8, dtype=torch.int64, device=device)
diff --git a/nerfacc_amd/_segments.py b/nerfacc_amd/_segments.py
--- a/nerfacc_amd/_segments.py
+++ b/nerfacc_amd/_segments.py
@@ -56,8 +56,13 @@
     return info
 
 
-def tag_trusted(packed_info: Tensor, n_elems: int) -> SegInfo:
-    return seginfo_from_packed(packed_info, n_elems, trusted=True)
+def tag_trusted(packed_info: Tensor, n_elems: int, tiles: Optional[Tensor] = None, n_tiles: int = 0) -> SegInfo:
+    if tiles is None:
+        return seginfo_from_packed(packed_info, n_elems, trusted=True)
+    n_rays = packed_info.shape[0]
+    info = SegInfo(packed_info, n_rays, n_elems, tiles, True, n_tiles=n_tiles, trusted=True)
+    setattr(packed_info, _ATTR, (packed_info._version, n_elems, info))
+    return info
 
 
 def pack_info_native(ray_indices: Tensor, n_rays: int):
diff --git a/nerfacc_amd/csrc/common.hip.h b/nerfacc_amd/csrc/common.hip.h
--- a/nerfacc_amd/csrc/common.hip.h
+++ b/nerfacc_amd/csrc/common.hip.h
@@ -49,6 +49,11 @@
     if (refill_env) { long c = 0; int m = 0; if (sscanf(refill_env, "%ld,%d", &c, &m) == 2 && c >= 64 && m >= 1 && m <= 64) { chunk = c / 64 * 64; min_busy = m; } }
     return RefillPlan{true, chunk, min_busy};
 }
+
+#ifndef NFA_SEG_TILE_ROWS
+#define NFA_SEG_TILE_ROWS 256
+#endif
+constexpr int64_t SEG_TILE_ROWS = NFA_SEG_TILE_ROWS;
 
 static inline hipStream_t as_stream(nfa_stream_t s) { return reinterpret_cast<hipStream_t>(s); }
 
diff --git a/nerfacc_amd/csrc/grid.hip b/nerfacc_amd/csrc/grid.hip
--- a/nerfacc_amd/csrc/grid.hip
+++ b/nerfacc_amd/csrc/grid.hip
@@ -428,13 +428,15 @@
     if (threadIdx.x == 0 && total) *total = carry;
 }
 
-template <bool SPINE>
+template <bool SPINE, bool TILES = false>
 __global__ __launch_bounds__(CS_THREADS) void cumsum_final_kernel(const int64_t *__restrict__ in, int64_t n,
                                                                    int64_t in_stride,
                                                                    const int64_t *__restrict__ partials,
                                                                    int64_t *__restrict__ out, int pairs,
                                                                    int64_t *__restrict__ total,
-                                                                   unsigned long long *__restrict__ stats = nullptr)
+                                                                   unsigned long long *__restrict__ stats = nullptr,
+                                                                   longlong2 *__restrict__ tiles = nullptr, int64_t tile_rows = 0,
+                                                                   int tile_shift = 0)
 {
     __shared__ int64_t lds[8];
     int64_t block_off = 0;
@@ -446,6 +448,8 @@
         block_off = partials[blockIdx.x];
     }
     const int64_t base = (int64_t)blockIdx.x * CS_BLOCK + (int64_t)threadIdx.x * CS_ITEMS;
+    int64_t cnt_before = 0;
+    if (TILES && base > 0 && base < n) cnt_before = in[(base - 1) * in_stride];
     int64_t v[CS_ITEMS];
     int64_t s = 0;
 #pragma unroll
@@ -466,29 +470,51 @@
         if (lane_id() == 0) atomicAdd(&stats[0], (unsigned long long)gm);
         if (threadIdx.x == 0) atomicAdd(&stats[1], (unsigned long long)tot);
     }
+    int64_t start_prev = run - cnt_before;
+    auto tile_rows_of = [&](int64_t r, int64_t e_first, int64_t b_hi) {
+        int64_t b = r == 0 ? 0 : (start_prev >> tile_shift) + (r - 1) / SEG_TILE_ROWS + 1;
+        if (b_hi >= tile_rows) b_hi = tile_rows - 1;
+        if (b < 0) b = 0;
+        for (; b <= b_hi; ++b) tiles[b] = make_longlong2(r, e_first);
+    };
 #pragma unroll
     for (int k = 0; k < CS_ITEMS; ++k) {
         if (base + k < n) {
             if (pairs) { out[2 * (base + k)] = run; out[2 * (base + k) + 1] = v[k]; }
             else out[base + k] = run;
+            if (TILES) {
+                tile_rows_of(base + k, run, (run >> tile_shift) + (base + k) / SEG_TILE_ROWS);
+                start_prev = run;
+            }
         }
         run += v[k];
     }
+    if (TILES && (n > 0 ? (base < n && n <= base + CS_ITEMS) : (blockIdx.x == 0 && threadIdx.x == 0)))
+        tile_rows_of(n, run, (run >> tile_shift) + n / SEG_TILE_ROWS + 1);
 }
 
 static int run_cumsum(const int64_t *in, int64_t n, int64_t in_stride, int64_t *out, int pairs, int64_t *total,
-                      void *scratch, hipStream_t s, unsigned long long *stats = nullptr)
+                      void *scratch, hipStream_t s, unsigned long long *stats = nullptr, bool partials_filled = false,
+                      longlong2 *tiles = nullptr, int64_t tile_rows = 0, int tile_shift = 0)
 {
     const int64_t n_blocks = ceil_div64(n > 0 ? n : 1, CS_BLOCK);
     int64_t *partials = reinterpret_cast<int64_t *>(scratch);
-    hipLaunchKernelGGL(cumsum_partials_kernel, dim3((unsigned)n_blocks), dim3(CS_THREADS), 0, s, in, n, in_stride, partials);
+    if (!partials_filled)
+        hipLaunchKernelGGL(cumsum_partials_kernel, dim3((unsigned)n_blocks), dim3(CS_THREADS), 0, s, in, n, in_stride, partials);
+    const dim3 grid((unsigned)n_blocks), block(CS_THREADS);
     if (n_blocks <= 2048) {
-        hipLaunchKernelGGL(cumsum_final_kernel<true>, dim3((unsigned)n_blocks), dim3(CS_THREADS), 0, s, in, n, in_stride, partials,
-                           out, pairs, total, stats);
+        if (tiles)
+            hipLaunchKernelGGL((cumsum_final_kernel<true, true>), grid, block, 0, s, in, n, in_stride, partials, out, pairs, total, stats,
+                               tiles, tile_rows, tile_shift);
+        else
+            hipLaunchKernelGGL(cumsum_final_kernel<true>, grid, block, 0, s, in, n, in_stride, partials, out, pairs, total, stats);
     } else {
         hipLaunchKernelGGL(cumsum_spine_kernel, dim3(1), dim3(CS_THREADS), 0, s, partials, n_blocks, total);
-        hipLaunchKernelGGL(cumsum_final_kernel<false>, dim3((unsigned)n_blocks), dim3(CS_THREADS), 0, s, in, n, in_stride, partials,
-                           out, pairs, nullptr, nullptr);
+        if (tiles)
+            hipLaunchKernelGGL((cumsum_final_kernel<false, true>), grid, block, 0, s, in, n, in_stride, partials, out, pairs, nullptr,
+                               nullptr, tiles, tile_rows, tile_shift);
+        else
+            hipLaunchKernelGGL(cumsum_final_kernel<false>, grid, block, 0, s, in, n, in_stride, partials, out, pairs, nullptr, nullptr);
     }
     NFA_CHECK_LAUNCH("exclusive_cumsum_i64");
     return NFA_OK;
@@ -594,6 +620,27 @@
                 "exclusive_cumsum_pairs_stats_i64: bad arguments");
     return run_cumsum(cnts, n, 1, packed_info, 1, total_and_stats, scratch, as_stream(stream),
                       reinterpret_cast<unsigned long long *>(total_and_stats + 1));
+}
+
+static_assert(CS_BLOCK == NFA_SCAN_BLOCK, "the block a partial sums is the header's");
+int64_t nfa_book_words(int64_t n_rays) { return NFA_BOOK_PARTIALS + (ceil_div64(n_rays > 0 ? n_rays : 1, CS_BLOCK) + 8) / 8 * 8; }
+
+int nfa_exclusive_cumsum_pairs_tiles_i64(const int64_t *cnts, int64_t n, int64_t *packed_info, int64_t *total_and_stats,
+                                         void *scratch, int partials_filled, int64_t *tiles, int64_t tile_rows,
+                                         int64_t tile_elems, nfa_stream_t stream)
+{
+    NFA_REQUIRE(n >= 0 && scratch && total_and_stats && (n == 0 || (cnts && packed_info)),
+                "exclusive_cumsum_pairs_tiles_i64: bad arguments");
+    int shift = 0;
+    if (tiles) {
+        NFA_REQUIRE(n < ((int64_t)1 << 31) - 64, "exclusive_cumsum_pairs_tiles_i64: too many rays");
+        NFA_REQUIRE(tile_rows >= 1 && tile_elems >= 64 && (tile_elems & (tile_elems - 1)) == 0,
+                    "exclusive_cumsum_pairs_tiles_i64: tile_rows must be >= 1 and tile_elems a power of two >= 64");
+        while (((int64_t)1 << shift) < tile_elems) ++shift;
+    }
+    return run_cumsum(cnts, n, 1, packed_info, 1, total_and_stats, scratch, as_stream(stream),
+                      reinterpret_cast<unsigned long long *>(total_and_stats + 1), partials_filled != 0,
+                      reinterpret_cast<longlong2 *>(tiles), tile_rows, shift);
 }
 
 int nfa_pack_info(const int64_t *ray_indices, int64_t n, int64_t n_rays, int64_t *packed_info, int32_t *flags,
diff --git a/nerfacc_amd/csrc/segscan.hip b/nerfacc_amd/csrc/segscan.hip
--- a/nerfacc_amd/csrc/segscan.hip
+++ b/nerfacc_amd/csrc/segscan.hip
@@ -8,10 +8,6 @@
 constexpr int SE = 4;
 constexpr int SQ = SE / 4;
 constexpr int SEG_CHUNK = 64 * SE;
-#ifndef NFA_SEG_TILE_ROWS
-#define NFA_SEG_TILE_ROWS 256
-#endif
-constexpr int64_t SEG_TILE_ROWS = NFA_SEG_TILE_ROWS;
 #ifndef NFA_VIS_EXP_FREE
 #define NFA_VIS_EXP_FREE 1
 #endif
diff --git a/nerfacc_amd/csrc/walk.hip b/nerfacc_amd/csrc/walk.hip
--- a/nerfacc_amd/csrc/walk.hip
+++ b/nerfacc_amd/csrc/walk.hip
@@ -43,6 +43,7 @@
     int32_t *overflow;
     const int32_t *order;
     int64_t n_order;
+    unsigned long long *partials;
     ApproachTable approach;
     LatticeTable lat;
 };
@@ -766,25 +767,43 @@
     int64_t n_walk = p.order ? p.n_order : a.n_rays;
     if (p.order && a.n_listed_dev) n_walk = min(n_walk, *a.n_listed_dev);
     const int64_t bid = xcd_fair_block(blockIdx.x, gridDim.x);
-    for (int64_t slot_i = bid * blockDim.x + threadIdx.x; slot_i < n_walk;
-         slot_i += (int64_t)blockDim.x * gridDim.x) {
-        const int64_t tid = p.order ? (int64_t)p.order[slot_i] : slot_i;
-        if (a.mode == 2 && a.rays_mask != nullptr && !a.rays_mask[tid]) {
-            if (a.terminate_planes) a.terminate_planes[tid] = a.near_planes[tid];
-            a.sm_cnts[tid] = 0;
-            if (a.iv_cnts) a.iv_cnts[tid] = 0;
-            p.run_cnts[tid] = 0;
-            continue;
-        }
-        WalkOut s;
-        walk_ray<FUSED, HAS_LIMIT, LATTICE>(a, p, tid, ev_lds, lane_off, tb, lt, steps_limit, s);
-        if (a.terminate_planes) a.terminate_planes[tid] = s.t_last;
-        a.sm_cnts[tid] = s.n_samples;
-        if (a.iv_cnts) a.iv_cnts[tid] = s.n_samples + s.n_chains;
-        int32_t n_runs = s.n_runs;
-        if (s.n_samples > (1 << 21) && n_runs <= p.max_runs) n_runs = p.max_runs + 1;
-        p.run_cnts[tid] = n_runs;
-        if (n_runs > p.max_runs) atomicAdd(p.overflow, 1);
+    const uint32_t lane = threadIdx.x & 63u;
+    for (int64_t slot_w = bid * blockDim.x + (int64_t)(__builtin_amdgcn_readfirstlane((int32_t)threadIdx.x) & ~63); slot_w < n_walk;
+         slot_w += (int64_t)blockDim.x * gridDim.x) {
+        const int64_t slot_i = slot_w + lane;
+        int32_t n_here = 0;
+        if (slot_i < n_walk) {
+            const int64_t tid = p.order ? (int64_t)p.order[slot_i] : slot_i;
+            if (a.mode == 2 && a.rays_mask != nullptr && !a.rays_mask[tid]) {
+                if (a.terminate_planes) a.terminate_planes[tid] = a.near_planes[tid];
+                a.sm_cnts[tid] = 0;
+                if (a.iv_cnts) a.iv_cnts[tid] = 0;
+                p.run_cnts[tid] = 0;
+            } else {
+                WalkOut s;
+                walk_ray<FUSED, HAS_LIMIT, LATTICE>(a, p, tid, ev_lds, lane_off, tb, lt, steps_limit, s);
+                if (a.terminate_planes) a.terminate_planes[tid] = s.t_last;
+                a.sm_cnts[tid] = s.n_samples;
+                n_here = s.n_samples;
+                if (a.iv_cnts) a.iv_cnts[tid] = s.n_samples + s.n_chains;
+                int32_t n_runs = s.n_runs;
+                if (s.n_samples > (1 << 21) && n_runs <= p.max_runs) n_runs = p.max_runs + 1;
+                p.run_cnts[tid] = n_runs;
+                if (n_runs > p.max_runs) atomicAdd(p.overflow, 1);
+            }
+        }
+        if (p.partials) {
+            unsigned long long *const slot = &p.partials[slot_w / NFA_SCAN_BLOCK];
+            if (__ballot(n_here >= (1 << 25)) == 0ull) {
+                int32_t v = n_here;
+                v += dpp_step<0>(0, v); v += dpp_step<1>(0, v); v += dpp_step<2>(0, v);
+                v += dpp_step<3>(0, v); v += dpp_step<4>(0, v); v += dpp_step<5>(0, v);
+                const uint32_t tot = (uint32_t)__builtin_amdgcn_readlane(v, 63);
+                if (lane == 0u && tot != 0u) atomicAdd(slot, (unsigned long long)tot);
+            } else if (n_here > 0) {
+                atomicAdd(slot, (unsigned long long)n_here);
+            }
+        }
     }
 }
 template <bool FUSED, bool HAS_LIMIT>
@@ -1078,7 +1097,14 @@
     NFA_REQUIRE(a.n_rays >= 0 && a.n_rays < (int64_t)1 << 31, "traverse_runs: n_rays out of range");
     NFA_REQUIRE(overflow_count, "traverse_runs: overflow_count is null");
     hipStream_t s = as_stream(stream);
-    if (!a.steps_limit_dev && hipMemsetAsync(overflow_count, 0, 2 * sizeof(int32_t), s) != hipSuccess) { set_error("traverse_runs: memset failed"); return NFA_EHIP; }
+    if (a.book) {
+        NFA_REQUIRE(!a.steps_limit_dev, "traverse_runs: args->book is not for device-driven calls");
+        NFA_REQUIRE(a.book_words >= nfa_book_words(a.n_rays),
+                    "traverse_runs: args->book_words is below nfa_book_words(n_rays)");
+        NFA_REQUIRE(overflow_count == reinterpret_cast<int32_t *>(a.book + NFA_BOOK_OVERFLOW),
+                    "traverse_runs: overflow_count must be args->book + NFA_BOOK_OVERFLOW");
+        if (hipMemsetAsync(a.book, 0, (size_t)a.book_words * sizeof(int64_t), s) != hipSuccess) { set_error("traverse_runs: memset failed"); return NFA_EHIP; }
+    } else if (!a.steps_limit_dev && hipMemsetAsync(overflow_count, 0, 2 * sizeof(int32_t), s) != hipSuccess) { set_error("traverse_runs: memset failed"); return NFA_EHIP; }
     if (a.n_rays == 0) return NFA_OK;
     NFA_REQUIRE(a.step_size > 0.0f && a.cone_angle == 0.0f, "traverse_runs: needs step_size > 0 and cone_angle == 0");
     NFA_REQUIRE(a.mode == 0 || a.mode == 2, "traverse_runs: mode must be 0 (all rays) or 2 (rays_mask + limit)");
@@ -1102,6 +1128,7 @@
     p.n_rays = a.n_rays;
     p.overflow = overflow_count;
     p.order = ray_order;
+    p.partials = (a.book && !ray_order) ? reinterpret_cast<unsigned long long *>(a.book + NFA_BOOK_PARTIALS) : nullptr;
     p.n_order = ray_order ? n_order : a.n_rays;
     NFA_REQUIRE(!ray_order || (n_order >= 0 && n_order <= a.n_rays), "traverse_runs: n_order out of range");
     if (ray_order && n_order == 0) return NFA_OK;
diff --git a/nerfacc_amd/grid.py b/nerfacc_amd/grid.py
--- a/nerfacc_amd/grid.py
+++ b/nerfacc_amd/grid.py
@@ -72,6 +72,21 @@
     B.call("nfa_exclusive_cumsum_pairs_stats_i64" if stats else "nfa_exclusive_cumsum_pairs_i64", B.ptr(cnts), cnts.numel(),
            B.ptr(packed), B.ptr(total_out), B.ptr(scratch), B.stream())
     return packed
+
+
+def _cumsum_packed_tiles(cnts: Tensor, book: Tensor, filled: bool, capacity: int):
+    n = cnts.numel()
+    packed = torch.empty((n, 2), dtype=torch.int64, device=cnts.device)
+    tiles, rows, tile_elems = None, 0, 0
+    if capacity > 0:
+        tile_elems, n_tiles = B.seg_plan(capacity, n)
+        if tile_elems >= 64 and tile_elems & (tile_elems - 1) == 0:
+            rows = int(B.load().nfa_seg_table_rows(n_tiles))
+            tiles = torch.empty((rows, 2), dtype=torch.int64, device=cnts.device)
+    B.call_group("nfa_exclusive_cumsum_pairs_stats_i64", lambda: B.call(
+        "nfa_exclusive_cumsum_pairs_tiles_i64", B.ptr(cnts), n, B.ptr(packed), B.ptr(book), B.ptr(book[B.BOOK_PARTIALS:]),
+        int(filled), B.ptr(tiles), rows, tile_elems, B.stream()))
+    return packed, tiles, tile_elems
 
 
 MAX_EVENT_LEVELS = 8
@@ -339,7 +354,7 @@
 def _traverse_samples(rays_o, rays_d, binaries, aabbs, near_planes, far_planes, step_size, cone_angle,
                       rays_mask=None, traverse_steps_limit=None, t_sorted=None, t_indices=None, hits=None,
                       return_terminate=False, near_hint=None, bin_rays=False, stats_sink=None, speculate=True, n_alive=None,
-                      alive_list=None):
+                      alive_list=None, _book=True):
     limit = -1 if traverse_steps_limit is None else int(traverse_steps_limit)
     use_runs = float(step_size) > 0.0 and float(cone_angle) == 0.0 and _walk_supported(binaries)
     use_cone_runs = CONE_RUNS and float(step_size) > 0.0 and float(cone_angle) > 0.0
@@ -371,9 +386,12 @@
         else:
             sm_cnts = torch.empty(n_rays, dtype=torch.int64, device=dev)
             terminate = torch.empty(n_rays, dtype=torch.float32, device=dev) if return_terminate else None
-        meta = torch.zeros(6, dtype=torch.int64, device=dev)
+        book = B.walk_book(n_rays, dev) if (use_runs and _book) else None
+        meta = book[:6] if book is not None else torch.zeros(6, dtype=torch.int64, device=dev)
         a = _traverse_args(rays_o, rays_d, rays_mask, binaries, aabbs, t_sorted, t_indices, hits, near_planes, far_planes,
                            step_size, cone_angle, limit, 2 if ((use_runs or use_cone_runs) and masked) else 0)
+        if book is not None:
+            a.book, a.book_words = B.ptr(book), book.numel()
         a.sm_cnts = B.ptr(sm_cnts)
         a.terminate_planes = B.ptr(terminate)
         if use_runs:
@@ -413,8 +431,12 @@
                        0 if order is None else order.numel(), B.stream())
         else:
             _launch(a)
-        packed_info = _cumsum_packed(sm_cnts, meta[0:3], stats=True)
         cap = _SPEC_CAPACITY.get(spec_key, 0) if (SPECULATE and speculate and use_runs) else 0
+        tiles = None
+        if book is not None:
+            packed_info, tiles, tile_elems = _cumsum_packed_tiles(sm_cnts, book, order is None, cap)
+        else:
+            packed_info = _cumsum_packed(sm_cnts, meta[0:3], stats=True)
         t_starts = t_ends = ray_indices = None
         if cap > 0:
             host = _pinned_meta(dev)
@@ -443,7 +465,7 @@
                                      rays_mask=rays_mask, traverse_steps_limit=traverse_steps_limit, t_sorted=t_sorted,
                                      t_indices=t_indices, hits=hits, return_terminate=return_terminate, near_hint=None,
                                      bin_rays=bin_rays, stats_sink=stats_sink, speculate=speculate, n_alive=n_alive,
-                                     alive_list=alive_list)
+                                     alive_list=alive_list, _book=_book)
         if stats_sink is not None and c_sum > 0:
             stats_sink["cells_max_over_mean"] = 64.0 * c_max / c_sum
         if SPECULATE and use_runs:
@@ -493,7 +515,11 @@
                 a.sm_ray_indices = None
                 _launch(a)
                 B.call("nfa_fill_ray_indices", n_rays, B.ptr(packed_info), B.ptr(ray_indices), B.stream())
-    info = tag_trusted(packed_info, n_sm)
+    n_tiles = 0
+    if tiles is not None:
+        real_tile_elems, n_tiles = B.seg_plan(n_sm, n_rays)
+        tiles = tiles[:int(B.load().nfa_seg_table_rows(n_tiles))] if (n_sm <= cap and real_tile_elems == tile_elems) else None
+    info = tag_trusted(packed_info, n_sm, tiles, n_tiles)
     tag_ray_indices(ray_indices, n_rays, info)
     if use_runs and not masked:
         tag_const_step(t_starts, t_ends, step_size)
```

After: 735.1 million rays/s, median of 6. +1.4%, better.
